# STLABTW/ST-DADK

Measured on NVIDIA B200. Metric: train_samples_per_s, higher is better.
Workload: dtype tf32

## Files before the change

### include/stdadk.h

```cpp
#ifndef STDADK_H
#define STDADK_H
#include <stddef.h>
#include <stdint.h>

#ifdef __cplusplus
extern "C" {
#endif

#define STDADK_VERSION 100
#define STDADK_MAX_Q 8

enum { STDADK_WENDLAND = 0, STDADK_GAUSSIAN = 1, STDADK_TRIANGULAR = 2 };
enum { STDADK_LOSS_NONE = 0, STDADK_LOSS_MSE = 1, STDADK_LOSS_PINBALL = 2 };

typedef struct {
    const float* knots4;
    const float* tknots2;
    int32_t k_s, k_t, p_cov, basis_fn;
} stdadk_basis;

typedef struct {
    const float* coords;
    const float* t;
    const float* xcov;
    const int64_t* index;
    int32_t grid_nx, grid_ny, grid_nt, _pad;
    int64_t row_begin;
    int64_t n_rows;
} stdadk_points;

typedef struct {
    const float* w_img;
    const float* bias;
    const float* gamma;
    const float* beta;
    int32_t n_in, n_out;
    float ln_eps;
    int32_t layer_id;
    const float* w_img_lo;
} stdadk_layer;

typedef struct {
    float p;
    uint32_t step;
    uint64_t seed;
    const int32_t* step_ptr;
    uint64_t key_offset;
} stdadk_dropout;

typedef struct {
    const float* w;
    const float* b;
    int32_t q;
    int32_t loss_type;
    const float* y;
    float taus[STDADK_MAX_Q];
    float inv_count;
    float nc_weight;
    int32_t nc_power;
    int32_t _pad;
    float* yhat;
    float* dyhat;
    float* loss_acc;
} stdadk_head;

typedef struct {
    const stdadk_basis* basis;
    stdadk_points pts;
    const float* a_img;
    stdadk_layer layer;
    stdadk_dropout drop;
    float* out_img;
    float* stats;
    const stdadk_head* head;
    const float* addend;
    float* feat_img;
    float* x_img;
    const float* a_img_lo;
    float* out_img_lo;
} stdadk_fwd_args;

typedef struct {
    const stdadk_basis* basis;
    stdadk_points pts;
    const float* a_img;
    stdadk_layer layer;
    stdadk_dropout drop;
    const float* stats;
    const stdadk_head* head;
    float* d_head_w;
    float* d_head_b;
    const float* dz_next_img;
    const float* wt_next_img;
    int32_t n_next, _pad;
    float* dz_img;
    float* d_bias;
    float* d_gamma;
    float* d_beta;
    const float* addend;
    const float* x_img;
    const float* a_img_lo;
    const float* dz_next_img_lo;
    const float* wt_next_img_lo;
    float* dz_img_lo;
} stdadk_bwd_args;

typedef struct {
    const stdadk_basis* basis;
    stdadk_points pts;
    const float* a_img;
    const float* dz_img;
    int32_t n_in, n_out;
    float* dw;
    int64_t stride_o, stride_i;
    const float* a_img_lo;
    const float* dz_img_lo;
} stdadk_wgrad_args;

typedef struct {
    const stdadk_basis* basis;
    stdadk_points pts;
    const float* dz_img;
    const float* w1s_img;
    int32_t n_out, _pad;
    float* d_centers;
    float* d_log_bw;
    const float* dz_img_lo;
    const float* w1s_img_lo;
} stdadk_knotgrad_args;

typedef struct {
    float* p;
    const float* g;
    float* m;
    float* v;
    float* shadow;
    int64_t n;
    int32_t n_groups;
    int32_t zero_grad;
    const int64_t* group_end;
    const float* hyper;
    const float* sqnorms;
    int32_t* step_count;
    float beta1, beta2, eps, ema_decay;
    float* loss_acc;
    float* loss_sum;
    float* loss_last;
    int32_t fuse_norm;
    int32_t _pad;
    float* norm_ws;
} stdadk_adamw_args;

int stdadk_version(void);
const char* stdadk_last_error(void);
size_t stdadk_sizeof(int which);

size_t stdadk_image_floats(int64_t rows, int64_t cols);

int stdadk_knots_prepare(const float* centers, const float* bw, const float* log_bw, float calib, int k,
                         float* knots4, void* stream);
int stdadk_tknots_prepare(const float* centers, const float* bw, int k, float* tknots2, void* stream);

int stdadk_basis_fwd(const stdadk_basis* basis, const stdadk_points* pts, float* phi, float* psi, void* stream);

int stdadk_pack_image(const float* src, int64_t row_stride, int64_t col_stride, int64_t rows, int64_t cols,
                      float* img, void* stream);
int stdadk_unpack_image(const float* img, int64_t rows, int64_t cols, float* dst, void* stream);
#define STDADK_MAX_PACK 8
typedef struct {
    const float* src;
    int64_t row_stride, col_stride, rows, cols;
    float* img;
    int32_t part;
    int32_t _pad;
} stdadk_pack_desc;
int stdadk_pack_images(const stdadk_pack_desc* descs, int n, void* stream);

size_t stdadk_celllist_ws_bytes(int32_t k_s, int32_t n_levels);
int stdadk_celllist_build(const float* knots4, int32_t k_s, const int32_t* level_begin, int32_t n_levels, void* ws,
                          size_t ws_bytes, void* stream);
#define STDADK_MAX_LEVELS 8
typedef struct {
    stdadk_points pts;
    const float* knots4;
    int32_t n_levels, basis_fn, n_out, p_cov;
    int32_t side[STDADK_MAX_LEVELS];
    int32_t offset[STDADK_MAX_LEVELS];
    float thetap[STDADK_MAX_LEVELS];
    const float* w1t;
    float* zs;
    const float* dz_img;
    float* dw1t;
    const void* celllist;
    int32_t celllist_k_s, _pad;
    float* d_centers;
    float* d_log_bw;
} stdadk_sparse_args;
int stdadk_sparse_l1_fwd(const stdadk_sparse_args* a, void* stream);
int stdadk_sparse_l1_wgrad(const stdadk_sparse_args* a, void* stream);

#define STDADK_MAX_HIDDEN 4
typedef struct {
    const stdadk_basis* basis;
    stdadk_points pts;
    int32_t n_layers, _pad;
    stdadk_layer layers[STDADK_MAX_HIDDEN];
    const stdadk_head* head;
} stdadk_predict_args;
int stdadk_predict_supported(const stdadk_predict_args* a);
int stdadk_predict(const stdadk_predict_args* a, void* stream);

typedef struct {
    const stdadk_basis* basis;
    const float* sites;
    int32_t grid_nx, grid_ny;
    int64_t n_sites;
    int32_t n_times, k_begin, k_end, n_layers;
    int64_t site_begin, site_end;
    stdadk_layer layers[STDADK_MAX_HIDDEN];
    const float* w1;
    int64_t w1_row_stride, w1_col_stride;
    const stdadk_head* head;
    int64_t row_base;
    float* zt_ws;
    int64_t out_k_stride;
} stdadk_field_args;
int stdadk_predict_field_supported(const stdadk_field_args* a);
int stdadk_predict_field(const stdadk_field_args* a, void* stream);

int stdadk_layer_fwd(const stdadk_fwd_args* a, void* stream);
int stdadk_layer_bwd(const stdadk_bwd_args* a, void* stream);
int stdadk_wgrad(const stdadk_wgrad_args* a, void* stream);

int stdadk_dense_basis_supported(int32_t n_in, int32_t n_out, int32_t k_s, int32_t k_t, int32_t q_head, int32_t training);
int32_t stdadk_dense_max_knots(int32_t p_cov, int32_t k_t, int32_t n_out, int32_t q_head, int32_t training);
int stdadk_knot_grad(const stdadk_knotgrad_args* a, void* stream);

size_t stdadk_sqnorm_ws_floats(void);
int stdadk_grad_sqnorm(const float* g, int64_t n, int n_groups, const int64_t* group_end, float* sqnorms,
                       float* workspace, void* stream);
int stdadk_adamw_ema_step(const stdadk_adamw_args* a, void* stream);

#define STDADK_MAX_PEERS 8
typedef struct {
    int32_t world, rank;
    float* g;
    int64_t n;
    void* recv[STDADK_MAX_PEERS];
    const int32_t* step_count;
    int32_t n_groups;
    int32_t mode;
    const int64_t* group_end;
    float* sqnorms;
    float* workspace;
} stdadk_peer_allreduce_args;
int stdadk_peer_allreduce(const stdadk_peer_allreduce_args* a, void* stream);

#ifdef __cplusplus
}
#endif
#endif
```

### st_dadk_b200/_lib.py

```python
from __future__ import annotations

import ctypes as C
import os

_HERE = os.path.dirname(os.path.abspath(__file__))
LIB_PATH = os.environ.get("STDADK_LIB") or os.path.join(_HERE, "libstdadk.so")
MAX_Q = 8

WENDLAND, GAUSSIAN, TRIANGULAR = 0, 1, 2
LOSS_NONE, LOSS_MSE, LOSS_PINBALL = 0, 1, 2
BASIS_CODE = {"wendland": WENDLAND, "gaussian": GAUSSIAN, "triangular": TRIANGULAR}
CALIBRATION = {"wendland": 1.0, "gaussian": 0.223477, "triangular": 0.654714}

fp = C.c_void_p


class Basis(C.Structure):
    _fields_ = [("knots4", fp), ("tknots2", fp), ("k_s", C.c_int32), ("k_t", C.c_int32), ("p_cov", C.c_int32),
                ("basis_fn", C.c_int32)]


class Points(C.Structure):
    _fields_ = [("coords", fp), ("t", fp), ("xcov", fp), ("index", fp), ("grid_nx", C.c_int32), ("grid_ny", C.c_int32),
                ("grid_nt", C.c_int32), ("_pad", C.c_int32), ("row_begin", C.c_int64), ("n_rows", C.c_int64)]


class Layer(C.Structure):
    _fields_ = [("w_img", fp), ("bias", fp), ("gamma", fp), ("beta", fp), ("n_in", C.c_int32), ("n_out", C.c_int32),
                ("ln_eps", C.c_float), ("layer_id", C.c_int32), ("w_img_lo", fp)]


class Dropout(C.Structure):
    _fields_ = [("p", C.c_float), ("step", C.c_uint32), ("seed", C.c_uint64), ("step_ptr", fp),
                ("key_offset", C.c_uint64)]


class Head(C.Structure):
    _fields_ = [("w", fp), ("b", fp), ("q", C.c_int32), ("loss_type", C.c_int32), ("y", fp),
                ("taus", C.c_float * MAX_Q), ("inv_count", C.c_float), ("nc_weight", C.c_float),
                ("nc_power", C.c_int32), ("_pad", C.c_int32), ("yhat", fp), ("dyhat", fp), ("loss_acc", fp)]


class FwdArgs(C.Structure):
    _fields_ = [("basis", C.POINTER(Basis)), ("pts", Points), ("a_img", fp), ("layer", Layer), ("drop", Dropout),
                ("out_img", fp), ("stats", fp), ("head", C.POINTER(Head)), ("addend", fp), ("feat_img", fp), ("x_img", fp),
                ("a_img_lo", fp), ("out_img_lo", fp)]


class BwdArgs(C.Structure):
    _fields_ = [("basis", C.POINTER(Basis)), ("pts", Points), ("a_img", fp), ("layer", Layer), ("drop", Dropout),
                ("stats", fp), ("head", C.POINTER(Head)), ("d_head_w", fp), ("d_head_b", fp), ("dz_next_img", fp),
                ("wt_next_img", fp), ("n_next", C.c_int32), ("_pad", C.c_int32), ("dz_img", fp), ("d_bias", fp),
                ("d_gamma", fp), ("d_beta", fp), ("addend", fp), ("x_img", fp), ("a_img_lo", fp), ("dz_next_img_lo", fp),
                ("wt_next_img_lo", fp), ("dz_img_lo", fp)]


class WgradArgs(C.Structure):
    _fields_ = [("basis", C.POINTER(Basis)), ("pts", Points), ("a_img", fp), ("dz_img", fp), ("n_in", C.c_int32),
                ("n_out", C.c_int32), ("dw", fp), ("stride_o", C.c_int64), ("stride_i", C.c_int64), ("a_img_lo", fp),
                ("dz_img_lo", fp)]


class KnotGradArgs(C.Structure):
    _fields_ = [("basis", C.POINTER(Basis)), ("pts", Points), ("dz_img", fp), ("w1s_img", fp), ("n_out", C.c_int32),
                ("_pad", C.c_int32), ("d_centers", fp), ("d_log_bw", fp), ("dz_img_lo", fp), ("w1s_img_lo", fp)]


class AdamWArgs(C.Structure):
    _fields_ = [("p", fp), ("g", fp), ("m", fp), ("v", fp), ("shadow", fp), ("n", C.c_int64),
                ("n_groups", C.c_int32), ("zero_grad", C.c_int32), ("group_end", C.POINTER(C.c_int64)), ("hyper", fp),
                ("sqnorms", fp), ("step_count", fp), ("beta1", C.c_float), ("beta2", C.c_float), ("eps", C.c_float),
                ("ema_decay", C.c_float), ("loss_acc", fp), ("loss_sum", fp), ("loss_last", fp), ("fuse_norm", C.c_int32),
                ("_pad", C.c_int32), ("norm_ws", fp)]


MAX_LEVELS = 8


class SparseArgs(C.Structure):
    _fields_ = [("pts", Points), ("knots4", fp), ("n_levels", C.c_int32), ("basis_fn", C.c_int32), ("n_out", C.c_int32),
                ("p_cov", C.c_int32), ("side", C.c_int32 * MAX_LEVELS), ("offset", C.c_int32 * MAX_LEVELS),
                ("thetap", C.c_float * MAX_LEVELS), ("w1t", fp), ("zs", fp), ("dz_img", fp), ("dw1t", fp),
                ("celllist", fp), ("celllist_k_s", C.c_int32), ("_pad", C.c_int32), ("d_centers", fp), ("d_log_bw", fp)]


class PackDesc(C.Structure):
    _fields_ = [("src", fp), ("row_stride", C.c_int64), ("col_stride", C.c_int64), ("rows", C.c_int64),
                ("cols", C.c_int64), ("img", fp), ("part", C.c_int32), ("_pad", C.c_int32)]


MAX_HIDDEN = 4


class PredictArgs(C.Structure):
    _fields_ = [("basis", C.POINTER(Basis)), ("pts", Points), ("n_layers", C.c_int32), ("_pad", C.c_int32),
                ("layers", Layer * MAX_HIDDEN), ("head", C.POINTER(Head))]


class FieldArgs(C.Structure):
    _fields_ = [("basis", C.POINTER(Basis)), ("sites", fp), ("grid_nx", C.c_int32), ("grid_ny", C.c_int32),
                ("n_sites", C.c_int64), ("n_times", C.c_int32), ("k_begin", C.c_int32), ("k_end", C.c_int32),
                ("n_layers", C.c_int32), ("site_begin", C.c_int64), ("site_end", C.c_int64),
                ("layers", Layer * MAX_HIDDEN), ("w1", fp), ("w1_row_stride", C.c_int64), ("w1_col_stride", C.c_int64),
                ("head", C.POINTER(Head)), ("row_base", C.c_int64), ("zt_ws", fp), ("out_k_stride", C.c_int64)]


MAX_PEERS = 8


class PeerAllreduceArgs(C.Structure):
    _fields_ = [("world", C.c_int32), ("rank", C.c_int32), ("g", fp), ("n", C.c_int64), ("recv", fp * MAX_PEERS),
                ("step_count", fp), ("n_groups", C.c_int32), ("mode", C.c_int32), ("group_end", C.POINTER(C.c_int64)),
                ("sqnorms", fp), ("workspace", fp)]


_lib = None

_PROTOS = {
    "stdadk_version": (C.c_int, []),
    "stdadk_last_error": (C.c_char_p, []),
    "stdadk_sizeof": (C.c_size_t, [C.c_int]),
    "stdadk_image_floats": (C.c_size_t, [C.c_int64, C.c_int64]),
    "stdadk_knots_prepare": (C.c_int, [fp, fp, fp, C.c_float, C.c_int, fp, fp]),
    "stdadk_tknots_prepare": (C.c_int, [fp, fp, C.c_int, fp, fp]),
    "stdadk_basis_fwd": (C.c_int, [C.POINTER(Basis), C.POINTER(Points), fp, fp, fp]),
    "stdadk_pack_image": (C.c_int, [fp, C.c_int64, C.c_int64, C.c_int64, C.c_int64, fp, fp]),
    "stdadk_unpack_image": (C.c_int, [fp, C.c_int64, C.c_int64, fp, fp]),
    "stdadk_pack_images": (C.c_int, [C.POINTER(PackDesc), C.c_int, fp]),
    "stdadk_predict_supported": (C.c_int, [C.POINTER(PredictArgs)]),
    "stdadk_predict": (C.c_int, [C.POINTER(PredictArgs), fp]),
    "stdadk_predict_field_supported": (C.c_int, [C.POINTER(FieldArgs)]),
    "stdadk_predict_field": (C.c_int, [C.POINTER(FieldArgs), fp]),
    "stdadk_peer_allreduce": (C.c_int, [C.POINTER(PeerAllreduceArgs), fp]),
    "stdadk_layer_fwd": (C.c_int, [C.POINTER(FwdArgs), fp]),
    "stdadk_layer_bwd": (C.c_int, [C.POINTER(BwdArgs), fp]),
    "stdadk_wgrad": (C.c_int, [C.POINTER(WgradArgs), fp]),
    "stdadk_dense_basis_supported": (C.c_int, [C.c_int32] * 6),
    "stdadk_dense_max_knots": (C.c_int32, [C.c_int32] * 5),
    "stdadk_knot_grad": (C.c_int, [C.POINTER(KnotGradArgs), fp]),
    "stdadk_sqnorm_ws_floats": (C.c_size_t, []),
    "stdadk_grad_sqnorm": (C.c_int, [fp, C.c_int64, C.c_int, C.POINTER(C.c_int64), fp, fp, fp]),
    "stdadk_adamw_ema_step": (C.c_int, [C.POINTER(AdamWArgs), fp]),
    "stdadk_celllist_ws_bytes": (C.c_size_t, [C.c_int32, C.c_int32]),
    "stdadk_celllist_build": (C.c_int, [fp, C.c_int32, C.POINTER(C.c_int32), C.c_int32, fp, C.c_size_t, fp]),
    "stdadk_sparse_l1_fwd": (C.c_int, [C.POINTER(SparseArgs), fp]),
    "stdadk_sparse_l1_wgrad": (C.c_int, [C.POINTER(SparseArgs), fp]),
}
EXPORTED = list(_PROTOS)


def lib():
    global _lib
    if _lib is None:
        if not os.path.exists(LIB_PATH):
            raise RuntimeError(
                f"{LIB_PATH} not found: build it with `python -c 'import __graft_entry__ as g; g.build()'` "
                "(nvcc, sm_100a).  st_dadk_b200 has no CPU or PyTorch fallback path.")
        L = C.CDLL(LIB_PATH)
        for name, (res, args) in _PROTOS.items():
            if not hasattr(L, name):
                continue
            fn = getattr(L, name)
            fn.restype = res
            fn.argtypes = args
        structs = [(0, Basis), (1, Points), (2, Layer), (3, Dropout), (4, Head), (5, FwdArgs), (6, BwdArgs), (7, WgradArgs),
                   (8, KnotGradArgs), (9, AdamWArgs), (10, PackDesc), (11, SparseArgs), (12, PredictArgs),
                   (14, PeerAllreduceArgs), (15, FieldArgs)]
        for i, st in structs:
            if L.stdadk_sizeof(i) != C.sizeof(st):
                raise RuntimeError(f"libstdadk ABI mismatch: {st.__name__} is {C.sizeof(st)} B in the binding, "
                                   f"{L.stdadk_sizeof(i)} B in the library")
        _lib = L
    return _lib


def check(code: int, what: str):
    if code != 0:
        msg = lib().stdadk_last_error().decode("utf-8", "replace")
        raise RuntimeError(f"libstdadk {what} failed (code {code}): {msg}")
```

### st_dadk_b200/csrc/api.cu

```cuda
#include <cstdarg>
#include <cstdio>
#include <cstring>

#include "layer.cuh"
#include "misc.cuh"
#include "sparse.cuh"
#include "predict.cuh"
#include "field.cuh"

using namespace stdadk;

static thread_local char g_err[512] = "";

static int fail(int code, const char* fmt, ...) {
    va_list ap;
    va_start(ap, fmt);
    vsnprintf(g_err, sizeof(g_err), fmt, ap);
    va_end(ap);
    return code;
}
static int check_launch(const char* what) {
    cudaError_t e = cudaGetLastError();
    if (e != cudaSuccess) return fail((int)e, "%s: %s", what, cudaGetErrorString(e));
    return 0;
// ... 183 lines not shown
    tknots_prepare_kernel<<<(k + 127) / 128, 128, 0, (cudaStream_t)stream>>>(centers, bw, k,
                                                                              reinterpret_cast<float2*>(tknots2));
    return check_launch("tknots_prepare");
}

int stdadk_basis_fwd(const stdadk_basis* basis, const stdadk_points* pts, float* phi, float* psi, void* stream) {
    if (int r = check_device()) return r;
    REQUIRE(basis && pts, "basis_fwd: NULL descriptor");
    if (int r = check_basis_points(basis, *pts, -1)) return r;
    if (pts->n_rows <= 0) return 0;
    long long total = pts->n_rows * (long long)(basis->k_s + basis->k_t);
    if (total == 0) return 0;
    basis_fwd_kernel<<<grid_for(total, 256), 256, 0, (cudaStream_t)stream>>>(to_basis(basis), to_points(*pts), phi,
                                                                              psi);
    return check_launch("basis_fwd");
}

int stdadk_pack_image(const float* src, int64_t row_stride, int64_t col_stride, int64_t rows, int64_t cols,
                      float* img, void* stream) {
    if (int r = check_device()) return r;
    REQUIRE(src && img && rows > 0 && cols > 0, "pack_image: bad arguments");
    REQUIRE((reinterpret_cast<uintptr_t>(img) & 127) == 0, "pack_image: image must be 128-byte aligned");
    int slabs = (int)ceil_div64(cols, SLAB_K);
    long long chunks = (long long)ceil_div64(rows, TILE_M) * slabs * (SLAB_FLOATS / 4);
    pack_image_kernel<<<grid_for(chunks, 256), 256, 0, (cudaStream_t)stream>>>(src, row_stride, col_stride, rows, cols,
                                                                                img, chunks, slabs);
    return check_launch("pack_image");
}

int stdadk_pack_images(const stdadk_pack_desc* descs, int n, void* stream) {
    if (int r = check_device()) return r;
    REQUIRE(descs && n >= 1 && n <= STDADK_MAX_PACK, "pack_images: 1..%d descriptors, got %d", STDADK_MAX_PACK, n);
    PackBatch B{};
    B.n = n;
    long long max_chunks = 0;
    for (int i = 0; i < n; ++i) {
        REQUIRE(descs[i].src && descs[i].img && descs[i].rows > 0 && descs[i].cols > 0, "pack_images: bad descriptor %d", i);
        REQUIRE((reinterpret_cast<uintptr_t>(descs[i].img) & 127) == 0, "pack_images: image %d must be 128-byte aligned", i);
        B.d[i] = descs[i];
        long long chunks = ceil_div64(descs[i].rows, TILE_M) * ceil_div64(descs[i].cols, SLAB_K) * (SLAB_FLOATS / 4);
        if (chunks > max_chunks) max_chunks = chunks;
    }
    dim3 grid(grid_for(max_chunks, 256, 2), n);
    launch_chained(pack_images_kernel, grid, 256, 0, stream, B);
    return check_launch("pack_images");
}

int stdadk_unpack_image(const float* img, int64_t rows, int64_t cols, float* dst, void* stream) {
    if (int r = check_device()) return r;
    REQUIRE(dst && img && rows > 0 && cols > 0, "unpack_image: bad arguments");
    int slabs = (int)ceil_div64(cols, SLAB_K);
    unpack_image_kernel<<<grid_for(rows * cols, 256), 256, 0, (cudaStream_t)stream>>>(img, rows, cols, dst, slabs);
    return check_launch("unpack_image");
}

static int check_layer(const stdadk_layer& l, const char* who) {
    REQUIRE(l.w_img && l.bias, "%s: weight image / bias is NULL", who);
    REQUIRE(l.n_out >= 1 && l.n_out <= MAX_N, "%s: n_out=%d outside [1,%d] (one UMMA N / LayerNorm row per thread)", who,
            l.n_out, MAX_N);
    REQUIRE(l.n_in >= 1, "%s: n_in=%d", who, l.n_in);
    REQUIRE((l.gamma == nullptr) == (l.beta == nullptr), "%s: gamma and beta must both be given or both NULL", who);
    REQUIRE(((reinterpret_cast<uintptr_t>(l.w_img) | reinterpret_cast<uintptr_t>(l.w_img_lo)) & 127) == 0,
            "%s: weight images must be 128-byte aligned", who);
    return 0;
}

constexpr uint32_t SMEM_LIMIT = 227 * 1024;
constexpr int BWD_CG = 2, BWD_NS = 4;
static uint32_t fwd_smem(int n_pad, int q, int k_s, int k_t, int tab_chunks, int cg) {
    return plan_smem(n_pad, q, k_s, k_t, false, cg, cg == 2 ? 2 : 4, tab_chunks).total;
}
static uint32_t bwd_smem(int n_pad, int q, int k_s, int k_t, int tab_chunks) {
    return plan_smem(n_pad, q, k_s, k_t, true, BWD_CG, BWD_NS, tab_chunks).total;
}

static unsigned long long* g_predict_dbg = nullptr;
int stdadk_layer_fwd(const stdadk_fwd_args* a, void* stream) {
    if (int r = check_device()) return r;
    REQUIRE(a, "layer_fwd: NULL args");
    if (int r = check_layer(a->layer, "layer_fwd")) return r;
    REQUIRE((a->basis != nullptr) != (a->a_img != nullptr), "layer_fwd: give exactly one of basis / a_img");
    if (a->basis)
        if (int r = check_basis_points(a->basis, a->pts, a->layer.n_in)) return r;
    REQUIRE(a->drop.p >= 0.0f && a->drop.p < 1.0f, "layer_fwd: dropout p=%f", a->drop.p);
    REQUIRE(!a->addend || (a->layer.n_out % 4 == 0 && (reinterpret_cast<uintptr_t>(a->addend) & 15) == 0),
            "layer_fwd: addend needs n_out %% 4 == 0 and 16-byte alignment");
    if (a->head) {
        REQUIRE(a->head->q >= 1 && a->head->q <= STDADK_MAX_Q, "layer_fwd: head q=%d outside [1,%d]", a->head->q,
                STDADK_MAX_Q);
        REQUIRE(a->head->w && a->head->b && a->head->yhat, "layer_fwd: head w/b/yhat NULL");
        REQUIRE(a->head->loss_type == STDADK_LOSS_NONE || (a->head->y && a->head->loss_acc),
                "layer_fwd: loss requested without y / loss_acc");
    } else {
        REQUIRE(a->out_img, "layer_fwd: out_img is NULL and there is no head");
    }
    const bool x3 = a->layer.w_img_lo != nullptr;
    if (x3) {
        REQUIRE(!a->a_img || a->a_img_lo, "layer_fwd: tf32x3 needs a_img_lo next to a_img");
        REQUIRE(!a->out_img || a->out_img_lo, "layer_fwd: tf32x3 needs out_img_lo next to out_img");
        REQUIRE(!a->feat_img, "layer_fwd: feat_img is not available in tf32x3 mode");
    }
    if (a->pts.n_rows <= 0) return 0;
    FwdK K{};
    K.basis = to_basis(a->basis);
    K.pts = to_points(a->pts);
    K.L = to_layer(a->layer, a->drop);
    K.head = to_head(a->head);
    K.a_img = a->a_img;
    K.a_img_lo = a->a_img_lo;
    K.out_img_lo = x3 ? a->out_img_lo : nullptr;
    K.passes = x3 ? 3 : 1;
    K.addend = a->addend;
    K.x_img = a->x_img;
    K.feat_img = a->basis ? a->feat_img : nullptr;
    K.dbg = g_predict_dbg;
    K.out_img = a->out_img;
    K.stats = a->stats;
    K.has_head = a->head ? 1 : 0;
    K.k_slabs = pad32(a->layer.n_in) / SLAB_K;
    K.n_pad = pad32(a->layer.n_out);
    K.thresh16 = dropout_thresh16(a->drop.p);
    K.drop_scale = a->drop.p > 0.0f ? 1.0f / (1.0f - a->drop.p) : 1.0f;
    const bool basis = a->basis != nullptr;
    int tiles = (int)ceil_div64(a->pts.n_rows, TILE_M);
    const int sms = g_sm_count > 0 ? g_sm_count : 148;
    const int cg = tiles >= 2 * sms ? 2 : 4;
    const bool half_tiles = 2 * tiles <= sms;
    if (half_tiles) tiles *= 2;
    K.tmem_cols = half_tiles ? tmem_cols_m64(K.n_pad) : pow2_cols(K.n_pad);
    const uint32_t smem = fwd_smem(K.n_pad, K.has_head ? K.head.q : 0, basis ? K.basis.k_s : 0, basis ? K.basis.k_t : 0,
                                   basis ? K.k_slabs * 8 : 0, cg);
    REQUIRE(smem <= SMEM_LIMIT, "layer_fwd: needs %u B of shared memory (> 227 KB): too many knots for the dense path",
            smem);
    K.n_tiles = tiles;
#define LAUNCH_FWD(B, TM, C)                                                                                 \
    do {                                                                                                     \
        if (int r = set_smem(layer_fwd_kernel<B, TM, C, (C == 2 ? 2 : 4)>, smem)) return r;                  \
        launch_chained(layer_fwd_kernel<B, TM, C, (C == 2 ? 2 : 4)>, dim3(tiles), n_threads(C), smem, stream, K); \
    } while (0)
    if (basis) {
        if (half_tiles) LAUNCH_FWD(true, 64, 4);
        else if (cg == 2) LAUNCH_FWD(true, 128, 2);
        else LAUNCH_FWD(true, 128, 4);
    } else {
        if (half_tiles) LAUNCH_FWD(false, 64, 4);
        else if (cg == 2) LAUNCH_FWD(false, 128, 2);
        else LAUNCH_FWD(false, 128, 4);
    }
#undef LAUNCH_FWD
    return check_launch("layer_fwd");
}

extern "C" void stdadk_debug_counters(void* dev_u64x16) { g_predict_dbg = static_cast<unsigned long long*>(dev_u64x16); }

static int fill_pred_layers(const stdadk_layer* layers, int n_layers, PredLayerP* out, const char* who) {
    for (int l = 0; l < n_layers; ++l) {
        const stdadk_layer& y = layers[l];
        if (int r = check_layer(y, who)) return r;
        REQUIRE(l == 0 || y.n_in == layers[l - 1].n_out, "%s: block %d n_in=%d != previous n_out=%d", who, l, y.n_in,
                layers[l - 1].n_out);
        PredLayerP& L = out[l];
        L.w_img = y.w_img;
        L.bias = y.bias;
        L.gamma = y.gamma;
        L.beta = y.beta;
        L.n_out = y.n_out;
        L.n_pad = pad32(y.n_out);
        L.k_slabs = pad32(y.n_in) / SLAB_K;
        L.has_ln = y.gamma != nullptr;
        L.eps = y.ln_eps;
    }
    return 0;
}

static int predict_fill(const stdadk_predict_args* a, PredK* K) {
    REQUIRE(a && a->basis && a->head, "predict: NULL args / basis / head");
    REQUIRE(a->n_layers >= 1 && a->n_layers <= PF_MAX_LAYERS, "predict: %d hidden blocks outside [1,%d]", a->n_layers,
            PF_MAX_LAYERS);
    if (int r = check_basis_points(a->basis, a->pts, a->layers[0].n_in)) return r;
    REQUIRE(a->head->q >= 1 && a->head->q <= STDADK_MAX_Q, "predict: head q=%d outside [1,%d]", a->head->q, STDADK_MAX_Q);
    REQUIRE(a->head->w && a->head->b && a->head->yhat, "predict: head w/b/yhat NULL");
    *K = PredK{};
    K->basis = to_basis(a->basis);
    K->pts = to_points(a->pts);
    K->n_layers = a->n_layers;
    K->q = a->head->q;
    K->head_w = a->head->w;
    K->head_b = a->head->b;
    K->yhat = a->head->yhat;
    if (int r = fill_pred_layers(a->layers, a->n_layers, K->L, "predict")) return r;
    uint32_t bytes = plan_predict(*K);
    REQUIRE(bytes <= 227 * 1024, "predict: the fused kernel needs %u B of shared memory (> 227 KB) for this shape", bytes);
    K->n_tiles = (int)ceil_div64(a->pts.n_rows, TILE_M);
    K->dbg = g_predict_dbg;
    return 0;
}

int stdadk_predict_supported(const stdadk_predict_args* a) {
    PredK K;
    return predict_fill(a, &K) == 0 ? 1 : 0;
}

int stdadk_predict(const stdadk_predict_args* a, void* stream) {
    if (int r = check_device()) return r;
    PredK Kl;
    if (int r = predict_fill(a, &Kl)) return r;
    if (a->pts.n_rows <= 0) return 0;
    if (int r = set_smem(predict_fused_kernel, Kl.sm.total)) return r;
    const int sms = g_sm_count > 0 ? g_sm_count : 148;
    const int grid = Kl.n_tiles < sms ? Kl.n_tiles : sms;
    predict_fused_kernel<<<grid, PF_NT, Kl.sm.total, (cudaStream_t)stream>>>(Kl);
    return check_launch("predict");
}

static int field_fill(const stdadk_field_args* a, FieldK* K) {
    REQUIRE(a && a->basis && a->head, "predict_field: NULL args / basis / head");
    REQUIRE(a->n_layers >= 1 && a->n_layers <= PF_MAX_LAYERS, "predict_field: %d hidden blocks outside [1,%d]", a->n_layers,
            PF_MAX_LAYERS);
    const stdadk_basis* b = a->basis;
    REQUIRE(b->p_cov == 0, "predict_field: covariates (p_cov=%d) are per (site, time): use stdadk_predict", b->p_cov);
    REQUIRE(b->k_s >= 1 && b->knots4 && (b->k_t == 0 || b->tknots2), "predict_field: basis tables missing");
    REQUIRE(((reinterpret_cast<uintptr_t>(b->knots4)) & 15) == 0, "predict_field: knots4 must be 16-byte aligned");
    REQUIRE(b->basis_fn >= 0 && b->basis_fn <= 2, "predict_field: unknown basis_fn %d", b->basis_fn);
    REQUIRE(a->layers[0].n_in == b->k_s, "predict_field: layers[0] is the spatial part: n_in=%d != k_s=%d", a->layers[0].n_in,
            b->k_s);
    REQUIRE(a->n_sites >= 1 && a->n_times >= 1, "predict_field: n_sites / n_times");
    REQUIRE(a->sites || (a->grid_nx > 0 && a->grid_ny > 0 && (int64_t)a->grid_nx * a->grid_ny == a->n_sites),
            "predict_field: give sites or a lattice with nx*ny == n_sites");
    REQUIRE(!a->sites || (reinterpret_cast<uintptr_t>(a->sites) & 7) == 0, "predict_field: sites must be 8-byte aligned");
    REQUIRE(0 <= a->k_begin && a->k_begin <= a->k_end && a->k_end <= a->n_times, "predict_field: time range");
    REQUIRE(0 <= a->site_begin && a->site_begin <= a->site_end && a->site_end <= a->n_sites, "predict_field: site range");
    REQUIRE(a->out_k_stride >= 0, "predict_field: out_k_stride");
    REQUIRE(a->head->q >= 1 && a->head->q <= STDADK_MAX_Q && a->head->w && a->head->b && a->head->yhat,
            "predict_field: head q / w / b / yhat");
    REQUIRE(a->w1 && a->zt_ws && (reinterpret_cast<uintptr_t>(a->zt_ws) & 15) == 0, "predict_field: w1 / zt_ws");
    *K = FieldK{};
    K->basis = to_basis(b);
    K->basis.k_t = 0;
    K->basis.tknots = nullptr;
    K->sites = a->sites;
    K->nx = a->grid_nx;
    K->ny = a->grid_ny;
    K->n_sites = a->n_sites;
    K->site_begin = a->site_begin;
    K->site_end = a->site_end;
    K->k_begin = a->k_begin;
    K->k_end = a->k_end;
    K->n_layers = a->n_layers;
    K->q = a->head->q;
    K->head_w = a->head->w;
    K->head_b = a->head->b;
    K->yhat = a->head->yhat;
    K->row_base = a->row_base;
    K->out_k_stride = a->out_k_stride > 0 ? a->out_k_stride : a->n_sites;
    K->zt = a->zt_ws;
    K->dbg = g_predict_dbg;
    if (int r = fill_pred_layers(a->layers, a->n_layers, K->L, "predict_field")) return r;
    REQUIRE(K->L[0].k_slabs <= PF_HSLABS, "predict_field: %d spatial knots exceed the resident operand (%d)", b->k_s,
            PF_HSLABS * SLAB_K);
    uint32_t bytes = plan_field(*K);
    REQUIRE(bytes <= 227 * 1024, "predict_field: the kernel needs %u B of shared memory (> 227 KB) for this shape", bytes);
    const int sms = g_sm_count > 0 ? g_sm_count : 148;
    const long long n_s = a->site_end - a->site_begin;
    const int tk = a->k_end - a->k_begin;
    K->n_site_tiles = (int)ceil_div64(n_s, TILE_M);
    int best_chunk = tk > 0 ? tk : 1;
    double best_cost = 1e30;
    for (int chunk = 1; chunk <= tk; ++chunk) {
        const long long units = (long long)K->n_site_tiles * ((tk + chunk - 1) / chunk);
        const double cost = (double)ceil_div64(units, sms) * (chunk + 1.0);
        if (cost < best_cost - 1e-9 || (cost < best_cost + 1e-9 && chunk > best_chunk)) {
            best_cost = cost;
            best_chunk = chunk;
        }
    }
    K->k_chunk = best_chunk;
    K->n_kchunks = tk > 0 ? (tk + best_chunk - 1) / best_chunk : 0;
    const long long units = (long long)K->n_site_tiles * K->n_kchunks;
    REQUIRE(units < (1ll << 31), "predict_field: too many work units");
    K->n_units = (int)units;
    return 0;
}

int stdadk_predict_field_supported(const stdadk_field_args* a) {
    FieldK K;
    return field_fill(a, &K) == 0 ? 1 : 0;
}

int stdadk_predict_field(const stdadk_field_args* a, void* stream) {
    if (int r = check_device()) return r;
    FieldK K;
    if (int r = field_fill(a, &K)) return r;
    if (K.n_units <= 0) return 0;
    const int pad0 = K.L[0].n_pad, total = a->n_times * pad0;
    field_zt_kernel<<<(total + 255) / 256, 256, 0, (cudaStream_t)stream>>>(
        a->w1, a->w1_row_stride, a->w1_col_stride, a->basis->k_s, a->layers[0].bias,
        reinterpret_cast<const float2*>(a->basis->tknots2), a->basis->k_t, K.L[0].n_out, pad0, a->n_times, a->zt_ws);
    if (int r = check_launch("predict_field (zt)")) return r;
    if (int r = set_smem(predict_field_kernel, K.sm.total)) return r;
    const int sms = g_sm_count > 0 ? g_sm_count : 148;
    const int grid = K.n_units < sms ? K.n_units : sms;
    predict_field_kernel<<<grid, PF_NT, K.sm.total, (cudaStream_t)stream>>>(K);
    return check_launch("predict_field");
}

int stdadk_layer_bwd(const stdadk_bwd_args* a, void* stream) {
    if (int r = check_device()) return r;
    REQUIRE(a, "layer_bwd: NULL args");
    if (int r = check_layer(a->layer, "layer_bwd")) return r;
    REQUIRE(a->x_img || ((a->basis != nullptr) != (a->a_img != nullptr)), "layer_bwd: give exactly one of basis / a_img");
    if (a->basis && !a->x_img)
        if (int r = check_basis_points(a->basis, a->pts, a->layer.n_in)) return r;
    REQUIRE((a->head != nullptr) != (a->dz_next_img != nullptr), "layer_bwd: give exactly one of head / dz_next_img");
    REQUIRE(a->dz_img && a->d_bias, "layer_bwd: dz_img / d_bias NULL");
    REQUIRE(!a->layer.gamma || (a->d_gamma && a->d_beta && a->stats), "layer_bwd: LayerNorm needs d_gamma/d_beta/stats");
    if (a->head) {
        REQUIRE(a->head->q >= 1 && a->head->q <= STDADK_MAX_Q && a->head->w && a->head->dyhat && a->d_head_w &&
                    a->d_head_b,
                "layer_bwd: head arguments incomplete");
    } else {
        REQUIRE(a->wt_next_img && a->n_next >= 1 && a->n_next <= MAX_N, "layer_bwd: wt_next_img / n_next invalid");
    }
    const bool x3 = a->layer.w_img_lo != nullptr;
    if (x3) {
        REQUIRE(a->x_img || !a->a_img || a->a_img_lo, "layer_bwd: tf32x3 needs a_img_lo next to a_img");
        REQUIRE(a->head || (a->dz_next_img_lo && a->wt_next_img_lo), "layer_bwd: tf32x3 needs dz_next_img_lo / wt_next_img_lo");
        REQUIRE(a->dz_img_lo, "layer_bwd: tf32x3 needs dz_img_lo");
    }
    if (a->pts.n_rows <= 0) return 0;
    BwdK K{};
    K.basis = to_basis(a->basis);
    K.pts = to_points(a->pts);
    K.L = to_layer(a->layer, a->drop);
    K.head = to_head(a->head);
    K.a_img = a->a_img;
    K.a_img_lo = a->a_img_lo;
    K.dz_next_img_lo = a->dz_next_img_lo;
    K.wt_next_img_lo = a->wt_next_img_lo;
    K.dz_img_lo = x3 ? a->dz_img_lo : nullptr;
    K.passes = x3 ? 3 : 1;
    K.addend = a->addend;
    K.x_img = a->x_img;
    K.stats = a->stats;
    K.dz_next_img = a->dz_next_img;
    K.wt_next_img = a->wt_next_img;
    K.dz_img = a->dz_img;
    K.d_bias = a->d_bias;
    K.d_gamma = a->d_gamma;
    K.d_beta = a->d_beta;
    K.d_head_w = a->d_head_w;
    K.d_head_b = a->d_head_b;
    K.has_head = a->head ? 1 : 0;
    K.k_slabs = a->x_img ? 0 : pad32(a->layer.n_in) / SLAB_K;
    K.k_slabs2 = a->head ? 0 : pad32(a->n_next) / SLAB_K;
    K.n_pad = pad32(a->layer.n_out);
    K.thresh16 = dropout_thresh16(a->drop.p);
    K.drop_scale = a->drop.p > 0.0f ? 1.0f / (1.0f - a->drop.p) : 1.0f;
    const bool basis = a->basis != nullptr && a->x_img == nullptr;
    constexpr int BCG = BWD_CG, BNS = BWD_NS;
    const uint32_t smem = bwd_smem(K.n_pad, K.has_head ? K.head.q : 0, basis ? K.basis.k_s : 0, basis ? K.basis.k_t : 0,
                                   basis ? K.k_slabs * 8 : 0);
    REQUIRE(smem <= SMEM_LIMIT, "layer_bwd: needs %u B of shared memory (> 227 KB)", smem);
    int tiles = (int)ceil_div64(a->pts.n_rows, TILE_M);
    const int sms = g_sm_count > 0 ? g_sm_count : 148;
    const bool half_tiles = a->x_img && 2 * tiles <= sms;
    if (half_tiles) tiles *= 2;
    K.tmem_cols = 2 * (half_tiles ? tmem_cols_m64(K.n_pad) : pow2_cols(K.n_pad));
    const bool ln = a->layer.gamma != nullptr, hd = a->head != nullptr;
#define LAUNCH_BWD(B, TM, LNV, HD)                                                                          \
    do {                                                                                                    \
        if (int r = set_smem(layer_bwd_kernel<B, TM, BCG, BNS, LNV, HD>, smem)) return r;                   \
        launch_chained(layer_bwd_kernel<B, TM, BCG, BNS, LNV, HD>, dim3(tiles), n_threads(BCG), smem, stream, K); \
    } while (0)
    if (half_tiles) {
        if (ln && hd) LAUNCH_BWD(false, 64, true, true);
        else if (ln) LAUNCH_BWD(false, 64, true, false);
        else if (hd) LAUNCH_BWD(false, 64, false, true);
        else LAUNCH_BWD(false, 64, false, false);
    } else if (basis) {
        if (ln && hd) LAUNCH_BWD(true, 128, true, true);
        else if (ln) LAUNCH_BWD(true, 128, true, false);
        else if (hd) LAUNCH_BWD(true, 128, false, true);
        else LAUNCH_BWD(true, 128, false, false);
    } else {
        if (ln && hd) LAUNCH_BWD(false, 128, true, true);
        else if (ln) LAUNCH_BWD(false, 128, true, false);
        else if (hd) LAUNCH_BWD(false, 128, false, true);
        else LAUNCH_BWD(false, 128, false, false);
    }
#undef LAUNCH_BWD
    return check_launch("layer_bwd");
}

int stdadk_wgrad(const stdadk_wgrad_args* a, void* stream) {
    if (int r = check_device()) return r;
    REQUIRE(a, "wgrad: NULL args");
    REQUIRE((a->basis != nullptr) != (a->a_img != nullptr), "wgrad: give exactly one of basis / a_img");
    REQUIRE(a->dz_img && a->dw, "wgrad: dz_img / dw NULL");
    REQUIRE(a->n_out >= 1 && a->n_out <= MAX_N && a->n_in >= 1, "wgrad: bad sizes n_in=%d n_out=%d", a->n_in, a->n_out);
    if (a->basis)
        if (int r = check_basis_points(a->basis, a->pts, a->n_in)) return r;
    if (a->pts.n_rows <= 0) return 0;
    const bool x3 = a->dz_img_lo != nullptr;
    REQUIRE(!x3 || !a->a_img || a->a_img_lo, "wgrad: tf32x3 needs a_img_lo next to a_img");
    WgradK K{};
    K.basis = to_basis(a->basis);
    K.pts = to_points(a->pts);
    K.a_img = a->a_img;
    K.a_img_lo = a->a_img_lo;
    K.dz_img_lo = a->dz_img_lo;
    K.passes = x3 ? 3 : 1;
    K.dz_img = a->dz_img;
    K.dw = a->dw;
    K.stride_o = a->stride_o;
    K.stride_i = a->stride_i;
    K.n_in = a->n_in;
    K.n_out = a->n_out;
    K.a_slabs = pad32(a->n_in) / SLAB_K;
    K.dz_slabs = pad32(a->n_out) / SLAB_K;
    K.n_row_tiles = (int)ceil_div64(a->pts.n_rows, TILE_M);
    int n_tiles_n = (K.a_slabs + 7) / 8;
    K.nt_slabs = (K.a_slabs + n_tiles_n - 1) / n_tiles_n;
    K.tmem_cols = pow2_cols(K.nt_slabs * SLAB_K);
    int m_tiles = (K.dz_slabs + 3) / 4;
    int per = m_tiles * n_tiles_n;
    int sms = g_sm_count > 0 ? g_sm_count : 148;
    int splits = sms / per;
    if (splits < 1) splits = 1;
    if (splits > K.n_row_tiles) splits = K.n_row_tiles;
    const bool basis = a->basis != nullptr;
    uint32_t smem = wgrad_smem_bytes(basis ? K.basis.k_s : 0, basis ? K.basis.k_t : 0);
    REQUIRE(smem <= SMEM_LIMIT, "wgrad: needs %u B of shared memory (> 227 KB)", smem);
    dim3 grid(splits, m_tiles, n_tiles_n);
    constexpr int WCG = 2;
    if (basis) {
        if (int r = set_smem(wgrad_kernel<true, WCG>, smem)) return r;
        launch_chained(wgrad_kernel<true, WCG>, grid, n_threads(WCG), smem, stream, K);
    } else {
        if (int r = set_smem(wgrad_kernel<false, WCG>, smem)) return r;
        launch_chained(wgrad_kernel<false, WCG>, grid, n_threads(WCG), smem, stream, K);
    }
    return check_launch("wgrad");
}

static int dense_basis_check(int n_in, int n_out, int k_s, int k_t, int q_head, int training) {
    REQUIRE(n_out >= 1 && n_out <= MAX_N && k_s >= 0 && k_t >= 0 && n_in >= k_s + k_t && q_head >= 0 &&
                q_head <= STDADK_MAX_Q,
            "dense_basis_supported: bad sizes n_in=%d n_out=%d k_s=%d k_t=%d q_head=%d", n_in, n_out, k_s, k_t, q_head);
    const int n_pad = pad32(n_out), tab_chunks = pad32(n_in) / SLAB_K * 8;
    for (int cg : {4, 2}) {
        const uint32_t b = fwd_smem(n_pad, q_head, k_s, k_t, tab_chunks, cg);
        REQUIRE(b <= SMEM_LIMIT, "layer_fwd: needs %u B of shared memory (> 227 KB): too many knots for the dense path", b);
    }
    if (!training) return 0;
    const uint32_t bb = bwd_smem(n_pad, q_head, k_s, k_t, tab_chunks);
    REQUIRE(bb <= SMEM_LIMIT, "layer_bwd: needs %u B of shared memory (> 227 KB)", bb);
    const uint32_t wb = wgrad_smem_bytes(k_s, k_t);
    REQUIRE(wb <= SMEM_LIMIT, "wgrad: needs %u B of shared memory (> 227 KB)", wb);
    return 0;
}

int stdadk_dense_basis_supported(int32_t n_in, int32_t n_out, int32_t k_s, int32_t k_t, int32_t q_head, int32_t training) {
    return dense_basis_check(n_in, n_out, k_s, k_t, q_head, training) == 0 ? 1 : 0;
}

int32_t stdadk_dense_max_knots(int32_t p_cov, int32_t k_t, int32_t n_out, int32_t q_head, int32_t training) {
    if (p_cov < 0 || dense_basis_check(p_cov + k_t, n_out, 0, k_t, q_head, training)) return -1;
    int lo = 0, hi = 1 << 14;
    while (hi - lo > 1) {
        const int mid = (lo + hi) / 2;
        if (dense_basis_check(p_cov + mid + k_t, n_out, mid, k_t, q_head, training) == 0) lo = mid;
        else hi = mid;
    }
    return lo;
}

int stdadk_knot_grad(const stdadk_knotgrad_args* a, void* stream) {
    if (int r = check_device()) return r;
    REQUIRE(a && a->basis && a->dz_img && a->w1s_img && a->d_centers && a->d_log_bw, "knot_grad: NULL argument");
    if (int r = check_basis_points(a->basis, a->pts, -1)) return r;
    REQUIRE(a->n_out >= 1 && a->n_out <= MAX_N, "knot_grad: n_out=%d", a->n_out);
    if (a->pts.n_rows <= 0 || a->basis->k_s == 0) return 0;
    KnotGradK K{};
    K.basis = to_basis(a->basis);
    K.pts = to_points(a->pts);
    REQUIRE((a->dz_img_lo != nullptr) == (a->w1s_img_lo != nullptr), "knot_grad: give both residual images or neither");
    K.dz_img = a->dz_img;
    K.w1s_img = a->w1s_img;
    K.dz_img_lo = a->dz_img_lo;
    K.w1s_img_lo = a->w1s_img_lo;
    K.passes = a->dz_img_lo ? 3 : 1;
    K.d_centers = a->d_centers;
    K.d_log_bw = a->d_log_bw;
    K.n_out = a->n_out;
    K.k_slabs = pad32(a->n_out) / SLAB_K;
// ... 42 lines not shown
    }
    REQUIRE((a->d_centers == nullptr) == (a->d_log_bw == nullptr), "sparse_l1: give d_centers and d_log_bw together");
    REQUIRE(!(wgrad && a->d_centers) || (a->w1t && (reinterpret_cast<uintptr_t>(a->w1t) & 15) == 0),
            "sparse_l1_wgrad: knot gradients need w1t (G = dz1 . W1t row)");
    K->d_centers = wgrad ? a->d_centers : nullptr;
    K->d_log_bw = wgrad ? a->d_log_bw : nullptr;
    K->knots = reinterpret_cast<const float4*>(a->knots4);
    K->w1t = a->w1t;
    K->zs = a->zs;
    K->dz_img = a->dz_img;
    K->dw1t = a->dw1t;
    K->n_out = a->n_out;
    K->p_cov = a->p_cov;
    K->fn = a->basis_fn;
    return 0;
}

static int make_groups(int n_groups, const int64_t* group_end, int64_t n, GroupsP* G) {
    REQUIRE(n_groups >= 1 && n_groups <= 8 && group_end, "optimizer: 1..8 parameter groups supported, got %d", n_groups);
    int64_t prev = 0;
    for (int i = 0; i < n_groups; ++i) {
        REQUIRE(group_end[i] >= prev, "optimizer: group_end must be non-decreasing");
        G->end[i] = prev = group_end[i];
    }
    REQUIRE(prev == n, "optimizer: last group_end (%lld) != n (%lld)", (long long)prev, (long long)n);
    G->n = n_groups;
    return 0;
}

size_t stdadk_celllist_ws_bytes(int32_t k_s, int32_t n_levels) {
    if (k_s < 0 || n_levels < 1 || n_levels > SP_MAX_LEVELS) return 0;
    return celllist_bytes(k_s, n_levels);
}

int stdadk_celllist_build(const float* knots4, int32_t k_s, const int32_t* level_begin, int32_t n_levels, void* ws,
                          size_t ws_bytes, void* stream) {
    if (int r = check_device()) return r;
    REQUIRE(knots4 && level_begin && ws && k_s >= 1, "celllist_build: NULL argument / no knots");
    REQUIRE(n_levels >= 1 && n_levels <= SP_MAX_LEVELS, "celllist_build: 1..%d levels, got %d", SP_MAX_LEVELS, n_levels);
    REQUIRE(((reinterpret_cast<uintptr_t>(ws) | reinterpret_cast<uintptr_t>(knots4)) & 15) == 0,
            "celllist_build: knots4 / workspace must be 16-byte aligned");
    REQUIRE(ws_bytes >= celllist_bytes(k_s, n_levels), "celllist_build: workspace of %zu B, need %zu B", ws_bytes,
            celllist_bytes(k_s, n_levels));
    CellBuildK K{};
    K.knots = reinterpret_cast<const float4*>(knots4);
    K.k_s = k_s;
    K.n_levels = n_levels;
    for (int l = 0; l <= n_levels; ++l) {
        REQUIRE(level_begin[l] >= (l ? level_begin[l - 1] : 0) && level_begin[l] <= k_s, "celllist_build: level_begin not monotone");
        K.level_begin[l] = level_begin[l];
    }
    REQUIRE(level_begin[0] == 0 && level_begin[n_levels] == k_s, "celllist_build: levels must cover [0, k_s)");
    K.ws = static_cast<int*>(ws);
    size_t ib = (celllist_ints(k_s, n_levels) * 4 + 15) & ~(size_t)15;
    K.sorted = reinterpret_cast<float4*>(static_cast<uint8_t*>(ws) + ib);
    celllist_build_kernel<<<1, CL_THREADS, 0, (cudaStream_t)stream>>>(K);
    return check_launch("celllist_build");
}

size_t stdadk_sqnorm_ws_floats(void) { return (size_t)SQNORM_BLOCKS * 8 + 8; }

int stdadk_grad_sqnorm(const float* g, int64_t n, int n_groups, const int64_t* group_end, float* sqnorms,
                       float* workspace, void* stream) {
    if (int r = check_device()) return r;
    REQUIRE(g && sqnorms && workspace && n > 0, "grad_sqnorm: bad arguments (workspace of stdadk_sqnorm_ws_floats() "
            "zero-initialised floats is required)");
    REQUIRE((reinterpret_cast<uintptr_t>(g) & 15) == 0, "grad_sqnorm: g must be 16-byte aligned");
    GroupsP G{};
    if (int r = make_groups(n_groups, group_end, n, &G)) return r;
    long long blocks = ((n >> 2) + SQNORM_THREADS * 4 - 1) / (SQNORM_THREADS * 4);
    if (blocks < 1) blocks = 1;
    if (blocks > SQNORM_BLOCKS) blocks = SQNORM_BLOCKS;
    sqnorm_kernel<<<(int)blocks, SQNORM_THREADS, 0, (cudaStream_t)stream>>>(g, n, G, sqnorms, workspace);
    return check_launch("grad_sqnorm");
}

int stdadk_sparse_l1_fwd(const stdadk_sparse_args* a, void* stream) {
    if (int r = check_device()) return r;
    SparseK K{};
    if (int r = sparse_fill(a, &K, false)) return r;
    if (a->pts.n_rows <= 0) return 0;
    int blocks = grid_for(a->pts.n_rows, SP_WARPS, 8);
    sparse_spatial_fwd_kernel<<<blocks, SP_WARPS * 32, 0, (cudaStream_t)stream>>>(K);
    return check_launch("sparse_l1_fwd");
}

int stdadk_sparse_l1_wgrad(const stdadk_sparse_args* a, void* stream) {
    if (int r = check_device()) return r;
    SparseK K{};
    if (int r = sparse_fill(a, &K, true)) return r;
    if (a->pts.n_rows <= 0) return 0;
    int blocks = grid_for(a->pts.n_rows, SP_WARPS, 8);
    sparse_spatial_wgrad_kernel<<<blocks, SP_WARPS * 32, 0, (cudaStream_t)stream>>>(K);
    return check_launch("sparse_l1_wgrad");
}

__global__ void step_inc_kernel(int* c) { *c += 1; }

int stdadk_peer_allreduce(const stdadk_peer_allreduce_args* a, void* stream) {
    if (int r = check_device()) return r;
    REQUIRE(a && a->g && a->step_count, "peer_allreduce: NULL argument");
    REQUIRE(a->world >= 2 && a->world <= PEER_MAX && a->rank >= 0 && a->rank < a->world,
            "peer_allreduce: world=%d rank=%d outside [2,%d]", a->world, a->rank, PEER_MAX);
    REQUIRE(a->n > 0 && a->n % 4 == 0, "peer_allreduce: n=%lld must be a positive multiple of 4", (long long)a->n);
    static_assert(PEER_MAX == STDADK_MAX_PEERS, "peer limits differ");
    REQUIRE((reinterpret_cast<uintptr_t>(a->g) & 15) == 0, "peer_allreduce: g must be 16-byte aligned");
    PeerK K{};
    for (int r = 0; r < a->world; ++r) {
        REQUIRE(a->recv[r] && (reinterpret_cast<uintptr_t>(a->recv[r]) & 15) == 0,
                "peer_allreduce: rank %d receive area not mapped / not 16-byte aligned", r);
        K.recv[r] = static_cast<uint4*>(a->recv[r]);
    }
    K.g = a->g;
    K.n2 = a->n / 2;
    K.step_count = a->step_count;
    K.rank = a->rank;
    K.world = a->world;
    REQUIRE(a->mode >= 0 && a->mode <= 2, "peer_allreduce: mode=%d (0 automatic, 1 one-shot, 2 two-phase)", a->mode);
    K.two_phase = a->mode == 2 || (a->mode == 0 && a->world >= 4);
    if (a->n_groups > 0) {
        REQUIRE(a->group_end && a->sqnorms && a->workspace, "peer_allreduce: fused norm needs group_end / sqnorms / workspace");
        K.n_norm = a->group_end[a->n_groups - 1];
        REQUIRE(K.n_norm <= a->n, "peer_allreduce: norm range exceeds n");
        if (int r = make_groups(a->n_groups, a->group_end, K.n_norm, &K.G)) return r;
        K.sq_out = a->sqnorms;
        K.ws = a->workspace;
    }
    long long blocks = (K.n2 + PEER_THREADS * 2 - 1) / (PEER_THREADS * 2);
    if (blocks > 148) blocks = 148;
    if (blocks < 1) blocks = 1;
    peer_allreduce_kernel<<<(int)blocks, PEER_THREADS, 0, (cudaStream_t)stream>>>(K);
    return check_launch("peer_allreduce");
}

int stdadk_adamw_ema_step(const stdadk_adamw_args* a, void* stream) {
    if (int r = check_device()) return r;
    REQUIRE(a && a->p && a->g && a->m && a->v && a->hyper && a->step_count && a->n > 0, "adamw: bad arguments");
    AdamK K{};
    if (int r = make_groups(a->n_groups, a->group_end, a->n, &K.G)) return r;
    K.p = a->p;
    K.g = a->g;
    K.m = a->m;
    K.v = a->v;
    K.shadow = a->shadow;
    K.n = a->n;
    K.hyper = a->hyper;
    K.sqnorms = a->sqnorms;
    K.step_count = a->step_count;
    K.beta1 = a->beta1;
    K.beta2 = a->beta2;
    K.eps = a->eps;
    K.ema_decay = a->ema_decay;
    K.g_zero = a->zero_grad ? const_cast<float*>(a->g) : nullptr;
    K.loss_acc = a->loss_acc;
    K.loss_sum = a->loss_sum;
    K.loss_last = a->loss_last;
    REQUIRE(((reinterpret_cast<uintptr_t>(a->p) | reinterpret_cast<uintptr_t>(a->g) | reinterpret_cast<uintptr_t>(a->m) |
              reinterpret_cast<uintptr_t>(a->v) | reinterpret_cast<uintptr_t>(a->shadow)) & 15) == 0,
            "adamw: buffers must be 16-byte aligned");
    if (a->fuse_norm) {
        REQUIRE(a->norm_ws, "adamw: fuse_norm needs norm_ws");
        K.sq_out = const_cast<float*>(a->sqnorms);
        K.norm_ws = a->norm_ws;
        K.step_rw = a->step_count;
        long long blocks = ((a->n + 3) / 4 + 255) / 256;
        if (blocks > 148) blocks = 148;
        const int sms = g_sm_count > 0 ? g_sm_count : 148;
        if (blocks > sms) blocks = sms;
        if (blocks < 1) blocks = 1;
        launch_chained(adamw_ema_kernel<true>, dim3((unsigned)blocks), 256, 0, stream, K);
        return check_launch("adamw_ema_step (fused tail)");
    }
    step_inc_kernel<<<1, 1, 0, (cudaStream_t)stream>>>(a->step_count);
    adamw_ema_kernel<false><<<grid_for((a->n + 3) / 4, 256, 8), 256, 0, (cudaStream_t)stream>>>(K);
    return check_launch("adamw_ema_step");
}

}
```

### st_dadk_b200/csrc/common.cuh

```cuda
#pragma once
#include <cuda_runtime.h>
#include <stdint.h>
#include <type_traits>

#include "../../include/stdadk.h"
#include "ptx.cuh"

namespace stdadk {

constexpr int TILE_M = 128;
constexpr int SLAB_K = 32;
constexpr int SLAB_FLOATS = TILE_M * SLAB_K;
constexpr int SLAB_BYTES = SLAB_FLOATS * 4;
constexpr int MAX_N = 256;

__host__ __device__ inline int pad32(int x) { return (x + 31) & ~31; }
__host__ __device__ inline int64_t ceil_div64(int64_t a, int64_t b) { return (a + b - 1) / b; }

struct BasisP {
    const float4* knots;
    const float2* tknots;
    int k_s, k_t, p_cov, fn;
};
struct PointsP {
    const float* coords;
    const float* t;
    const float* xcov;
    const long long* index;
    int nx, ny, nt, _pad;
    long long row_begin;
    long long n_rows;
};
struct HeadP {
    const float* w;
    const float* b;
    const float* y;
    float* yhat;
    float* dyhat;
    float* loss_acc;
    int q, loss_type, nc_power, _pad;
    float inv_count, nc_weight;
    float taus[STDADK_MAX_Q];
};
struct LayerP {
    const float* w_img;
    const float* w_img_lo;
    const float* bias;
    const float* gamma;
    const float* beta;
    int n_in, n_out, layer_id, _pad;
    float eps, drop_p;
    unsigned int step, _pad2;
    unsigned long long seed;
    const int* step_ptr;
    unsigned long long key_offset;
};
__device__ __forceinline__ unsigned int dropout_step(const LayerP& L) {
    return L.step_ptr ? (unsigned int)(*L.step_ptr) : L.step;
}
__device__ __forceinline__ long long sample_of(const PointsP& P, long long g) { return P.index ? P.index[g] : g; }

__device__ __forceinline__ float rsqrt_approx(float x) {
    float r;
    asm("rsqrt.approx.ftz.f32 %0, %1;" : "=f"(r) : "f"(x));
    return r;
}
__device__ __forceinline__ float ex2_approx(float x) {
    float r;
    asm("ex2.approx.ftz.f32 %0, %1;" : "=f"(r) : "f"(x));
    return r;
}
template <int FN>
__device__ __forceinline__ float phi_from_d2(float d2, float th2, float inv_th) {
    if (FN == STDADK_GAUSSIAN) return ex2_approx(-0.72134752044448170f * (d2 * inv_th * inv_th));
    const float r = d2 * rsqrt_approx(fmaxf(d2, 1e-30f)) * inv_th;
    const float u = fmaxf(1.0f - r, 0.0f);
    float v;
    if (FN == STDADK_TRIANGULAR) {
        v = u;
    } else {
        const float u2 = u * u;
        v = (u2 * u2) * u2 * fmaf(fmaf(35.0f / 3.0f, r, 6.0f), r, 1.0f);
    }
    return d2 < th2 ? v : 0.0f;
}
__device__ __forceinline__ float phi_eval(int fn, float dx, float dy, float th2, float inv_th) {
    const float d2 = __fadd_rn(__fmul_rn(dx, dx), __fmul_rn(dy, dy));
    if (fn == STDADK_GAUSSIAN) return phi_from_d2<STDADK_GAUSSIAN>(d2, th2, inv_th);
    if (!(d2 < th2)) return 0.0f;
    if (fn == STDADK_TRIANGULAR) return phi_from_d2<STDADK_TRIANGULAR>(d2, th2, inv_th);
    return phi_from_d2<STDADK_WENDLAND>(d2, th2, inv_th);
}
__device__ __forceinline__ float phi_dr(int fn, float r) {
    if (fn == STDADK_GAUSSIAN) return -r * exp2f(-0.72134752044448170f * r * r);
    if (!(r < 1.0f)) return 0.0f;
    if (fn == STDADK_TRIANGULAR) return -1.0f;
    float u = 1.0f - r;
    float u2 = u * u;
    return -(56.0f / 3.0f) * r * fmaf(5.0f, r, 1.0f) * u2 * u2 * u;
}
__device__ __forceinline__ float psi_eval(float t, float c, float inv_bw) {
    float s = (t - c) * inv_bw;
    return ex2_approx(-0.72134752044448170f * s * s);
}

__device__ __forceinline__ void load_point(const PointsP& P, long long g, float& x, float& y, float& t) {
    if (P.nx > 0) {
        long long j = g % P.ny;
        long long i = (g / P.ny) % P.nx;
        long long k = g / ((long long)P.ny * P.nx);
        x = P.nx > 1 ? __fdiv_rn((float)i, (float)(P.nx - 1)) : 0.0f;
        y = P.ny > 1 ? __fdiv_rn((float)j, (float)(P.ny - 1)) : 0.0f;
        t = P.nt > 1 ? __fdiv_rn((float)k, (float)(P.nt - 1)) : 0.0f;
    } else {
        long long sidx = sample_of(P, g);
        float2 c = *reinterpret_cast<const float2*>(P.coords + 2 * sidx);
        x = c.x;
        y = c.y;
        t = P.t[sidx];
    }
}

__device__ __forceinline__ float feature_value(const BasisP& B, const float4* sk, const float2* st, int f, float x,
                                               float y, float t, const float* xrow) {
    if (f < B.p_cov) return xrow ? xrow[f] : 0.0f;
    f -= B.p_cov;
    if (f < B.k_s) {
        float4 kn = sk[f];
        return phi_eval(B.fn, x - kn.x, y - kn.y, kn.z, kn.w);
    }
    f -= B.k_s;
    if (f < B.k_t) {
        float2 tk = st[f];
        return psi_eval(t, tk.x, tk.y);
    }
    return 0.0f;
}

__device__ __forceinline__ void philox4x32_10(uint32_t c0, uint32_t c1, uint32_t c2, uint32_t c3, uint32_t k0,
                                              uint32_t k1, uint32_t (&out)[4]) {
#pragma unroll
    for (int i = 0; i < 10; ++i) {
        uint32_t hi0 = __umulhi(0xD2511F53u, c0), lo0 = 0xD2511F53u * c0;
        uint32_t hi1 = __umulhi(0xCD9E8D57u, c2), lo1 = 0xCD9E8D57u * c2;
        c0 = hi1 ^ c1 ^ k0;
        c1 = lo1;
        c2 = hi0 ^ c3 ^ k1;
        c3 = lo0;
        k0 += 0x9E3779B9u;
        k1 += 0xBB67AE85u;
    }
    out[0] = c0; out[1] = c1; out[2] = c2; out[3] = c3;
}
__device__ __noinline__ uint32_t dropout_keep8(unsigned long long seed, uint32_t step, uint32_t layer,
                                                  unsigned long long row, uint32_t block, uint32_t thresh16) {
    uint32_t o[4];
    philox4x32_10((uint32_t)row, block, layer | ((uint32_t)(row >> 32) << 8), step, (uint32_t)seed,
                  (uint32_t)(seed >> 32), o);
    uint32_t bits = 0;
#pragma unroll
    for (int e = 0; e < 8; ++e) {
// ... 31 lines not shown
```

### st_dadk_b200/csrc/layer.cuh

```cuda
#pragma once
#include "common.cuh"

namespace stdadk {

constexpr int WG_NSTAGE = 2;
constexpr int RED_STRIDE = 4 + STDADK_MAX_Q;
__host__ __device__ constexpr int n_work(int cg) { return 128 * cg; }
__host__ __device__ constexpr int n_threads(int cg) { return 128 * cg + 64; }
__device__ __forceinline__ void worker_barrier(int nw) { asm volatile("bar.sync 1, %0;" ::"r"(nw) : "memory"); }

template <int TM>
struct TileGeo {
    static_assert(TM == 128 || TM == 64, "tile height");
    static constexpr int ROWS_PER_WARP = TM / 4;
    static constexpr int WARP_COLS = TM == 128 ? 32 : 64;
    __device__ static int row(int q4, int lane) { return q4 * ROWS_PER_WARP + (TM == 128 ? lane : (lane & 15)); }
    __device__ static int chunk_off(int lane) { return TM == 128 ? 0 : (lane >> 4) * 32; }
    __device__ static int group(int cg, int lane) { return TM == 128 ? cg : 2 * cg + (lane >> 4); }
    __host__ __device__ static constexpr int groups(int cg) { return TM == 128 ? cg : 2 * cg; }
};
template <int TM>
__device__ __forceinline__ void acc_ld(uint32_t taddr, float (&v)[32]) {
    if (TM == 128) tmem_ld32(taddr, v);
    else tmem_ld16x2<32>(taddr, v);
}
__device__ __forceinline__ float2 halfwarp_transpose_sum(float (&v)[32], int lane) {
#pragma unroll
    for (int off = 8, n = 16; off >= 1; off >>= 1, n >>= 1) {
        bool upper = (lane & off) != 0;
#pragma unroll
        for (int i = 0; i < n; ++i) {
            float send = upper ? v[i] : v[i + n];
            float keep = upper ? v[i + n] : v[i];
            v[i] = keep + __shfl_xor_sync(0xffffffffu, send, off);
        }
    }
    return make_float2(v[0], v[1]);
}
template <int TM>
__device__ __forceinline__ void colsum_chunk(float* cs, int c0, bool cvalid, float (&v)[32], int lane) {
    if (TM == 128) {
        const float s = warp_transpose_sum(v, lane);
        atomicAdd(&cs[c0 + lane], s);
    } else {
        const float2 s = halfwarp_transpose_sum(v, lane);
        if (cvalid) {
            atomicAdd(&cs[c0 + 2 * (lane & 15)], s.x);
            atomicAdd(&cs[c0 + 2 * (lane & 15) + 1], s.y);
        }
    }
}

struct SmemPlan {
    uint32_t a_off, b_off, bar_off, tmem_off, vec_off, headw_off, knots_off, tknots_off, colsum_off, red_off, total;
};
__host__ __device__ inline SmemPlan plan_smem(int n_pad, int q, int k_s, int k_t, bool bwd, int cg = 1, int ns = 2,
                                              int tab_chunks = 0) {
    SmemPlan s;
    uint32_t o = 0;
    s.a_off = o; o += ns * SLAB_BYTES;
    s.b_off = o; o += ns * (uint32_t)n_pad * 128u;
    s.bar_off = o; o += 128;
    s.tmem_off = o; o += 16;
    s.vec_off = o; o += 4u * n_pad * 4u;
    s.headw_off = o; o += (uint32_t)(q > 0 ? (q * n_pad + STDADK_MAX_Q) * 4 : 0);
    o = (o + 15u) & ~15u;
    s.knots_off = o; o += tab_chunks > 0 ? (uint32_t)tab_chunks * 64u : (uint32_t)k_s * 16u;
    s.tknots_off = o; o += tab_chunks > 0 ? 0u : (uint32_t)k_t * 8u;
    o = (o + 15u) & ~15u;
    s.colsum_off = o; o += bwd ? (uint32_t)((3 + q) * n_pad + STDADK_MAX_Q) * 4u : 0u;
    s.red_off = s.a_off;
    (void)cg;
    s.total = o + 1024;
    return s;
}

struct FwdK {
    BasisP basis;
    PointsP pts;
    LayerP L;
    HeadP head;
    const float* a_img;
    const float* a_img_lo;
    const float* addend;
    float* out_img;
    float* out_img_lo;
    float* x_img;
    float* feat_img;
    float* stats;
    int has_head, k_slabs, n_pad, tmem_cols;
    unsigned int thresh16;
    float drop_scale;
    int n_tiles, passes;
    unsigned long long* dbg;
};
#ifdef STDADK_PF_DEBUG
#define FWD_T(slot)                                                       \
    do {                                                                  \
        if (P.dbg && tid == 0) {                                          \
            unsigned long long now_;                                      \
            asm volatile("mov.u64 %0, %%globaltimer;" : "=l"(now_));      \
            atomicAdd(P.dbg + (slot), now_ - t_prev_);                    \
            t_prev_ = now_;                                               \
        }                                                                 \
    } while (0)
#define FWD_WAIT(slot, stmt)                                               \
    do {                                                                   \
        unsigned long long w0_ = 0, w1_;                                   \
        if (P.dbg) asm volatile("mov.u64 %0, %%globaltimer;" : "=l"(w0_)); \
        stmt;                                                              \
        if (P.dbg) {                                                       \
            asm volatile("mov.u64 %0, %%globaltimer;" : "=l"(w1_));        \
            atomicAdd(P.dbg + (slot), w1_ - w0_);                          \
        }                                                                  \
    } while (0)
#else
#define FWD_T(slot)
#define FWD_WAIT(slot, stmt) stmt
#endif

struct BwdK {
    BasisP basis;
    PointsP pts;
    LayerP L;
    HeadP head;
    const float* a_img;
    const float* a_img_lo;
    const float* addend;
    const float* x_img;
    const float* stats;
    const float* dz_next_img;
    const float* dz_next_img_lo;
    const float* wt_next_img;
    const float* wt_next_img_lo;
    float* dz_img;
    float* dz_img_lo;
    float* d_bias;
    float* d_gamma;
    float* d_beta;
    float* d_head_w;
    float* d_head_b;
    int has_head, k_slabs, k_slabs2, n_pad, tmem_cols, passes;
    unsigned int thresh16;
    float drop_scale;
};

template <int FN>
__device__ __forceinline__ float4 spatial_chunk(const float4* kp, float x, float y, bool lo) {
    float d2[4], th2[4], ith[4];
    bool in = false;
#pragma unroll
    for (int e = 0; e < 4; ++e) {
        const float4 kn = kp[e];
        const float dx = x - kn.x, dy = y - kn.y;
        d2[e] = __fadd_rn(__fmul_rn(dx, dx), __fmul_rn(dy, dy));
        th2[e] = kn.z;
        ith[e] = kn.w;
        in |= d2[e] < th2[e];
    }
    if (FN != STDADK_GAUSSIAN && !__any_sync(__activemask(), in)) return make_float4(0.f, 0.f, 0.f, 0.f);
    float o[4];
#pragma unroll
    for (int e = 0; e < 4; ++e) o[e] = tf32_part(phi_from_d2<FN>(d2[e], th2[e], ith[e]), lo);
    return make_float4(o[0], o[1], o[2], o[3]);
}
__device__ __forceinline__ float4 feature_chunk(const BasisP& B, const float4* sk, const float2* st, int f, float x,
                                                float y, float t, const float* xrow, bool lo = false) {
    const int s0 = B.p_cov, s1 = B.p_cov + B.k_s, t1 = s1 + B.k_t;
    if (f >= s0 && f + 4 <= s1) {
        const float4* kp = sk + (f - s0);
        if (B.fn == STDADK_WENDLAND) return spatial_chunk<STDADK_WENDLAND>(kp, x, y, lo);
        if (B.fn == STDADK_TRIANGULAR) return spatial_chunk<STDADK_TRIANGULAR>(kp, x, y, lo);
        return spatial_chunk<STDADK_GAUSSIAN>(kp, x, y, lo);
    }
    if (f >= s1 && f + 4 <= t1) {
        const float2* tp = st + (f - s1);
        float o[4];
#pragma unroll
        for (int e = 0; e < 4; ++e) {
            float2 tk = tp[e];
            o[e] = tf32_part(psi_eval(t, tk.x, tk.y), lo);
        }
        return make_float4(o[0], o[1], o[2], o[3]);
    }
    if (f >= t1) return make_float4(0.f, 0.f, 0.f, 0.f);
    return make_float4(tf32_part(feature_value(B, sk, st, f + 0, x, y, t, xrow), lo),
                       tf32_part(feature_value(B, sk, st, f + 1, x, y, t, xrow), lo),
                       tf32_part(feature_value(B, sk, st, f + 2, x, y, t, xrow), lo),
                       tf32_part(feature_value(B, sk, st, f + 3, x, y, t, xrow), lo));
}

__device__ __forceinline__ int chunk_kind(const BasisP& B, int f) {
    const int s0 = B.p_cov, s1 = s0 + B.k_s, t1 = s1 + B.k_t;
    if (f >= s0 && f + 4 <= s1) return 0;
    if (f >= s1 && f + 4 <= t1) return 1;
    if (f >= t1) return 2;
    return 3;
}
__device__ __forceinline__ void build_chunk_tables(const BasisP& B, float4* tab, int n_chunks, int tid, int nt) {
    for (int ci = tid; ci < n_chunks; ci += nt) {
        const int f = 4 * ci, kind = chunk_kind(B, f);
        float4* g = tab + 4 * ci;
        if (kind == 0) {
            const float4* kp = B.knots + (f - B.p_cov);
            const float4 k0 = kp[0], k1 = kp[1], k2 = kp[2], k3 = kp[3];
            g[0] = make_float4(k0.x, k1.x, k2.x, k3.x);
            g[1] = make_float4(k0.y, k1.y, k2.y, k3.y);
            g[2] = make_float4(k0.z, k1.z, k2.z, k3.z);
            g[3] = make_float4(k0.w, k1.w, k2.w, k3.w);
        } else if (kind == 1) {
            const float2* tp = B.tknots + (f - B.p_cov - B.k_s);
            const float2 t0 = tp[0], t1 = tp[1], t2 = tp[2], t3 = tp[3];
            g[0] = make_float4(t0.x, t1.x, t2.x, t3.x);
            g[1] = make_float4(t0.y, t1.y, t2.y, t3.y);
        }
    }
}
template <int FN, bool LO, int NC>
__device__ __forceinline__ void spatial_chunks_soa(const float4* g, float2 xx, float2 yy, float4 (&out)[NC]) {
    constexpr bool lo = LO;
    float2 d2a[NC], d2b[NC];
    float4 th2[NC], ith[NC];
    bool in = false;
#pragma unroll
    for (int k = 0; k < NC; ++k) {
        const float4 cx = g[4 * k], cy = g[4 * k + 1];
        th2[k] = g[4 * k + 2];
        ith[k] = g[4 * k + 3];
        const float2 dxa = sub2(xx, make_float2(cx.x, cx.y)), dxb = sub2(xx, make_float2(cx.z, cx.w));
        const float2 dya = sub2(yy, make_float2(cy.x, cy.y)), dyb = sub2(yy, make_float2(cy.z, cy.w));
        const float2 pxa = mul2(dxa, dxa), pya = mul2(dya, dya), pxb = mul2(dxb, dxb), pyb = mul2(dyb, dyb);
        d2a[k] = make_float2(__fadd_rn(pxa.x, pya.x), __fadd_rn(pxa.y, pya.y));
        d2b[k] = make_float2(__fadd_rn(pxb.x, pyb.x), __fadd_rn(pxb.y, pyb.y));
        in |= (d2a[k].x < th2[k].x) | (d2a[k].y < th2[k].y) | (d2b[k].x < th2[k].z) | (d2b[k].y < th2[k].w);
    }
    if (FN == STDADK_GAUSSIAN) {
        const float2 kk = make_float2(-0.72134752044448170f, -0.72134752044448170f);
#pragma unroll
        for (int k = 0; k < NC; ++k) {
            const float2 ia = make_float2(ith[k].x, ith[k].y), ib = make_float2(ith[k].z, ith[k].w);
            const float2 ea = mul2(kk, mul2(mul2(d2a[k], ia), ia)), eb = mul2(kk, mul2(mul2(d2b[k], ib), ib));
            out[k] = make_float4(tf32_part(ex2_approx(ea.x), lo), tf32_part(ex2_approx(ea.y), lo),
                                 tf32_part(ex2_approx(eb.x), lo), tf32_part(ex2_approx(eb.y), lo));
        }
        return;
    }
    if (!__any_sync(__activemask(), in)) {
#pragma unroll
        for (int k = 0; k < NC; ++k) out[k] = make_float4(0.f, 0.f, 0.f, 0.f);
        return;
    }
    const float2 one = make_float2(1.0f, 1.0f);
#pragma unroll
    for (int k = 0; k < NC; ++k) {
        const float2 qa = make_float2(rsqrt_approx(fmaxf(d2a[k].x, 1e-30f)), rsqrt_approx(fmaxf(d2a[k].y, 1e-30f)));
        const float2 qb = make_float2(rsqrt_approx(fmaxf(d2b[k].x, 1e-30f)), rsqrt_approx(fmaxf(d2b[k].y, 1e-30f)));
        const float2 ra = mul2(mul2(d2a[k], qa), make_float2(ith[k].x, ith[k].y));
        const float2 rb = mul2(mul2(d2b[k], qb), make_float2(ith[k].z, ith[k].w));
        float2 ua = sub2(one, ra), ub = sub2(one, rb);
        ua = make_float2(fmaxf(ua.x, 0.0f), fmaxf(ua.y, 0.0f));
        ub = make_float2(fmaxf(ub.x, 0.0f), fmaxf(ub.y, 0.0f));
        float2 va = ua, vb = ub;
        if (FN == STDADK_WENDLAND) {
            const float2 c35 = make_float2(35.0f / 3.0f, 35.0f / 3.0f), c6 = make_float2(6.0f, 6.0f);
            const float2 u2a = mul2(ua, ua), u2b = mul2(ub, ub);
            va = mul2(mul2(mul2(u2a, u2a), u2a), fma2(fma2(c35, ra, c6), ra, one));
            vb = mul2(mul2(mul2(u2b, u2b), u2b), fma2(fma2(c35, rb, c6), rb, one));
        }
        out[k] = make_float4(tf32_part(d2a[k].x < th2[k].x ? va.x : 0.0f, lo), tf32_part(d2a[k].y < th2[k].y ? va.y : 0.0f, lo),
                             tf32_part(d2b[k].x < th2[k].z ? vb.x : 0.0f, lo), tf32_part(d2b[k].y < th2[k].w ? vb.y : 0.0f, lo));
    }
}
template <int FN, bool LO>
__device__ __forceinline__ float4 spatial_chunk_soa(const float4* g, float2 xx, float2 yy) {
    float4 o[1];
    spatial_chunks_soa<FN, LO, 1>(g, xx, yy, o);
    return o[0];
}
template <bool LO>
__device__ __forceinline__ float4 temporal_chunk_soa(const float4* g, float2 tt) {
    constexpr bool lo = LO;
    const float4 c = g[0], ib = g[1];
    const float2 kk = make_float2(-0.72134752044448170f, -0.72134752044448170f);
    const float2 sa = mul2(sub2(tt, make_float2(c.x, c.y)), make_float2(ib.x, ib.y));
    const float2 sb = mul2(sub2(tt, make_float2(c.z, c.w)), make_float2(ib.z, ib.w));
    const float2 ea = mul2(mul2(kk, sa), sa), eb = mul2(mul2(kk, sb), sb);
    return make_float4(tf32_part(ex2_approx(ea.x), lo), tf32_part(ex2_approx(ea.y), lo), tf32_part(ex2_approx(eb.x), lo),
                       tf32_part(ex2_approx(eb.y), lo));
}
template <int FN, bool LO, int NC>
__device__ __forceinline__ void gen_basis_slab_soa(const BasisP& B, const float4* tab, int slab, float x, float y, float t,
                                                   const float* xrow, uint32_t slab_saddr, uint32_t r, int c_begin, int c_end,
                                                   float* gslab) {
    constexpr bool lo = LO;
    const float2 xx = make_float2(x, x), yy = make_float2(y, y), tt = make_float2(t, t);
// ... 94 lines not shown
#pragma unroll
    for (int c = 0; c < 8; ++c) {
        const float4 hi = make_float4(to_tf32(v[4 * c]), to_tf32(v[4 * c + 1]), to_tf32(v[4 * c + 2]), to_tf32(v[4 * c + 3]));
        *reinterpret_cast<float4*>(reinterpret_cast<uint8_t*>(img + off) + swz_off(row, c)) = hi;
        if (img_lo)
            *reinterpret_cast<float4*>(reinterpret_cast<uint8_t*>(img_lo + off) + swz_off(row, c)) =
                make_float4(to_tf32(v[4 * c] - hi.x), to_tf32(v[4 * c + 1] - hi.y), to_tf32(v[4 * c + 2] - hi.z),
                            to_tf32(v[4 * c + 3] - hi.w));
    }
}

__device__ __forceinline__ uint8_t* align_smem(uint8_t* p) {
    return p + ((1024u - (smem_u32(p) & 1023u)) & 1023u);
}

__device__ __forceinline__ void add_addend_chunk(float (&v)[32], const float* addend_row, int c0, int n_out) {
#pragma unroll
    for (int c = 0; c < 8; ++c) {
        if (c0 + 4 * c < n_out) {
            float4 a = *reinterpret_cast<const float4*>(addend_row + c0 + 4 * c);
            v[4 * c] += a.x; v[4 * c + 1] += a.y; v[4 * c + 2] += a.z; v[4 * c + 3] += a.w;
        }
    }
}

__device__ __forceinline__ void image_store_chunk(float* img, int tile, int slabs, int c0, uint32_t row, const float (&v)[32]) {
    float* dst = img + ((size_t)tile * slabs + (c0 / SLAB_K)) * SLAB_FLOATS;
#pragma unroll
    for (int c = 0; c < 8; ++c)
        *reinterpret_cast<float4*>(reinterpret_cast<uint8_t*>(dst) + swz_off(row, c)) =
            make_float4(v[4 * c], v[4 * c + 1], v[4 * c + 2], v[4 * c + 3]);
}
__device__ __forceinline__ void image_load_chunk(const float* img, int tile, int slabs, int c0, uint32_t row, float (&v)[32]) {
    const float* src = img + ((size_t)tile * slabs + (c0 / SLAB_K)) * SLAB_FLOATS;
#pragma unroll
    for (int c = 0; c < 8; ++c) {
        float4 q = *reinterpret_cast<const float4*>(reinterpret_cast<const uint8_t*>(src) + swz_off(row, c));
        v[4 * c] = q.x; v[4 * c + 1] = q.y; v[4 * c + 2] = q.z; v[4 * c + 3] = q.w;
    }
}

__device__ __forceinline__ float row_loss(const HeadP& H, const float* yh, float yt, float* dy) {
    float loss = 0.0f;
    const int q = H.q;
    if (H.loss_type == STDADK_LOSS_MSE) {
#pragma unroll
        for (int k = 0; k < STDADK_MAX_Q; ++k)
            if (k < q) {
                float e = yh[k] - yt;
                loss += e * e;
                dy[k] = 2.0f * e * H.inv_count;
            }
        loss *= H.inv_count;
    } else {
#pragma unroll
        for (int k = 0; k < STDADK_MAX_Q; ++k)
            if (k < q) {
                float tau = H.taus[k];
                float err = yt - yh[k];
                loss += fmaxf((tau - 1.0f) * err, tau * err);
                float g = err > 0.0f ? -tau : (err < 0.0f ? 1.0f - tau : 0.5f - tau);
                dy[k] = g * H.inv_count;
            }
        loss *= H.inv_count;
        if (H.nc_weight > 0.0f && q > 1) {
            float inv_rows = H.inv_count * (float)q;
            float pen = 0.0f;
#pragma unroll
            for (int k = 0; k < STDADK_MAX_Q - 1; ++k)
                if (k + 1 < q) {
                    float d = yh[k] - yh[k + 1];
                    if (d > 0.0f) {
                        float gd = (H.nc_power == 2 ? 2.0f * d : 1.0f) * H.nc_weight * inv_rows;
                        pen += (H.nc_power == 2 ? d * d : d);
                        dy[k] += gd;
                        dy[k + 1] -= gd;
                    }
                }
            loss += pen * H.nc_weight * inv_rows;
        }
    }
    return loss;
}

__device__ __forceinline__ void pf_bias_stats(float (&v)[32], const float* sb, int nv, bool& have, float& K, float& S1,
                                              float& S2) {
#pragma unroll
    for (int c = 0; c < 8; ++c) {
        const float4 b = *reinterpret_cast<const float4*>(sb + 4 * c);
        const float2 lo = add2(make_float2(v[4 * c], v[4 * c + 1]), make_float2(b.x, b.y));
        const float2 hi = add2(make_float2(v[4 * c + 2], v[4 * c + 3]), make_float2(b.z, b.w));
        v[4 * c] = lo.x; v[4 * c + 1] = lo.y; v[4 * c + 2] = hi.x; v[4 * c + 3] = hi.y;
    }
    if (!have) {
        K = v[0];
        have = true;
    }
    if (nv >= 32) {
        const float2 nk = make_float2(-K, -K);
        float2 a1[2] = {make_float2(0.f, 0.f), make_float2(0.f, 0.f)}, a2[2] = {make_float2(0.f, 0.f), make_float2(0.f, 0.f)};
#pragma unroll
        for (int i = 0; i < 32; i += 2) {
            const float2 d = add2(make_float2(v[i], v[i + 1]), nk);
            a1[(i >> 1) & 1] = add2(a1[(i >> 1) & 1], d);
            a2[(i >> 1) & 1] = fma2(d, d, a2[(i >> 1) & 1]);
        }
        S1 += (a1[0].x + a1[0].y) + (a1[1].x + a1[1].y);
        S2 += (a2[0].x + a2[0].y) + (a2[1].x + a2[1].y);
    } else {
#pragma unroll
        for (int i = 0; i < 32; ++i)
            if (i < nv) {
                const float d = v[i] - K;
                S1 += d;
                S2 = fmaf(d, d, S2);
            }
    }
}

__device__ __forceinline__ void pf_normalize(float (&v)[32], const float* sg, const float* sbt, bool has_ln, float rstd,
                                             float nmr, int nv) {
    if (has_ln) {
        const float2 r2 = make_float2(rstd, rstd), n2 = make_float2(nmr, nmr);
#pragma unroll
        for (int c = 0; c < 8; ++c) {
            const float4 g = *reinterpret_cast<const float4*>(sg + 4 * c);
            const float4 b = *reinterpret_cast<const float4*>(sbt + 4 * c);
            const float2 y0 = fma2(fma2(make_float2(v[4 * c], v[4 * c + 1]), r2, n2), make_float2(g.x, g.y),
                                   make_float2(b.x, b.y));
            const float2 y1 = fma2(fma2(make_float2(v[4 * c + 2], v[4 * c + 3]), r2, n2), make_float2(g.z, g.w),
                                   make_float2(b.z, b.w));
            v[4 * c] = fmaxf(y0.x, 0.0f);
            v[4 * c + 1] = fmaxf(y0.y, 0.0f);
            v[4 * c + 2] = fmaxf(y1.x, 0.0f);
            v[4 * c + 3] = fmaxf(y1.y, 0.0f);
        }
    } else {
#pragma unroll
        for (int i = 0; i < 32; ++i) v[i] = fmaxf(v[i], 0.0f);
    }
    if (nv < 32) {
#pragma unroll
        for (int i = 0; i < 32; ++i)
            if (i >= nv) v[i] = 0.0f;
    }
}

__device__ __forceinline__ uint32_t pf_keep_mask(unsigned long long seed, uint32_t step, uint32_t layer,
                                                 unsigned long long key_row, int c0, uint32_t thresh16) {
    uint32_t keep = 0;
#pragma unroll 1
    for (int b = 0; b < 4; ++b) keep |= dropout_keep8(seed, step, layer, key_row, (uint32_t)(c0 / 8 + b), thresh16) << (8 * b);
    return keep;
}
__device__ __forceinline__ void pf_dropout(float (&v)[32], uint32_t keep, float scale) {
#pragma unroll
    for (int i = 0; i < 32; ++i) v[i] = ((keep >> i) & 1u) ? v[i] * scale : 0.0f;
}
__device__ __forceinline__ void pf_head_partial(const float (&v)[32], const float* shw, int n_pad, int c0, int q,
                                                float (&yh)[STDADK_MAX_Q]) {
#pragma unroll 1
    for (int k = 0; k < q; ++k) {
        const float* wk = shw + k * n_pad + c0;
        float a0 = 0.0f, a1 = 0.0f, a2 = 0.0f, a3 = 0.0f;
#pragma unroll
        for (int c = 0; c < 8; ++c) {
            const float4 w = *reinterpret_cast<const float4*>(wk + 4 * c);
            a0 = fmaf(v[4 * c], w.x, a0);
            a1 = fmaf(v[4 * c + 1], w.y, a1);
            a2 = fmaf(v[4 * c + 2], w.z, a2);
            a3 = fmaf(v[4 * c + 3], w.w, a3);
        }
        const float acc = (a0 + a1) + (a2 + a3);
#pragma unroll
        for (int kk = 0; kk < STDADK_MAX_Q; ++kk)
            if (kk == k) yh[kk] += acc;
    }
}

struct EpiCtx {
    const float* sbias;
    const float* sgam;
    const float* sbet;
    const float* shw;
    const float* shb;
    float* red;
    uint32_t trow;
    int tile, row, irow, cg, lane;
    long long lrow, grow;
    bool rvalid, tile_valid;
};
template <int CG, int TM>
__device__ __forceinline__ void fwd_epilogue(const FwdK& P, const EpiCtx& E) {
    using G = TileGeo<TM>;
    constexpr int NW = n_work(CG), NG = G::groups(CG), WSTEP = G::WARP_COLS * CG;
    const float* sbias = E.sbias;
    const float* sgam = E.sgam;
    const float* sbet = E.sbet;
    const float* shw = E.shw;
    const float* shb = E.shb;
    float* red = E.red;
    const uint32_t trow = E.trow;
    const int tile = E.tile, row = E.row, irow = E.irow, cg = E.cg, lane = E.lane;
    const long long lrow = E.lrow, grow = E.grow;
    const bool rvalid = E.rvalid, tile_valid = E.tile_valid;
    const int n_pad = P.n_pad, n_out = P.L.n_out;
    const bool has_ln = P.L.gamma != nullptr;
    const int coff = G::chunk_off(lane), grp = G::group(cg, lane);
    float* myred = red + ((size_t)grp * TM + row) * RED_STRIDE;
    const float* arow = (P.addend && rvalid) ? P.addend + (size_t)lrow * n_out : nullptr;
    float v[32];
    float mean = 0.0f, rstd = 1.0f;
    if (has_ln) {
        float K = 0.0f, S1 = 0.0f, S2 = 0.0f, cntv = 0.0f;
        bool have = false;
        for (int wc = G::WARP_COLS * cg; wc < n_pad; wc += WSTEP) {
            const int c0 = wc + coff, nv = n_out - c0;
            if ((TM == 128 ? nv : n_out - wc) <= 0) break;
            acc_ld<TM>(trow + wc, v);
            if (TM == 128 || nv > 0) {
                if (arow) add_addend_chunk(v, arow, c0, n_out);
                pf_bias_stats(v, sbias + c0, min(nv, 32), have, K, S1, S2);
                cntv += (float)min(nv, 32);
            }
        }
        const float inv_n = 1.0f / (float)n_out;
        if (NG > 1) {
            *reinterpret_cast<float4*>(myred) = make_float4(K, S1, S2, cntv);
            worker_barrier(NW);
            float4 part[NG];
            float tot = 0.0f;
#pragma unroll
            for (int g = 0; g < NG; ++g) {
                part[g] = *reinterpret_cast<const float4*>(red + ((size_t)g * TM + row) * RED_STRIDE);
                tot += fmaf(part[g].w, part[g].x, part[g].y);
            }
            mean = tot * inv_n;
            float m2 = 0.0f;
#pragma unroll
            for (int g = 0; g < NG; ++g) {
                float dk = mean - part[g].x;
                m2 += part[g].z - 2.0f * dk * part[g].y + part[g].w * dk * dk;
            }
            rstd = 1.0f / sqrtf(fmaxf(m2 * inv_n, 0.0f) + P.L.eps);
        } else {
            float m1 = S1 * inv_n;
            mean = K + m1;
            rstd = 1.0f / sqrtf(fmaxf(S2 * inv_n - m1 * m1, 0.0f) + P.L.eps);
        }
        if (P.stats && rvalid && grp == 0) {
            P.stats[2 * lrow] = mean;
            P.stats[2 * lrow + 1] = rstd;
        }
    }
    const float nmr = -mean * rstd;
    float yh[STDADK_MAX_Q];
#pragma unroll
    for (int k = 0; k < STDADK_MAX_Q; ++k) yh[k] = 0.0f;
    const bool drop = P.L.drop_p > 0.0f;
    const unsigned int drop_step = drop ? dropout_step(P.L) : 0u;
    for (int wc = G::WARP_COLS * cg; wc < n_pad; wc += WSTEP) {
        const int c0 = wc + coff;
        const bool cvalid = TM == 128 || c0 < n_pad;
        uint32_t keep = 0xFFFFFFFFu;
        if (drop && cvalid)
            keep = pf_keep_mask(P.L.seed, drop_step, (uint32_t)P.L.layer_id, P.L.key_offset + (unsigned long long)lrow, c0,
                                P.thresh16);
        acc_ld<TM>(trow + wc, v);
        if (arow) add_addend_chunk(v, arow, c0, n_out);
#pragma unroll
        for (int c = 0; c < 8; ++c) {
            const float4 b = *reinterpret_cast<const float4*>(sbias + c0 + 4 * c);
            const float2 lo = add2(make_float2(v[4 * c], v[4 * c + 1]), make_float2(b.x, b.y));
            const float2 hi = add2(make_float2(v[4 * c + 2], v[4 * c + 3]), make_float2(b.z, b.w));
            v[4 * c] = lo.x; v[4 * c + 1] = lo.y; v[4 * c + 2] = hi.x; v[4 * c + 3] = hi.y;
        }
        if (P.x_img && tile_valid && cvalid)
            image_store_chunk(P.x_img, tile, n_pad / SLAB_K, c0, (uint32_t)irow, v);
        const int nv = rvalid ? min(32, max(n_out - c0, 0)) : 0;
        pf_normalize(v, sgam + c0, sbet + c0, has_ln, rstd, nmr, nv);
        if (drop) pf_dropout(v, keep, P.drop_scale);
        if (P.has_head && cvalid) pf_head_partial(v, shw, n_pad, c0, P.head.q, yh);
        if (P.out_img && tile_valid && cvalid)
            store_operand_chunk(P.out_img, P.out_img_lo, tile, n_pad / SLAB_K, c0, (uint32_t)irow, v);
    }
    if (P.has_head) {
        if (NG > 1) {
#pragma unroll
            for (int k = 0; k < STDADK_MAX_Q; ++k)
                if (k < P.head.q) myred[4 + k] = yh[k];
            worker_barrier(NW);
        }
        if (cg == 0) {
            float loss = 0.0f;
            if (rvalid && grp == 0) {
                float dy[STDADK_MAX_Q];
#pragma unroll
                for (int k = 0; k < STDADK_MAX_Q; ++k)
                    if (k < P.head.q) {
                        if (NG > 1) {
                            float acc = 0.0f;
#pragma unroll
                            for (int g = 0; g < NG; ++g) acc += red[((size_t)g * TM + row) * RED_STRIDE + 4 + k];
                            yh[k] = acc;
                        }
                        yh[k] += shb[k];
// ... 84 lines not shown
    tc_fence_after();
    const uint32_t tmem_base = *tmem_slot;
    FWD_T(0);

    if (warp == 4 * CG) {
        if (lane == 0) {
            const size_t a_off = (size_t)itile * P.k_slabs * SLAB_FLOATS + (size_t)irow0 * SLAB_K;
            const int n_virt = P.k_slabs * P.passes;
            const int n_pre = BASIS ? 0 : min(n_virt, NSTAGE);
            for (int v = 0; v < n_pre; ++v) {
                const int s = v / P.passes, p = v - s * P.passes;
                issue_slab_copies(pass_b_lo(p) ? P.L.w_img_lo : P.L.w_img, P.k_slabs, s, n_pad,
                                  (pass_a_lo(p) ? P.a_img_lo : P.a_img) + a_off, sA + (size_t)v * SLAB_FLOATS,
                                  sB + v * b_stage_floats, &full[v], TM * 128u, true);
            }
            pdl_wait();
            pdl_launch_dependents();
            for (int v = 0; v < n_pre; ++v) {
                const int s = v / P.passes, p = v - s * P.passes;
                issue_a_slab(s, (pass_a_lo(p) ? P.a_img_lo : P.a_img) + a_off, sA + (size_t)v * SLAB_FLOATS, &full[v],
                             TM * 128u);
            }
            for (int v = n_pre; v < n_virt; ++v) {
                const int s = v / P.passes, p = v - s * P.passes;
                int stage = v % NSTAGE, it = v / NSTAGE;
                if (it > 0) FWD_WAIT(7, mbar_wait(&empty[stage], (it - 1) & 1));
                const float* w_src = pass_b_lo(p) ? P.L.w_img_lo : P.L.w_img;
                const float* a_tile = BASIS ? nullptr : (pass_a_lo(p) ? P.a_img_lo : P.a_img) + a_off;
                issue_slab_copies(w_src, P.k_slabs, s, n_pad, a_tile, sA + (size_t)stage * SLAB_FLOATS,
                                  sB + stage * b_stage_floats, &full[stage], TM * 128u);
            }
        }
        __syncwarp();
    } else if (warp == 4 * CG + 1) {
        if (lane == 0) {
            const uint32_t idesc = umma_idesc_tf32((uint32_t)n_pad, 0, 0, TM);
            const int n_virt = P.k_slabs * P.passes;
            for (int s = 0; s < n_virt; ++s) {
                int stage = s % NSTAGE, it = s / NSTAGE;
                FWD_WAIT(6, mbar_wait(&full[stage], it & 1));
                tc_fence_after();
                issue_slab_mma(tmem_base, sA + (size_t)stage * SLAB_FLOATS, sB + stage * b_stage_floats, idesc,
                               s == 0);
                umma_commit(&empty[stage]);
            }
            umma_commit(accf);
        }
        __syncwarp();
    } else {
        pdl_wait();
        const int q4 = warp & 3, cg = warp >> 2;
        const int row = G::row(q4, lane), grp = G::group(cg, lane);
        const long long lrow = (long long)tile * TM + row;
        const bool rvalid = tile_valid && lrow < P.pts.n_rows;
        const long long grow = P.pts.row_begin + lrow;
        if (BASIS) {
            float x = 0.f, y = 0.f, t = 0.f;
            const float* xrow = nullptr;
            if (rvalid) {
                load_point(P.pts, grow, x, y, t);
                if (P.basis.p_cov > 0 && P.pts.xcov) xrow = P.pts.xcov + sample_of(P.pts, grow) * P.basis.p_cov;
            }
            auto gen_all = [&](auto fn_tag) {
                constexpr int FN = decltype(fn_tag)::value;
                int stage = 0, it = 0;
                for (int s = 0; s < P.k_slabs; ++s) {
                    float* gslab = (P.feat_img && tile_valid)
                                       ? P.feat_img + ((size_t)itile * P.k_slabs + s) * SLAB_FLOATS + (size_t)irow0 * SLAB_K
                                       : nullptr;
                    for (int p = 0; p < P.passes; ++p) {
                        if (it > 0) {
                            if (tid == 0) FWD_WAIT(5, mbar_wait(&empty[stage], (it - 1) & 1));
                            else mbar_wait(&empty[stage], (it - 1) & 1);
                        }
                        const uint32_t sa = smem_u32(sA + (size_t)stage * SLAB_FLOATS);
                        if (pass_a_lo(p))
                            gen_basis_slab_soa<FN, true, 2>(P.basis, ctab, s, x, y, t, xrow, sa, (uint32_t)row, grp * (8 / NG),
                                                         (grp + 1) * (8 / NG), nullptr);
                        else
                            gen_basis_slab_soa<FN, false, 2>(P.basis, ctab, s, x, y, t, xrow, sa, (uint32_t)row, grp * (8 / NG),
                                                          (grp + 1) * (8 / NG), p == 0 ? gslab : nullptr);
                        fence_proxy_async_smem();
                        mbar_arrive_warp(&full[stage]);
                        if (++stage == NSTAGE) { stage = 0; ++it; }
                    }
                }
            };
            if (P.basis.fn == STDADK_WENDLAND) gen_all(std::integral_constant<int, STDADK_WENDLAND>{});
            else if (P.basis.fn == STDADK_TRIANGULAR) gen_all(std::integral_constant<int, STDADK_TRIANGULAR>{});
            else gen_all(std::integral_constant<int, STDADK_GAUSSIAN>{});
        }
        FWD_T(1);
        mbar_wait(accf, 0);
        tc_fence_after();
        FWD_T(2);
        EpiCtx E{sbias, sgam, sbet, shw, shb, red, tmem_base + ((uint32_t)(q4 * 32) << 16), itile, row, irow0 + row, cg, lane,
                 lrow, grow, rvalid, tile_valid};
        fwd_epilogue<CG, TM>(P, E);
        tc_fence_before();
        FWD_T(3);
    }
    __syncthreads();
    if (warp == 4 * CG) tmem_dealloc(tmem_base, (uint32_t)P.tmem_cols);
    FWD_T(4);
}

__device__ __forceinline__ void head_dh_chunk(float (&g)[32], const float (&dyh)[STDADK_MAX_Q], const float* shw, int n_pad,
                                              int c0, int q) {
#pragma unroll
    for (int i = 0; i < 32; ++i) g[i] = 0.0f;
#pragma unroll 1
    for (int k = 0; k < q; ++k) {
        float dk = 0.0f;
#pragma unroll
        for (int kk = 0; kk < STDADK_MAX_Q; ++kk)
            if (kk == k) dk = dyh[kk];
        const float* wk = shw + k * n_pad + c0;
#pragma unroll
        for (int i = 0; i < 32; ++i) g[i] = fmaf(dk, wk[i], g[i]);
    }
}

template <bool BASIS, int TM, int CG, int NS, bool LN, bool HEAD>
__global__ void __launch_bounds__(n_threads(CG), 1) layer_bwd_kernel(const __grid_constant__ BwdK P) {
    using G = TileGeo<TM>;
    constexpr int NW = n_work(CG), NT = n_threads(CG), NSTAGE = NS, NG = G::groups(CG);
    constexpr int WSTEP = G::WARP_COLS * CG;
    constexpr int MAXCH = MAX_N / WSTEP;
    extern __shared__ uint8_t smem_raw[];
    uint8_t* smem = align_smem(smem_raw);
    const int q = HEAD ? P.head.q : 0;
    const SmemPlan sp = plan_smem(P.n_pad, q, BASIS ? P.basis.k_s : 0, BASIS ? P.basis.k_t : 0, true, CG, NS,
                                  BASIS ? P.k_slabs * 8 : 0);
    float* sA = reinterpret_cast<float*>(smem + sp.a_off);
    float* sB = reinterpret_cast<float*>(smem + sp.b_off);
    uint64_t* full = reinterpret_cast<uint64_t*>(smem + sp.bar_off);
    uint64_t* empty = full + NSTAGE;
    uint64_t* accf = full + 2 * NSTAGE;
    uint32_t* tmem_slot = reinterpret_cast<uint32_t*>(smem + sp.tmem_off);
    float* sbias = reinterpret_cast<float*>(smem + sp.vec_off);
    float* sgam = sbias + P.n_pad;
    float* sbet = sgam + P.n_pad;
    float* shw = reinterpret_cast<float*>(smem + sp.headw_off);
    float4* ctab = reinterpret_cast<float4*>(smem + sp.knots_off);
    float* cs_bias = reinterpret_cast<float*>(smem + sp.colsum_off);
    float* cs_gam = cs_bias + P.n_pad;
    float* cs_bet = cs_gam + P.n_pad;
    float* cs_hw = cs_bet + P.n_pad;
    float* cs_hb = cs_hw + q * P.n_pad;
    float* red = reinterpret_cast<float*>(smem + sp.red_off);

    const int tid = threadIdx.x, warp = tid >> 5, lane = tid & 31;
    const int tile = blockIdx.x;
    const int itile = tile / (TILE_M / TM), irow0 = (tile % (TILE_M / TM)) * TM;
    const int n_pad = P.n_pad, n_out = P.L.n_out;
    constexpr bool has_ln = LN;
    const size_t b_stage_floats = (size_t)n_pad * SLAB_K;
    const int virt1 = P.k_slabs * P.passes;
    const int total_slabs = virt1 + P.k_slabs2 * P.passes;
    const uint32_t acc1_off = (uint32_t)(P.tmem_cols / 2);

    if (tid == NW) {
        for (int s = 0; s < NSTAGE; ++s) {
            mbar_init(&full[s], BASIS ? 1 + NW / 32 : 1);
            mbar_init(&empty[s], 1);
        }
        mbar_init(accf, 1);
        mbar_fence_init();
    }
    if (warp == 4 * CG) {
        __syncwarp();
        tmem_alloc(tmem_slot, (uint32_t)P.tmem_cols);
    }
    if (BASIS) build_chunk_tables(P.basis, ctab, P.k_slabs * 8, tid, NT);
    for (int i = tid; i < n_pad; i += NT) {
        bool ok = i < n_out;
        sbias[i] = ok ? P.L.bias[i] : 0.0f;
        sgam[i] = (ok && has_ln) ? P.L.gamma[i] : 1.0f;
        sbet[i] = (ok && has_ln) ? P.L.beta[i] : 0.0f;
    }
    for (int i = tid; i < (3 + q) * n_pad + STDADK_MAX_Q; i += NT) cs_bias[i] = 0.0f;
    if (HEAD) {
        for (int i = tid; i < q * n_pad; i += NT) {
            int k = i / n_pad, c = i - k * n_pad;
            shw[i] = c < n_out ? P.head.w[(size_t)k * n_out + c] : 0.0f;
        }
    }
    tc_fence_before();
    __syncthreads();
    tc_fence_after();
    const uint32_t tmem_base = *tmem_slot;

    if (warp == 4 * CG) {
        if (lane == 0) {
            const size_t a_off = (size_t)itile * P.k_slabs * SLAB_FLOATS + (size_t)irow0 * SLAB_K;
            const size_t dzn_off = (size_t)itile * P.k_slabs2 * SLAB_FLOATS + (size_t)irow0 * SLAB_K;
            const int n_pre = min(total_slabs, NSTAGE);
            auto wait_then_dz_next = [&]() {
                pdl_wait();
                pdl_launch_dependents();
                for (int v = virt1; v < n_pre; ++v) {
                    const int s = (v - virt1) / P.passes, p = (v - virt1) - s * P.passes;
                    issue_a_slab(s, (pass_a_lo(p) ? P.dz_next_img_lo : P.dz_next_img) + dzn_off,
                                 sA + (size_t)v * SLAB_FLOATS, &full[v], TM * 128u);
                }
            };
            for (int v = 0; v < total_slabs; ++v) {
                if (v == n_pre) wait_then_dz_next();
                int stage = v % NSTAGE, it = v / NSTAGE;
                if (it > 0) mbar_wait(&empty[stage], (it - 1) & 1);
                float* a_dst = sA + (size_t)stage * SLAB_FLOATS;
                float* b_dst = sB + stage * b_stage_floats;
                if (v < virt1) {
                    const int s = v / P.passes, p = v - s * P.passes;
                    const float* a_tile = BASIS ? nullptr : (pass_a_lo(p) ? P.a_img_lo : P.a_img) + a_off;
                    issue_slab_copies(pass_b_lo(p) ? P.L.w_img_lo : P.L.w_img, P.k_slabs, s, n_pad, a_tile, a_dst, b_dst,
                                      &full[stage], TM * 128u);
                } else {
                    const int s = (v - virt1) / P.passes, p = (v - virt1) - s * P.passes;
                    issue_slab_copies(pass_b_lo(p) ? P.wt_next_img_lo : P.wt_next_img, P.k_slabs2, s, n_pad,
                                      (pass_a_lo(p) ? P.dz_next_img_lo : P.dz_next_img) + dzn_off, a_dst, b_dst, &full[stage],
                                      TM * 128u, v < n_pre);
                }
            }
            if (total_slabs == n_pre) wait_then_dz_next();
        }
        __syncwarp();
    } else if (warp == 4 * CG + 1) {
        if (lane == 0) {
            const uint32_t idesc = umma_idesc_tf32((uint32_t)n_pad, 0, 0, TM);
            for (int s = 0; s < total_slabs; ++s) {
                int stage = s % NSTAGE, it = s / NSTAGE;
                mbar_wait(&full[stage], it & 1);
                tc_fence_after();
                bool second = s >= virt1;
                issue_slab_mma(tmem_base + (second ? acc1_off : 0u), sA + (size_t)stage * SLAB_FLOATS,
                               sB + stage * b_stage_floats, idesc, s == 0 || s == virt1);
                umma_commit(&empty[stage]);
            }
            umma_commit(accf);
        }
        __syncwarp();
    } else {
        const int q4 = warp & 3, cg = warp >> 2;
        const int row = G::row(q4, lane), irow = irow0 + row, grp = G::group(cg, lane), coff = G::chunk_off(lane);
        const int c_begin = grp * (8 / NG), c_end = (grp + 1) * (8 / NG);
        const long long lrow = (long long)tile * TM + row;
        const bool rvalid = lrow < P.pts.n_rows;
        const long long grow = P.pts.row_begin + lrow;
        if (BASIS) {
            float x = 0.f, y = 0.f, t = 0.f;
            const float* xrow = nullptr;
            if (rvalid) {
                load_point(P.pts, grow, x, y, t);
                if (P.basis.p_cov > 0 && P.pts.xcov) xrow = P.pts.xcov + sample_of(P.pts, grow) * P.basis.p_cov;
            }
            auto gen_all = [&](auto fn_tag) {
                constexpr int FN = decltype(fn_tag)::value;
                for (int v = 0; v < total_slabs; ++v) {
                    int stage = v % NSTAGE, it = v / NSTAGE;
                    if (it > 0) mbar_wait(&empty[stage], (it - 1) & 1);
                    if (v < virt1) {
                        const int s = v / P.passes, p = v - s * P.passes;
                        const uint32_t sa = smem_u32(sA + (size_t)stage * SLAB_FLOATS);
                        if (pass_a_lo(p))
                            gen_basis_slab_soa<FN, true, 2>(P.basis, ctab, s, x, y, t, xrow, sa, (uint32_t)row, c_begin,
                                                            c_end, nullptr);
                        else
                            gen_basis_slab_soa<FN, false, 2>(P.basis, ctab, s, x, y, t, xrow, sa, (uint32_t)row, c_begin,
                                                             c_end, nullptr);
                        fence_proxy_async_smem();
                    }
                    mbar_arrive_warp(&full[stage]);
                }
            };
            if (P.basis.fn == STDADK_WENDLAND) gen_all(std::integral_constant<int, STDADK_WENDLAND>{});
            else if (P.basis.fn == STDADK_TRIANGULAR) gen_all(std::integral_constant<int, STDADK_TRIANGULAR>{});
            else gen_all(std::integral_constant<int, STDADK_GAUSSIAN>{});
        }
        pdl_wait();
        mbar_wait(accf, 0);
        tc_fence_after();
        const uint32_t trow = tmem_base + ((uint32_t)(q4 * 32) << 16);
        float* myred = red + ((size_t)grp * TM + row) * RED_STRIDE;
        const float* arow = (P.addend && rvalid) ? P.addend + (size_t)lrow * n_out : nullptr;
        float mean = 0.0f, rstd = 1.0f;
        if (has_ln && rvalid) {
            mean = P.stats[2 * lrow];
            rstd = P.stats[2 * lrow + 1];
        }
        float dyh[STDADK_MAX_Q];
#pragma unroll
        for (int k = 0; k < STDADK_MAX_Q; ++k)
            dyh[k] = (HEAD && rvalid && k < q) ? P.head.dyhat[lrow * q + k] : 0.0f;
        const bool drop = P.L.drop_p > 0.0f;
        const unsigned int drop_step = drop ? dropout_step(P.L) : 0u;
        const float inv_n = 1.0f / (float)n_out;
        uint32_t actbits[MAXCH];
        float Sa = 0.0f, Sb = 0.0f;
        float z[32], g[32], tmp[32];

        int ch = 0;
        for (int wc = G::WARP_COLS * cg; wc < n_pad; wc += WSTEP, ++ch) {
            const int c0 = wc + coff;
            const bool cvalid = TM == 128 || c0 < n_pad;
            if (P.x_img) {
                if (cvalid) image_load_chunk(P.x_img, itile, n_pad / SLAB_K, c0, (uint32_t)irow, z);
            } else {
                acc_ld<TM>(trow + wc, z);
                if (arow) add_addend_chunk(z, arow, c0, n_out);
#pragma unroll
                for (int i = 0; i < 32; ++i) z[i] += sbias[c0 + i];
            }
            if (!cvalid)
#pragma unroll
                for (int i = 0; i < 32; ++i) z[i] = 0.0f;
            if (!HEAD) acc_ld<TM>(trow + acc1_off + wc, g);
            else head_dh_chunk(g, dyh, shw, n_pad, c0, cvalid ? q : 0);
            uint32_t keep = 0xFFFFFFFFu;
            if (drop && cvalid) {
                keep = 0;
#pragma unroll 1
                for (int b = 0; b < 4; ++b)
                    keep |= dropout_keep8(P.L.seed, drop_step, (uint32_t)P.L.layer_id, P.L.key_offset + (unsigned long long)lrow,
                                          (uint32_t)(c0 / 8 + b), P.thresh16)
                            << (8 * b);
            }
            uint32_t act = 0;
#pragma unroll
            for (int i = 0; i < 32; ++i) {
                const int col = c0 + i;
                float x = z[i];
                float xh = has_ln ? (x - mean) * rstd : x;
                float yv = has_ln ? fmaf(xh, sgam[col], sbet[col]) : x;
                bool on = (yv > 0.0f) && ((keep >> i) & 1u) && (col < n_out) && rvalid;
                act |= (on ? 1u : 0u) << i;
                const float dh = g[i];
                float h = on ? yv * P.drop_scale : 0.0f;
                g[i] = on ? dh * P.drop_scale : 0.0f;
                z[i] = xh;
                tmp[i] = h;
            }
#pragma unroll
            for (int k = 0; k < MAXCH; ++k)
                if (k == ch) actbits[k] = act;
            if (HEAD) {
                for (int k = 0; k < q; ++k) {
                    float hv[32];
                    const float dk = dyh[k];
#pragma unroll
                    for (int i = 0; i < 32; ++i) hv[i] = dk * tmp[i];
                    colsum_chunk<TM>(cs_hw + k * n_pad, c0, cvalid, hv, lane);
                }
            }
            if (has_ln) {
#pragma unroll
                for (int i = 0; i < 32; ++i) {
                    float gy = g[i] * sgam[c0 + i];
                    Sa += gy;
                    Sb = fmaf(gy, z[i], Sb);
                    tmp[i] = g[i] * z[i];
                }
                colsum_chunk<TM>(cs_gam, c0, cvalid, tmp, lane);
#pragma unroll
                for (int i = 0; i < 32; ++i) tmp[i] = g[i];
                colsum_chunk<TM>(cs_bet, c0, cvalid, tmp, lane);
            } else {
                if (cvalid) store_operand_chunk(P.dz_img, P.dz_img_lo, itile, n_pad / SLAB_K, c0, (uint32_t)irow, g);
                colsum_chunk<TM>(cs_bias, c0, cvalid, g, lane);
            }
        }
        if (HEAD && cg == 0) {
            for (int k = 0; k < q; ++k) {
                float s = warp_sum(TM == 128 || lane < 16 ? dyh[k] : 0.0f);
                if (lane == 0) atomicAdd(&cs_hb[k], s);
            }
        }
        if (has_ln) {
            if (NG > 1) {
                myred[0] = Sa;
                myred[1] = Sb;
                worker_barrier(NW);
                Sa = Sb = 0.0f;
#pragma unroll
                for (int gq = 0; gq < NG; ++gq) {
                    Sa += red[((size_t)gq * TM + row) * RED_STRIDE];
                    Sb += red[((size_t)gq * TM + row) * RED_STRIDE + 1];
                }
            }
            const float ma = Sa * inv_n, mb = Sb * inv_n;
            ch = 0;
            for (int wc = G::WARP_COLS * cg; wc < n_pad; wc += WSTEP, ++ch) {
                const int c0 = wc + coff;
                const bool cvalid = TM == 128 || c0 < n_pad;
                if (P.x_img) {
                    if (cvalid) image_load_chunk(P.x_img, itile, n_pad / SLAB_K, c0, (uint32_t)irow, z);
                } else {
                    acc_ld<TM>(trow + wc, z);
                    if (arow) add_addend_chunk(z, arow, c0, n_out);
#pragma unroll
                    for (int i = 0; i < 32; ++i) z[i] += sbias[c0 + i];
                }
                if (!cvalid)
#pragma unroll
                    for (int i = 0; i < 32; ++i) z[i] = 0.0f;
                if (!HEAD) acc_ld<TM>(trow + acc1_off + wc, g);
                else head_dh_chunk(g, dyh, shw, n_pad, c0, cvalid ? q : 0);
                uint32_t act = 0;
#pragma unroll
                for (int k = 0; k < MAXCH; ++k)
                    if (k == ch) act = actbits[k];
#pragma unroll
                for (int i = 0; i < 32; ++i) {
                    const int col = c0 + i;
                    float xh = (z[i] - mean) * rstd;
                    const float dh = g[i];
                    float gy = ((act >> i) & 1u) ? dh * P.drop_scale * sgam[col] : 0.0f;
                    float dz = rstd * (gy - ma - xh * mb);
                    g[i] = (col < n_out && rvalid) ? dz : 0.0f;
                }
                if (cvalid) store_operand_chunk(P.dz_img, P.dz_img_lo, itile, n_pad / SLAB_K, c0, (uint32_t)irow, g);
                colsum_chunk<TM>(cs_bias, c0, cvalid, g, lane);
            }
        }
        tc_fence_before();
        worker_barrier(NW);
        for (int c = tid; c < n_out; c += NW) {
            atomicAdd(&P.d_bias[c], cs_bias[c]);
            if (has_ln) {
                atomicAdd(&P.d_gamma[c], cs_gam[c]);
                atomicAdd(&P.d_beta[c], cs_bet[c]);
            }
            for (int k = 0; k < q; ++k) atomicAdd(&P.d_head_w[(size_t)k * n_out + c], cs_hw[k * n_pad + c]);
        }
        if (tid < q) atomicAdd(&P.d_head_b[tid], cs_hb[tid]);
    }
    __syncthreads();
    if (warp == 4 * CG) tmem_dealloc(tmem_base, (uint32_t)P.tmem_cols);
}

struct WgradK {
    BasisP basis;
    PointsP pts;
    const float* a_img;
    const float* a_img_lo;
    const float* dz_img;
    const float* dz_img_lo;
    float* dw;
    long long stride_o, stride_i;
    int n_in, n_out, a_slabs, dz_slabs, n_row_tiles, nt_slabs, tmem_cols, passes;
};
constexpr int WG_HALF_ROWS = 64;
constexpr int WG_CHUNK_BYTES = WG_HALF_ROWS * 128;
constexpr int WG_A_BYTES = 4 * WG_CHUNK_BYTES;
constexpr int WG_B_BYTES = 8 * WG_CHUNK_BYTES;
constexpr int WG_STAGE_BYTES = WG_A_BYTES + WG_B_BYTES;

__host__ __device__ inline uint32_t wgrad_smem_bytes(int k_s, int k_t) {
    return WG_NSTAGE * WG_STAGE_BYTES + 64 + 16 + 16 + (uint32_t)k_s * 16u + (uint32_t)k_t * 8u + 16 + 1024;
}
__device__ __forceinline__ uint32_t swz32_off(uint32_t row, uint32_t c16) {
    return row * 128u + ((((c16 >> 1) ^ (row & 3u)) << 5) | ((c16 & 1u) << 4));
}
__device__ __forceinline__ uint64_t umma_desc_sw128_32b(uint32_t saddr, uint32_t lbo_bytes, uint32_t sbo_bytes) {
    return (uint64_t)((saddr & 0x3FFFFu) >> 4) | ((uint64_t)((lbo_bytes >> 4) & 0x3FFFu) << 16) |
           ((uint64_t)((sbo_bytes >> 4) & 0x3FFFu) << 32) | (1ull << 46) | (1ull << 61);
}
template <int NW>
__device__ __forceinline__ void restage_half_tiles(const float* dz_tile, int mslab0, int m_chunks, const float* a_tile,
                                                   int nslab0, int n_chunks, int half, uint32_t sa, uint32_t sb, int tid) {
    constexpr int BD = 2048 / NW, BA = 4096 / NW;
    static_assert(NW * BD == 2048 && NW * BA == 4096, "worker count must divide the half-tile unit counts");
    const int units_d = m_chunks * 512, units_a = a_tile ? n_chunks * 512 : 0;
    const size_t hoff = (size_t)half * WG_HALF_ROWS * SLAB_K;
    float4 vd[BD], va[BA];
#pragma unroll
    for (int j = 0; j < BD; ++j) {
        const int u = tid + j * NW;
        if (u < units_d)
            vd[j] = __ldg(reinterpret_cast<const float4*>(dz_tile + (size_t)(mslab0 + (u >> 9)) * SLAB_FLOATS + hoff) + (u & 511));
    }
#pragma unroll
    for (int j = 0; j < BA; ++j) {
        const int u = tid + j * NW;
        if (u < units_a)
            va[j] = __ldg(reinterpret_cast<const float4*>(a_tile + (size_t)(nslab0 + (u >> 9)) * SLAB_FLOATS + hoff) + (u & 511));
    }
#pragma unroll
    for (int j = 0; j < BD; ++j) {
        const int u = tid + j * NW;
        if (u < units_d) {
            const int c = u >> 9, w = u & 511;
            const uint32_t r = (uint32_t)(w >> 3), lc = (uint32_t)(w & 7) ^ (r & 7u);
            st_shared_v4(sa + c * WG_CHUNK_BYTES + swz32_off(r, lc), vd[j].x, vd[j].y, vd[j].z, vd[j].w);
        }
    }
#pragma unroll
    for (int j = 0; j < BA; ++j) {
        const int u = tid + j * NW;
        if (u < units_a) {
            const int c = u >> 9, w = u & 511;
            const uint32_t r = (uint32_t)(w >> 3), lc = (uint32_t)(w & 7) ^ (r & 7u);
            st_shared_v4(sb + c * WG_CHUNK_BYTES + swz32_off(r, lc), va[j].x, va[j].y, va[j].z, va[j].w);
        }
    }
}

template <int NW>
__device__ __noinline__ void wgrad_gen_basis_half(const WgradK& P, const float4* sk, const float2* st, int rt, int half,
                                                  int pass, uint32_t sb, int row64, int par, int n_chunks) {
    float x = 0.f, y = 0.f, t = 0.f;
    const float* xrow = nullptr;
    long long lrow = (long long)rt * TILE_M + half * WG_HALF_ROWS + row64;
    if (lrow < P.pts.n_rows) {
        long long grow = P.pts.row_begin + lrow;
        load_point(P.pts, grow, x, y, t);
        if (P.basis.p_cov > 0 && P.pts.xcov) xrow = P.pts.xcov + sample_of(P.pts, grow) * P.basis.p_cov;
    }
    const int ni = blockIdx.z;
    for (int c = par; c < n_chunks; c += NW / 64) {
        const int slab = ni * P.nt_slabs + c;
#pragma unroll 1
        for (int c16 = 0; c16 < 8; ++c16) {
            float4 v = feature_chunk(P.basis, sk, st, slab * SLAB_K + c16 * 4, x, y, t, xrow, pass_b_lo(pass));
            st_shared_v4(sb + c * WG_CHUNK_BYTES + swz32_off((uint32_t)row64, (uint32_t)c16), v.x, v.y, v.z, v.w);
        }
    }
}

template <bool BASIS, int CG>
__global__ void __launch_bounds__(n_threads(CG), 1) wgrad_kernel(const __grid_constant__ WgradK P) {
    constexpr int NW = n_work(CG), NT = n_threads(CG);
    extern __shared__ uint8_t smem_raw[];
    uint8_t* smem = align_smem(smem_raw);
    uint8_t* stage_base = smem;
    uint64_t* full = reinterpret_cast<uint64_t*>(smem + WG_NSTAGE * WG_STAGE_BYTES);
    uint64_t* empty = full + WG_NSTAGE;
    uint64_t* accf = full + 2 * WG_NSTAGE;
    uint64_t* kbar = accf + 1;
    uint32_t* tmem_slot = reinterpret_cast<uint32_t*>(smem + WG_NSTAGE * WG_STAGE_BYTES + 64);
    float4* sk = reinterpret_cast<float4*>(smem + WG_NSTAGE * WG_STAGE_BYTES + 96);
    float2* st = reinterpret_cast<float2*>(reinterpret_cast<uint8_t*>(sk) + (size_t)(BASIS ? P.basis.k_s : 0) * 16);

    const int tid = threadIdx.x, warp = tid >> 5, lane = tid & 31;
    const int split = blockIdx.x, n_split = gridDim.x, mi = blockIdx.y, ni = blockIdx.z;
    const int m_chunks = min(4, P.dz_slabs - mi * 4);
    const int n_chunks = min(P.nt_slabs, P.a_slabs - ni * P.nt_slabs);
    const int n_mma = n_chunks * SLAB_K;
    int my_tiles = 0;
    for (int rt = split; rt < P.n_row_tiles; rt += n_split) ++my_tiles;
    const int n_iter = my_tiles * 2 * P.passes;

    if (tid == NW) {
        for (int s = 0; s < WG_NSTAGE; ++s) {
            mbar_init(&full[s], NW / 32);
            mbar_init(&empty[s], 1);
        }
        mbar_init(accf, 1);
        mbar_init(kbar, 1);
        mbar_fence_init();
        if (BASIS) stage_knots_async(P.basis, sk, st, kbar);
    }
    if (warp == 4 * CG) {
        __syncwarp();
        tmem_alloc(tmem_slot, (uint32_t)P.tmem_cols);
    }
    if (m_chunks < 4) {
        for (int s = 0; s < WG_NSTAGE; ++s) {
            float4* zp = reinterpret_cast<float4*>(stage_base + s * WG_STAGE_BYTES + m_chunks * WG_CHUNK_BYTES);
            int n16 = (4 - m_chunks) * WG_CHUNK_BYTES / 16;
            for (int i = tid; i < n16; i += NT) zp[i] = make_float4(0.f, 0.f, 0.f, 0.f);
        }
        fence_proxy_async_smem();
    }
    tc_fence_before();
    __syncthreads();
    tc_fence_after();
    const uint32_t tmem_base = *tmem_slot;

    if (n_iter > 0) {
        if (warp == 4 * CG + 1) {
            if (lane == 0) {
                const uint32_t idesc = umma_idesc_tf32((uint32_t)n_mma, 1, 1);
                for (int itn = 0; itn < n_iter; ++itn) {
                    int stage = itn % WG_NSTAGE, it = itn / WG_NSTAGE;
                    mbar_wait(&full[stage], it & 1);
                    tc_fence_after();
                    uint32_t sa = smem_u32(stage_base + stage * WG_STAGE_BYTES);
// ... 199 lines not shown
```

### st_dadk_b200/csrc/misc.cuh

```cuda
#pragma once
#include "common.cuh"

namespace stdadk {

__global__ void pack_image_kernel(const float* __restrict__ src, long long row_stride, long long col_stride,
                                  long long rows, long long cols, float* __restrict__ img, long long n_chunks,
                                  int slabs) {
    for (long long idx = blockIdx.x * (long long)blockDim.x + threadIdx.x; idx < n_chunks;
         idx += (long long)gridDim.x * blockDim.x) {
        int chunk = (int)(idx & 7);
        int row = (int)((idx >> 3) & 127);
        long long ts = idx >> 10;
        int slab = (int)(ts % slabs);
        long long tile = ts / slabs;
        long long r = tile * TILE_M + row;
        float v[4];
#pragma unroll
        for (int e = 0; e < 4; ++e) {
            long long c = (long long)slab * SLAB_K + chunk * 4 + e;
            v[e] = (r < rows && c < cols) ? to_tf32(src[r * row_stride + c * col_stride]) : 0.0f;
        }
        float* dst = img + ts * SLAB_FLOATS;
        *reinterpret_cast<float4*>(reinterpret_cast<uint8_t*>(dst) + swz_off((uint32_t)row, (uint32_t)chunk)) =
            make_float4(v[0], v[1], v[2], v[3]);
// ... 198 lines not shown
    return make_float2(__uint_as_float(q.x), __uint_as_float(q.z));
}
constexpr int PEER_THREADS = 256;
__device__ __forceinline__ void peer_two_phase(const PeerK& P, unsigned int epoch, long long par_off, long long i0,
                                               long long stride) {
    float2* g2 = reinterpret_cast<float2*>(P.g);
    const long long m = (P.n2 + P.world - 1) / P.world;
    const long long own_lo = (long long)P.rank * m, own_hi = min(P.n2, own_lo + m);
    const uint4* mine = P.recv[P.rank];
    for (long long i = i0; i < P.n2; i += stride) {
        if (i >= own_lo && i < own_hi) continue;
        const int owner = (int)(i / m);
        const float2 v = g2[i];
        uint4* dst = nullptr;
#pragma unroll
        for (int p = 0; p < PEER_MAX; ++p)
            if (p == owner) dst = P.recv[p];
        st_sys_v4(dst + (par_off + P.rank) * P.n2 + i, make_uint4(__float_as_uint(v.x), epoch, __float_as_uint(v.y), epoch));
    }
    for (long long i = i0; i < P.n2; i += stride) {
        if (i < own_lo || i >= own_hi) continue;
        const float2 own = g2[i];
        float2 sum = make_float2(0.0f, 0.0f);
#pragma unroll
        for (int s = 0; s < PEER_MAX; ++s)
            if (s < P.world) {
                const float2 v = s == P.rank ? own : peer_wait_packet(mine + (par_off + s) * P.n2 + i, epoch);
                sum.x += v.x;
                sum.y += v.y;
            }
        g2[i] = sum;
        const uint4 pkt = make_uint4(__float_as_uint(sum.x), epoch, __float_as_uint(sum.y), epoch);
#pragma unroll
        for (int p = 0; p < PEER_MAX; ++p)
            if (p < P.world && p != P.rank) st_sys_v4(P.recv[p] + (par_off + P.rank) * P.n2 + i, pkt);
    }
    for (long long i = i0; i < P.n2; i += stride) {
        if (i >= own_lo && i < own_hi) continue;
        const int owner = (int)(i / m);
        g2[i] = peer_wait_packet(mine + (par_off + owner) * P.n2 + i, epoch);
    }
}
__global__ void __launch_bounds__(PEER_THREADS) peer_allreduce_kernel(const __grid_constant__ PeerK P) {
    const unsigned int epoch = (unsigned int)(*P.step_count) + 1u;
    const long long par_off = (long long)(epoch & 1u) * P.world;
    const long long stride = (long long)gridDim.x * blockDim.x;
    const long long i0 = blockIdx.x * (long long)blockDim.x + threadIdx.x;
    float2* g2 = reinterpret_cast<float2*>(P.g);
    float acc[8];
#pragma unroll
    for (int k = 0; k < 8; ++k) acc[k] = 0.0f;
    if (P.two_phase) {
        peer_two_phase(P, epoch, par_off, i0, stride);
        if (P.G.n == 0) return;
        for (long long i = i0; i < P.n2; i += stride) {
            const float2 sum = g2[i];
            const long long e = i << 1;
            const float vv[2] = {sum.x, sum.y};
#pragma unroll
            for (int j = 0; j < 2; ++j)
                if (e + j < P.n_norm) {
                    const int gi = group_of(P.G, e + j);
#pragma unroll
                    for (int k = 0; k < 8; ++k)
                        if (k == gi) acc[k] = fmaf(vv[j], vv[j], acc[k]);
                }
        }
    } else {
    for (long long i = i0; i < P.n2; i += stride) {
        const float2 v = g2[i];
        const uint4 pkt = make_uint4(__float_as_uint(v.x), epoch, __float_as_uint(v.y), epoch);
#pragma unroll
        for (int p = 0; p < PEER_MAX; ++p)
            if (p < P.world && p != P.rank) st_sys_v4(P.recv[p] + (par_off + P.rank) * P.n2 + i, pkt);
    }
    const uint4* mine = P.recv[P.rank];
    for (long long i = i0; i < P.n2; i += stride) {
        const float2 own = g2[i];
        float2 sum = make_float2(0.0f, 0.0f);
#pragma unroll
        for (int s = 0; s < PEER_MAX; ++s)
            if (s < P.world) {
                float2 v = own;
                if (s != P.rank) v = peer_wait_packet(mine + (par_off + s) * P.n2 + i, epoch);
                sum.x += v.x;
                sum.y += v.y;
            }
        g2[i] = sum;
        if (P.G.n > 0) {
            const long long e = i << 1;
            const float vv[2] = {sum.x, sum.y};
#pragma unroll
            for (int j = 0; j < 2; ++j)
                if (e + j < P.n_norm) {
                    const int gi = group_of(P.G, e + j);
#pragma unroll
                    for (int k = 0; k < 8; ++k)
                        if (k == gi) acc[k] = fmaf(vv[j], vv[j], acc[k]);
                }
        }
    }
    }
    if (P.G.n == 0) return;
    __shared__ float wsum[PEER_THREADS / 32][8];
    __shared__ bool last;
    const int warp = threadIdx.x >> 5, lane = threadIdx.x & 31;
#pragma unroll
    for (int k = 0; k < 8; ++k) {
        float s = warp_sum(acc[k]);
        if (lane == 0) wsum[warp][k] = s;
    }
    __syncthreads();
    if (threadIdx.x < 8) {
        float s = 0.0f;
        for (int w = 0; w < PEER_THREADS / 32; ++w) s += wsum[w][threadIdx.x];
        P.ws[blockIdx.x * 8 + threadIdx.x] = s;
    }
    __threadfence();
    __syncthreads();
    if (threadIdx.x == 0) {
        unsigned int* ticket = reinterpret_cast<unsigned int*>(P.ws + gridDim.x * 8);
        unsigned int t = atomicAdd(ticket, 1u);
        last = (t == gridDim.x - 1);
        if (last) *ticket = 0u;
    }
    __syncthreads();
    if (last && threadIdx.x < P.G.n) {
        __threadfence();
        float s = 0.0f;
        for (unsigned int b = 0; b < gridDim.x; ++b) s += P.ws[b * 8 + threadIdx.x];
        P.sq_out[threadIdx.x] = s;
    }
}

struct AdamK {
    float* p;
    const float* g;
    float* m;
    float* v;
    float* shadow;
    long long n;
    GroupsP G;
    const float* hyper;
    const float* sqnorms;
    const int* step_count;
    float beta1, beta2, eps, ema_decay;
    float* g_zero;
    float* loss_acc;
    float* loss_sum;
    float* loss_last;
    float* sq_out;
    float* norm_ws;
    int* step_rw;
};
template <bool FUSED>
__global__ void __launch_bounds__(256) adamw_ema_kernel(AdamK A) {
    __shared__ float s_sq[8];
    int step;
    if (FUSED) {
        pdl_wait();
        step = *A.step_count + 1;
        float acc[8];
#pragma unroll
        for (int k = 0; k < 8; ++k) acc[k] = 0.0f;
        if (A.sqnorms) {
            const long long n4q = A.n >> 2;
            const float4* gq = reinterpret_cast<const float4*>(A.g);
            for (long long i = blockIdx.x * (long long)blockDim.x + threadIdx.x; i < n4q; i += (long long)gridDim.x * blockDim.x) {
                const float4 v = __ldg(gq + i);
                const long long e = i << 2;
                const float vv[4] = {v.x, v.y, v.z, v.w};
#pragma unroll
                for (int j = 0; j < 4; ++j) {
                    const int gi = group_of(A.G, e + j);
#pragma unroll
                    for (int k = 0; k < 8; ++k)
                        if (k == gi) acc[k] = fmaf(vv[j], vv[j], acc[k]);
                }
            }
            if (blockIdx.x == 0 && threadIdx.x < (A.n & 3)) {
                const long long i = (n4q << 2) + threadIdx.x;
                const float v = A.g[i];
                const int gi = group_of(A.G, i);
#pragma unroll
                for (int k = 0; k < 8; ++k)
                    if (k == gi) acc[k] = fmaf(v, v, acc[k]);
            }
        }
        __shared__ float wsum[8][8];
        const int warp = threadIdx.x >> 5, lane = threadIdx.x & 31;
#pragma unroll
        for (int k = 0; k < 8; ++k) {
            const float sk = warp_sum(acc[k]);
            if (lane == 0) wsum[warp][k] = sk;
        }
        __syncthreads();
        if (threadIdx.x < 8) {
            float sk = 0.0f;
            for (int w = 0; w < 8; ++w) sk += wsum[w][threadIdx.x];
            A.norm_ws[blockIdx.x * 8 + threadIdx.x] = sk;
        }
        __threadfence();
        __syncthreads();
        if (threadIdx.x == 0) {
            unsigned int* cnt = reinterpret_cast<unsigned int*>(A.norm_ws + gridDim.x * 8);
            volatile unsigned int* gen = cnt + 1;
            const unsigned int my_gen = *gen;
            if (atomicAdd(cnt, 1u) == gridDim.x - 1) {
                *cnt = 0u;
                __threadfence();
                atomicAdd(const_cast<unsigned int*>(gen), 1u);
            } else {
                long long t0 = clock64();
                while (*gen == my_gen) {
                    if (clock64() - t0 > 4000000000LL) __trap();
                }
            }
            __threadfence();
        }
        __syncthreads();
        if (threadIdx.x < 8) {
            float sk = 0.0f;
            for (unsigned int b = 0; b < gridDim.x; ++b) sk += __ldcg(&A.norm_ws[b * 8 + threadIdx.x]);
            s_sq[threadIdx.x] = sk;
            if (blockIdx.x == 0 && A.sq_out && threadIdx.x < A.G.n) A.sq_out[threadIdx.x] = sk;
        }
        if (blockIdx.x == 0 && threadIdx.x == 0) *A.step_rw = step;
        __syncthreads();
    } else {
        step = *A.step_count;
    }
    const float bc1 = 1.0f - powf(A.beta1, (float)step);
    const float bc2 = 1.0f - powf(A.beta2, (float)step);
    const float inv_sqrt_bc2 = 1.0f / sqrtf(bc2);
    float lr[8], wd[8], clip[8];
#pragma unroll
    for (int k = 0; k < 8; ++k) {
        lr[k] = wd[k] = 0.0f;
        clip[k] = 1.0f;
        if (k < A.G.n) {
            lr[k] = A.hyper[4 * k];
            wd[k] = A.hyper[4 * k + 1];
            float mx = A.hyper[4 * k + 2];
            if (A.sqnorms && mx > 0.0f) clip[k] = fminf(1.0f, mx / (sqrtf(FUSED ? s_sq[k] : A.sqnorms[k]) + 1e-6f));
        }
    }
    auto update = [&](long long i, float g, float& p, float& m, float& v, float& sh) {
        int gi = group_of(A.G, i);
        float l = lr[0], w = wd[0], c = clip[0];
#pragma unroll
        for (int k = 1; k < 8; ++k)
            if (k == gi) { l = lr[k]; w = wd[k]; c = clip[k]; }
        g *= c;
        p *= (1.0f - l * w);
        m = A.beta1 * m + (1.0f - A.beta1) * g;
        v = A.beta2 * v + (1.0f - A.beta2) * g * g;
        float denom = sqrtf(v) * inv_sqrt_bc2 + A.eps;
        p -= (l / bc1) * (m / denom);
        sh = A.ema_decay * sh + (1.0f - A.ema_decay) * p;
    };
    const long long n4 = A.n >> 2;
    const float4* g4 = reinterpret_cast<const float4*>(A.g);
    float4* p4 = reinterpret_cast<float4*>(A.p);
    float4* m4 = reinterpret_cast<float4*>(A.m);
    float4* v4 = reinterpret_cast<float4*>(A.v);
    float4* s4 = reinterpret_cast<float4*>(A.shadow);
    for (long long i = blockIdx.x * (long long)blockDim.x + threadIdx.x; i < n4;
         i += (long long)gridDim.x * blockDim.x) {
        float4 g = __ldg(g4 + i), p = p4[i], m = m4[i], v = v4[i];
        float4 sh = s4 ? s4[i] : make_float4(0.f, 0.f, 0.f, 0.f);
        const long long e = i << 2;
        update(e, g.x, p.x, m.x, v.x, sh.x);
        update(e + 1, g.y, p.y, m.y, v.y, sh.y);
        update(e + 2, g.z, p.z, m.z, v.z, sh.z);
        update(e + 3, g.w, p.w, m.w, v.w, sh.w);
        p4[i] = p;
        m4[i] = m;
        v4[i] = v;
        if (s4) s4[i] = sh;
        if (A.g_zero) reinterpret_cast<float4*>(A.g_zero)[i] = make_float4(0.f, 0.f, 0.f, 0.f);
    }
    if (blockIdx.x == 0 && threadIdx.x == 0 && A.loss_acc && A.loss_sum) {
        const float step_loss = *A.loss_acc;
        *A.loss_sum += step_loss;
        if (A.loss_last) *A.loss_last = step_loss;
        *A.loss_acc = 0.0f;
    }
    if (blockIdx.x == 0 && threadIdx.x < (A.n & 3)) {
        long long i = (n4 << 2) + threadIdx.x;
        float p = A.p[i], m = A.m[i], v = A.v[i], sh = A.shadow ? A.shadow[i] : 0.0f;
        update(i, A.g[i], p, m, v, sh);
        A.p[i] = p;
        A.m[i] = m;
        A.v[i] = v;
        if (A.shadow) A.shadow[i] = sh;
        if (A.g_zero) A.g_zero[i] = 0.0f;
    }
}

}
```

### st_dadk_b200/executor.py

```python
from __future__ import annotations

import ctypes as C
from dataclasses import dataclass
from typing import Dict, List, Optional, Sequence, Tuple

import torch

from . import _lib as L
from . import ops


@dataclass
class NetSpec:
    centers: torch.Tensor
    bandwidths: Optional[torch.Tensor]
    log_bandwidths: Optional[torch.Tensor]
    t_centers: torch.Tensor
    t_bandwidths: torch.Tensor
    weights: List[torch.Tensor]
    biases: List[torch.Tensor]
    gammas: List[Optional[torch.Tensor]]
    betas: List[Optional[torch.Tensor]]
    head_w: torch.Tensor
    head_b: torch.Tensor
    basis_fn: str = "wendland"
    p_cov: int = 0
    dropout: float = 0.0
    ln_eps: float = 1e-5
    learnable_basis: bool = False
    lattice_sides: Optional[List[int]] = None
    level_sizes: Optional[List[int]] = None
    precision: str = "tf32"

    @property
    def n_hidden(self):
        return len(self.weights)

    @property
    def q(self):
        return self.head_w.shape[0]


@dataclass
class LossSpec:
    kind: str = "mse"
    taus: Sequence[float] = ()
    nc_weight: float = 0.0
    nc_power: int = 1


class _Workspace:
    def __init__(self, spec: NetSpec, n_rows: int, device, sparse: bool = False, save_x: bool = False,
                 save_feat: bool = False):
        self.n_rows = n_rows
        self.feat = ops.new_image(n_rows, spec.weights[0].shape[1], device) if save_feat else None
        self.zs = torch.empty(n_rows, spec.weights[0].shape[0], dtype=torch.float32, device=device) if sparse else None
        self.h = [ops.new_image(n_rows, w.shape[0], device) for w in spec.weights[:-1]]
        self.dz = [ops.new_image(n_rows, w.shape[0], device) for w in spec.weights]
        x3 = spec.precision == "tf32x3"
        self.h_lo = [ops.new_image(n_rows, w.shape[0], device) for w in spec.weights[:-1]] if x3 else None
        self.dz_lo = [ops.new_image(n_rows, w.shape[0], device) for w in spec.weights] if x3 else None
        self.stats = [torch.empty(n_rows, 2, dtype=torch.float32, device=device) if g is not None else None
                      for g in spec.gammas]
        self.x = [ops.new_image(n_rows, w.shape[0], device) for w in spec.weights] if save_x else None
        self.yhat = torch.empty(n_rows, spec.q, dtype=torch.float32, device=device)
        self.dyhat = torch.empty(n_rows, spec.q, dtype=torch.float32, device=device)


class Executor:
    MAX_WORKSPACES = 4
    DENSE_MAX_KNOTS = 2048
    SAVE_X_MAX_ROWS = 148 * 2 * 128
    SAVE_FEAT_MIN_ROWS = SAVE_X_MAX_ROWS + 1
    store_basis_operand = False

    def __init__(self, spec: NetSpec, force_sparse: bool = False, force_dense: bool = False):
        self.spec = spec
        self.force_sparse = force_sparse
        self.force_dense = force_dense
        self._setup_regime(spec)
        dev = spec.centers.device
        if dev.type != "cuda":
            raise RuntimeError("st_dadk_b200.Executor needs CUDA tensors: the hot path has no CPU implementation")
        self.device = dev
        self._ws: Dict[int, _Workspace] = {}
        self.on_evict = None
        self._ctx = None
        self._pack_key = None
        self.w_img: List[torch.Tensor] = [None] * spec.n_hidden
        self.wt_img: List[torch.Tensor] = [None] * spec.n_hidden
        self.w1s_img = None
        self.w_img_lo: List[torch.Tensor] = [None] * spec.n_hidden
        self.wt_img_lo: List[torch.Tensor] = [None] * spec.n_hidden
        self.w1s_img_lo = None
        self.knots4 = torch.empty(max(spec.centers.shape[0], 1), 4, dtype=torch.float32, device=dev)
        self.tknots2 = torch.empty(max(spec.t_centers.shape[0], 1), 2, dtype=torch.float32, device=dev)
        self.loss_acc = torch.zeros(1, dtype=torch.float32, device=dev)
        self._grad_flat = None
        self.grads = None
        self._knots_ready = False
        self._side = None
        self.fused_predict = True
        self._fused_ok = None
        self._field_ok = None
        self._cell_ws = None
        self._w1sf_img = None
        self._w1sf_key = None
        self._zt_ws = None

    @property
    def x3(self) -> bool:
        return self.spec.precision == "tf32x3"

    def _setup_regime(self, spec: NetSpec):
        if spec.precision not in ("tf32", "tf32x3"):
            raise ValueError(f"precision must be 'tf32' or 'tf32x3', got {spec.precision!r}")
        k_s, k_t = spec.centers.shape[0], spec.t_centers.shape[0]
        n_out = spec.weights[0].shape[0]
        q_head = spec.q if spec.n_hidden == 1 else 0
        fits, why = ops.dense_basis_supported(spec.p_cov, k_s, k_t, n_out, q_head)
        too_big = ""
        self.predict_only = None
        if not fits:
            limit = ops.dense_max_knots(spec.p_cov, k_t, n_out, q_head)
            too_big = (f"the dense path holds at most {limit} spatial knots with a first block of {n_out} outputs "
                       f"and {k_t} temporal knots ({why})")
            if self.force_dense:
                fwd_fits, fwd_why = ops.dense_basis_supported(spec.p_cov, k_s, k_t, n_out, q_head, training=False)
                if not fwd_fits:
                    fwd_limit = ops.dense_max_knots(spec.p_cov, k_t, n_out, q_head, training=False)
                    raise RuntimeError(f"force_dense: {k_s} spatial knots do not fit: the dense forward holds at most "
                                       f"{fwd_limit} spatial knots with a first block of {n_out} outputs and {k_t} "
                                       f"temporal knots ({fwd_why})")
                self.predict_only = f"force_dense: {k_s} spatial knots can be predicted but not trained: {too_big}"
        want = self.force_sparse or (not self.force_dense and (k_s > self.DENSE_MAX_KNOTS or not fits))
        self.sparse = False
        self.lat = None
        self.level_begin = None
        if not want:
            return
        problems = []
        if spec.basis_fn == "gaussian":
            problems.append("the gaussian basis is not compactly supported")
        if spec.p_cov != 0:
            problems.append("covariates are not supported together with the support walk")
        if spec.weights[0].shape[0] % 4:
            problems.append("first hidden width must be a multiple of 4")
        sizes = [int(v) for v in (spec.level_sizes or [k_s])]
        if sum(sizes) != k_s or len(sizes) > 8:
            problems.append("level_sizes must be at most 8 contiguous ranges adding up to the number of knots")
        if problems:
            if self.force_sparse or not fits:
                reason = f" ({too_big})" if too_big else ""
                raise RuntimeError(f"{k_s} spatial knots need the support-walking path{reason}, but " + "; ".join(problems))
            return
        if spec.lattice_sides is not None and not spec.learnable_basis:
            sides = [int(v) for v in spec.lattice_sides]
            offs, o = [], 0
            for sd in sides:
                offs.append(o)
                o += sd * sd
            assert o == k_s, "lattice_sides do not add up to the number of knots"
            bw = spec.bandwidths[torch.tensor(offs, device=spec.bandwidths.device)].float().cpu().numpy()
            import numpy as _np
            calib = _np.float32(L.CALIBRATION[spec.basis_fn])
            self.lat = (sides, offs, [float(_np.float32(b) * calib) for b in bw])
        else:
            self.level_begin = [0]
            for n in sizes:
                self.level_begin.append(self.level_begin[-1] + n)
        self.sparse = True

    def rebind(self, spec: NetSpec):
        if spec.precision != self.spec.precision:
            self._ws.clear()
            if self.on_evict is not None:
                self.on_evict()
        self.spec = spec
        self._setup_regime(spec)
        self._pack_key = None
        self._knots_ready = False
        self._fused_ok = None
        self._field_ok = None
        self._w1sf_key = None

    def _key(self):
        s = self.spec
        ts = [s.centers, s.bandwidths, s.log_bandwidths, *s.weights]
        return tuple((t.data_ptr(), t._version) for t in ts if t is not None)

    def prepare(self, force: bool = True, for_backward: bool = False):
        s = self.spec
        key = (self._key(), for_backward)
        if not force and key == self._pack_key:
            return
        if s.learnable_basis or not self._knots_ready:
            ops.knots_prepare(s.centers, s.bandwidths if s.log_bandwidths is None else None, s.log_bandwidths,
                              s.basis_fn, out=self.knots4)
            ops.tknots_prepare(s.t_centers, s.t_bandwidths, out=self.tknots2)
            if self.sparse and self.level_begin is not None:
                self._cell_ws = ops.celllist_build(self.knots4, self.level_begin, self._cell_ws)
            self._knots_ready = True
        srcs, outs, slots, parts = [], [], [], []
        x3 = self.x3

        def add(src, kind, l):
            store = {"w": self.w_img, "wt": self.wt_img, "w1s": None}[kind]
            srcs.append(src); outs.append(store[l] if store is not None else self.w1s_img)
            slots.append((kind, l, 0)); parts.append(0)
            if x3:
                store = {"w": self.w_img_lo, "wt": self.wt_img_lo, "w1s": None}[kind]
                srcs.append(src); outs.append(store[l] if store is not None else self.w1s_img_lo)
                slots.append((kind, l, 1)); parts.append(1)

        for l, w in enumerate(s.weights):
            if l == 0 and self.sparse:
                k_s = s.centers.shape[0]
                add(w[:, k_s:], "w", l)
                wt = w.t()
                self._w1t = wt if wt.is_contiguous() else wt.contiguous()
            else:
                add(w, "w", l)
            if for_backward and l > 0:
                add(w.t(), "wt", l)
        if for_backward and s.learnable_basis and not self.sparse:
            add(s.weights[0][:, s.p_cov:s.p_cov + s.centers.shape[0]].t(), "w1s", 0)
        for (kind, l, part), img in zip(slots, ops.pack_images(srcs, outs, parts)):
            if kind == "w":
                (self.w_img_lo if part else self.w_img)[l] = img
            elif kind == "wt":
                (self.wt_img_lo if part else self.wt_img)[l] = img
            elif part:
                self.w1s_img_lo = img
            else:
                self.w1s_img = img
        self._pack_key = key

    def _workspace(self, n_rows: int) -> _Workspace:
        ws = self._ws.get(n_rows)
        if ws is None:
            if len(self._ws) >= self.MAX_WORKSPACES:
                self._ws.pop(next(iter(self._ws)))
                if self.on_evict is not None:
                    self.on_evict()
            ws = self._ws[n_rows] = _Workspace(self.spec, n_rows, self.device, self.sparse,
                                               save_x=n_rows <= self.SAVE_X_MAX_ROWS,
                                               save_feat=(self.store_basis_operand and not self.sparse and not self.x3
                                                          and n_rows >= self.SAVE_FEAT_MIN_ROWS))
        return ws

    def _basis(self) -> L.Basis:
        s = self.spec
        k_s = 0 if self.sparse else s.centers.shape[0]
        return ops.make_basis(self.knots4, self.tknots2, k_s, s.t_centers.shape[0], s.p_cov, s.basis_fn)

# ... 136 lines not shown
        a.layers[0] = ops.make_layer(self._w1sf_img, s.biases[0], s.gammas[0], s.betas[0], k_s, w1.shape[0], s.ln_eps, 0)
        a.w1 = w1.data_ptr()
        a.w1_row_stride, a.w1_col_stride = w1.stride(0), w1.stride(1)
        a.head = C.pointer(head)
        a.row_base = row_base
        a.out_k_stride = out_k_stride
        a.zt_ws = self._zt_ws.data_ptr()
        return a

    def field_supported(self) -> bool:
        s = self.spec
        if self.sparse or self.x3 or not self.fused_predict or s.p_cov != 0 or s.n_hidden > L.MAX_HIDDEN:
            return False
        if self._field_ok is None:
            probe = torch.empty(1, s.q, dtype=torch.float32, device=self.device)
            self._field_ok = ops.predict_field_supported(self._field_args(None, (1, 1), 1, 1, 0, 1, 0, 1, probe, 0))
        return bool(self._field_ok)

    def predict_field(self, yhat: torch.Tensor, begin: int, end: int, n_sites: int, n_times: int,
                      sites: Optional[torch.Tensor] = None, grid: Optional[Tuple[int, int]] = None) -> int:
        S = n_sites
        k0, k1 = begin // S, (end - 1) // S if end > begin else begin // S
        rects = []
        if end <= begin:
            return 0
        if k0 == k1:
            rects.append((k0, k0 + 1, begin - k0 * S, end - k0 * S))
        else:
            lo = k0
            if begin > k0 * S:
                rects.append((k0, k0 + 1, begin - k0 * S, S))
                lo = k0 + 1
            hi = k1 + 1
            if end < (k1 + 1) * S:
                hi = k1
            if hi > lo:
                rects.append((lo, hi, 0, S))
            if hi == k1:
                rects.append((k1, k1 + 1, 0, end - k1 * S))
        for (ka, kb, sa, sb) in rects:
            ops.predict_field(self._field_args(sites, grid, S, n_times, ka, kb, sa, sb, yhat, begin))
        return 2 * len(rects)

    def predict_field_sites(self, yhat: torch.Tensor, site_begin: int, site_end: int, n_sites: int, n_times: int,
                            sites: Optional[torch.Tensor] = None, grid: Optional[Tuple[int, int]] = None) -> int:
        if site_end <= site_begin:
            return 0
        ops.predict_field(self._field_args(sites, grid, n_sites, n_times, 0, n_times, site_begin, site_end, yhat,
                                           site_begin, site_end - site_begin))
        return 2

    def alloc_grads(self, flat: Optional[torch.Tensor] = None, views: Optional[dict] = None):
        s = self.spec
        if views is not None:
            self._grad_flat, self.grads = flat, views
            return
        shapes = []
        for w in s.weights:
            shapes.append(w.shape[0] * w.shape[1])
        sizes = shapes + [b.numel() for b in s.biases] + \
            [g.numel() if g is not None else 0 for g in s.gammas] * 2 + \
            [s.head_w.numel(), s.head_b.numel(), s.centers.numel(), s.centers.shape[0]]
        flat = torch.zeros(sum(sizes), dtype=torch.float32, device=self.device)
        o = 0
        g = {"weights": [], "biases": [], "gammas": [], "betas": []}
        for w in s.weights:
            n = w.shape[0] * w.shape[1]
            g["weights"].append(flat[o:o + n].view(w.shape[1], w.shape[0]).t())
            o += n
        for b in s.biases:
            g["biases"].append(flat[o:o + b.numel()])
            o += b.numel()
        for name in ("gammas", "betas"):
            for gm in s.gammas:
                n = gm.numel() if gm is not None else 0
                g[name].append(flat[o:o + n] if n else None)
                o += n
        g["head_w"] = flat[o:o + s.head_w.numel()].view_as(s.head_w)
        o += s.head_w.numel()
        g["head_b"] = flat[o:o + s.head_b.numel()]
        o += s.head_b.numel()
        g["centers"] = flat[o:o + s.centers.numel()].view(-1, 2)
        o += s.centers.numel()
        g["log_bandwidths"] = flat[o:o + s.centers.shape[0]]
        self._grad_flat, self.grads = flat, g

    def _wgrad_block(self, l: int, pts, ws, basis, g):
        s = self.spec
        w = s.weights[l]
        gw = g["weights"][l]
        a = L.WgradArgs()
        a.pts = pts
        if l == 0 and ws.feat is None:
            a.basis = C.pointer(basis)
        else:
            a.a_img = (ws.feat if l == 0 else ws.h[l - 1]).data_ptr()
            if self.x3:
                a.a_img_lo = ws.h_lo[l - 1].data_ptr()
        a.dz_img = ws.dz[l].data_ptr()
        if self.x3:
            a.dz_img_lo = ws.dz_lo[l].data_ptr()
        a.n_in, a.n_out = self._n_in(l), w.shape[0]
        if l == 0 and self.sparse:
            k_s = s.centers.shape[0]
            gd = gw[:, k_s:]
            a.dw = gd.data_ptr()
            a.stride_o, a.stride_i = gd.stride(0), gd.stride(1)
            ops.wgrad(a)
            if gw.stride(0) != 1 or gw.stride(1) != w.shape[0]:
                raise RuntimeError("support-walk wgrad needs the first-layer gradient stored (in, out)-contiguous")
            kg = {}
            if s.learnable_basis:
                kg = dict(d_centers=g["centers"], d_log_bw=g["log_bandwidths"], w1t=self._w1t)
            ops.sparse_l1_wgrad(self._sparse_args(pts, ws, dz_img=ws.dz[0], dw1t=gw, **kg))
            return
        a.dw = gw.data_ptr()
        a.stride_o, a.stride_i = gw.stride(0), gw.stride(1)
        ops.wgrad(a)

    def backward(self, dyhat: Optional[torch.Tensor] = None, zero: bool = True) -> dict:
        if self._ctx is None:
            raise RuntimeError("Executor.backward called without a saved forward")
        s = self.spec
        pts, drop, ws = self._ctx
        if self.grads is None:
            self.alloc_grads()
        if zero:
            self._grad_flat.zero_()
        g = self.grads
        if dyhat is not None:
            ws.dyhat.copy_(dyhat)
        basis = self._basis()
        nh = s.n_hidden
        main = torch.cuda.current_stream()
        if self._side is None:
            self._side = torch.cuda.Stream(device=self.device)
        side = self._side
        head = ops.make_head(s.head_w, s.head_b, s.q, ws.yhat, dyhat=ws.dyhat)
        for l in reversed(range(nh)):
            a = L.BwdArgs()
            a.pts = pts
            if l == 0 and ws.feat is None:
                a.basis = C.pointer(basis)
                if self.sparse:
                    a.addend = ws.zs.data_ptr()
            else:
                a.a_img = (ws.feat if l == 0 else ws.h[l - 1]).data_ptr()
                if self.x3:
                    a.a_img_lo = ws.h_lo[l - 1].data_ptr()
            a.layer = self._layer(l)
            a.drop = drop
            if ws.x is not None:
                a.x_img = ws.x[l].data_ptr()
            if ws.stats[l] is not None:
                a.stats = ws.stats[l].data_ptr()
                a.d_gamma = g["gammas"][l].data_ptr()
                a.d_beta = g["betas"][l].data_ptr()
            if l == nh - 1:
                a.head = C.pointer(head)
                a.d_head_w = g["head_w"].data_ptr()
                a.d_head_b = g["head_b"].data_ptr()
            else:
                a.dz_next_img = ws.dz[l + 1].data_ptr()
                a.wt_next_img = self.wt_img[l + 1].data_ptr()
                a.n_next = s.weights[l + 1].shape[0]
                if self.x3:
                    a.dz_next_img_lo = ws.dz_lo[l + 1].data_ptr()
                    a.wt_next_img_lo = self.wt_img_lo[l + 1].data_ptr()
            a.dz_img = ws.dz[l].data_ptr()
            if self.x3:
                a.dz_img_lo = ws.dz_lo[l].data_ptr()
            a.d_bias = g["biases"][l].data_ptr()
            ops.layer_bwd(a)
            if l == 0:
                self._wgrad_block(l, pts, ws, basis, g)
            else:
                side.wait_stream(main)
                with torch.cuda.stream(side):
                    self._wgrad_block(l, pts, ws, basis, g)
        main.wait_stream(side)
        if s.learnable_basis and not self.sparse:
            a = L.KnotGradArgs()
            a.basis = C.pointer(basis)
            a.pts = pts
            a.dz_img = ws.dz[0].data_ptr()
            a.w1s_img = self.w1s_img.data_ptr()
            if self.x3:
                a.dz_img_lo = ws.dz_lo[0].data_ptr()
                a.w1s_img_lo = self.w1s_img_lo.data_ptr()
            a.n_out = s.weights[0].shape[0]
            a.d_centers = g["centers"].data_ptr()
            a.d_log_bw = g["log_bandwidths"].data_ptr()
            ops.knot_grad(a)
        return g
```

### st_dadk_b200/ops.py

```python
from __future__ import annotations

import ctypes as C
from typing import Optional, Sequence

import torch

from . import _lib as L

TILE_M, SLAB_K, SLAB_FLOATS = 128, 32, 4096


def _stream() -> int:
    return torch.cuda.current_stream().cuda_stream


def _ptr(t: Optional[torch.Tensor]):
    if t is None:
        return None
    if not t.is_cuda:
        raise RuntimeError("st_dadk_b200: expected a CUDA tensor (there is no CPU path)")
    return t.data_ptr()


def _f32c(t: torch.Tensor, name: str) -> torch.Tensor:
# ... 36 lines not shown
        descs[i] = L.PackDesc(_ptr(src), src.stride(0), src.stride(1), rows, cols, _ptr(out),
                              int(parts[i]) if parts is not None else 0, 0)
        res.append(out)
    for lo in range(0, len(srcs), 8):
        n = min(8, len(srcs) - lo)
        sub = (L.PackDesc * n)(*descs[lo:lo + n])
        L.check(L.lib().stdadk_pack_images(sub, n, _stream()), "pack_images")
    return res


def unpack_image(img: torch.Tensor, rows: int, cols: int) -> torch.Tensor:
    out = torch.empty(rows, cols, dtype=torch.float32, device=img.device)
    L.check(L.lib().stdadk_unpack_image(_ptr(img), rows, cols, _ptr(out), _stream()), "unpack_image")
    return out


def knots_prepare(centers: torch.Tensor, bandwidths: Optional[torch.Tensor], log_bandwidths: Optional[torch.Tensor],
                  basis_fn: str, out: Optional[torch.Tensor] = None) -> torch.Tensor:
    k = centers.shape[0]
    centers = _f32c(centers, "centers")
    bw = _f32c(bandwidths, "bandwidths") if bandwidths is not None else None
    lbw = _f32c(log_bandwidths, "log_bandwidths") if log_bandwidths is not None else None
    if out is None:
        out = torch.empty(max(k, 1), 4, dtype=torch.float32, device=centers.device)
    L.check(L.lib().stdadk_knots_prepare(_ptr(centers), _ptr(bw), _ptr(lbw), L.CALIBRATION[basis_fn], k, _ptr(out),
                                         _stream()), "knots_prepare")
    return out


def tknots_prepare(centers: torch.Tensor, bandwidths: torch.Tensor, out: Optional[torch.Tensor] = None) -> torch.Tensor:
    k = centers.shape[0]
    if out is None:
        out = torch.empty(max(k, 1), 2, dtype=torch.float32, device=centers.device)
    L.check(L.lib().stdadk_tknots_prepare(_ptr(_f32c(centers, "t_centers")), _ptr(_f32c(bandwidths, "t_bandwidths")),
                                          k, _ptr(out), _stream()), "tknots_prepare")
    return out


def make_basis(knots4: torch.Tensor, tknots2: torch.Tensor, k_s: int, k_t: int, p_cov: int, basis_fn: str) -> L.Basis:
    return L.Basis(_ptr(knots4), _ptr(tknots2), k_s, k_t, p_cov, L.BASIS_CODE[basis_fn])


class PointsRef(L.Points):
    _keep = None


def make_points(coords: Optional[torch.Tensor] = None, t: Optional[torch.Tensor] = None,
                xcov: Optional[torch.Tensor] = None, grid: Optional[Sequence[int]] = None, row_begin: int = 0,
                n_rows: Optional[int] = None, index: Optional[torch.Tensor] = None) -> L.Points:
    if grid is not None:
        nx, ny, nt = grid
        if n_rows is None:
            n_rows = nx * ny * nt - row_begin
        return PointsRef(None, None, None, None, nx, ny, nt, 0, row_begin, n_rows)
    if index is not None:
        if index.dtype != torch.int64 or not index.is_cuda or not index.is_contiguous():
            raise RuntimeError("make_points: index must be a contiguous CUDA int64 tensor")
        if n_rows is None:
            n_rows = index.shape[0] - row_begin
    if n_rows is None:
        n_rows = coords.shape[0] - row_begin
    if coords is not None:
        coords, t = _f32c(coords, "coords"), _f32c(t, "t")
    if xcov is not None and xcov.numel() > 0:
        xcov = _f32c(xcov, "X")
    else:
        xcov = None
    pts = PointsRef(_ptr(coords), _ptr(t), _ptr(xcov), _ptr(index), 0, 0, 0, 0, row_begin, n_rows)
    pts._keep = (coords, t, xcov, index)
    return pts


def basis_fwd(basis: L.Basis, pts: L.Points, device) -> tuple:
    n = pts.n_rows
    phi = torch.empty(n, basis.k_s, dtype=torch.float32, device=device)
    psi = torch.empty(n, basis.k_t, dtype=torch.float32, device=device)
    L.check(L.lib().stdadk_basis_fwd(C.byref(basis), C.byref(pts), _ptr(phi), _ptr(psi), _stream()), "basis_fwd")
    return phi, psi


def make_layer(w_img, bias, gamma, beta, n_in, n_out, eps, layer_id, w_img_lo=None) -> L.Layer:
    return L.Layer(_ptr(w_img), _ptr(bias), _ptr(gamma), _ptr(beta), n_in, n_out, eps, layer_id, _ptr(w_img_lo))


def make_head(w, b, q, yhat, loss_type=L.LOSS_NONE, y=None, taus=None, inv_count=0.0, dyhat=None, loss_acc=None,
              nc_weight=0.0, nc_power=1) -> L.Head:
    h = L.Head()
    h.w, h.b, h.q, h.loss_type, h.y = _ptr(w), _ptr(b), q, loss_type, _ptr(y)
    for i, tau in enumerate(taus or []):
        h.taus[i] = float(tau)
    h.inv_count, h.nc_weight, h.nc_power = inv_count, nc_weight, nc_power
    h.yhat, h.dyhat, h.loss_acc = _ptr(yhat), _ptr(dyhat), _ptr(loss_acc)
    return h


def layer_fwd(args: L.FwdArgs):
    L.check(L.lib().stdadk_layer_fwd(C.byref(args), _stream()), "layer_fwd")


def predict_supported(args: L.PredictArgs) -> bool:
    return bool(L.lib().stdadk_predict_supported(C.byref(args)))


def predict(args: L.PredictArgs):
    L.check(L.lib().stdadk_predict(C.byref(args), _stream()), "predict")


def predict_field_supported(args: L.FieldArgs) -> bool:
    return bool(L.lib().stdadk_predict_field_supported(C.byref(args)))


def predict_field(args: L.FieldArgs):
    L.check(L.lib().stdadk_predict_field(C.byref(args), _stream()), "predict_field")


def layer_bwd(args: L.BwdArgs):
    L.check(L.lib().stdadk_layer_bwd(C.byref(args), _stream()), "layer_bwd")


def wgrad(args: L.WgradArgs):
    L.check(L.lib().stdadk_wgrad(C.byref(args), _stream()), "wgrad")


def knot_grad(args: L.KnotGradArgs):
    L.check(L.lib().stdadk_knot_grad(C.byref(args), _stream()), "knot_grad")


def dense_basis_supported(p_cov: int, k_s: int, k_t: int, n_out: int, q_head: int, training: bool = True) -> tuple:
    lib = L.lib()
    if lib.stdadk_dense_basis_supported(p_cov + k_s + k_t, n_out, k_s, k_t, q_head, int(training)):
        return True, ""
    return False, lib.stdadk_last_error().decode("utf-8", "replace")


def dense_max_knots(p_cov: int, k_t: int, n_out: int, q_head: int, training: bool = True) -> int:
    return int(L.lib().stdadk_dense_max_knots(p_cov, k_t, n_out, q_head, int(training)))


_sqnorm_ws = {}


def grad_sqnorm(g: torch.Tensor, group_end: Sequence[int], out: torch.Tensor, workspace: Optional[torch.Tensor] = None):
    if workspace is None:
        workspace = _sqnorm_ws.get(g.device)
        if workspace is None:
            workspace = _sqnorm_ws[g.device] = torch.zeros(L.lib().stdadk_sqnorm_ws_floats(), device=g.device)
    arr = (C.c_int64 * len(group_end))(*group_end)
    L.check(L.lib().stdadk_grad_sqnorm(_ptr(g), g.numel(), len(group_end), arr, _ptr(out), _ptr(workspace), _stream()),
            "grad_sqnorm")


def adamw_ema_step(p, g, m, v, shadow, group_end: Sequence[int], hyper: torch.Tensor, sqnorms, step_count,
                   beta1=0.9, beta2=0.999, eps=1e-8, ema_decay=0.0, zero_grad=False, loss_acc=None, loss_sum=None,
                   loss_last=None, norm_ws=None):
    arr = (C.c_int64 * len(group_end))(*group_end)
    a = L.AdamWArgs(_ptr(p), _ptr(g), _ptr(m), _ptr(v), _ptr(shadow), p.numel(), len(group_end), int(bool(zero_grad)),
                    arr, _ptr(hyper), _ptr(sqnorms), _ptr(step_count), beta1, beta2, eps, ema_decay, _ptr(loss_acc),
                    _ptr(loss_sum), _ptr(loss_last), int(norm_ws is not None), 0, _ptr(norm_ws))
    L.check(L.lib().stdadk_adamw_ema_step(C.byref(a), _stream()), "adamw_ema_step")


def peer_allreduce(args: L.PeerAllreduceArgs):
    L.check(L.lib().stdadk_peer_allreduce(C.byref(args), _stream()), "peer_allreduce")


def make_sparse_args(pts: L.Points, knots4, basis_fn: str, n_out: int, p_cov: int, sides=None, offsets=None,
                     thetaps=None, w1t=None, zs=None, dz_img=None, dw1t=None, celllist=None, n_levels=None,
                     d_centers=None, d_log_bw=None) -> L.SparseArgs:
    a = L.SparseArgs()
    a.pts = pts
    a.knots4 = _ptr(knots4)
    a.basis_fn, a.n_out, a.p_cov = L.BASIS_CODE[basis_fn], n_out, p_cov
    if celllist is not None:
        a.n_levels, a.celllist, a.celllist_k_s = int(n_levels), _ptr(celllist), int(knots4.shape[0])
    else:
        a.n_levels = len(sides)
        for i, (sd, of, th) in enumerate(zip(sides, offsets, thetaps)):
            a.side[i], a.offset[i], a.thetap[i] = int(sd), int(of), float(th)
    a.w1t, a.zs, a.dz_img, a.dw1t = _ptr(w1t), _ptr(zs), _ptr(dz_img), _ptr(dw1t)
    a.d_centers, a.d_log_bw = _ptr(d_centers), _ptr(d_log_bw)
    return a


def celllist_build(knots4: torch.Tensor, level_begin: Sequence[int], ws: Optional[torch.Tensor] = None) -> torch.Tensor:
    k_s, nl = int(knots4.shape[0]), len(level_begin) - 1
    need = L.lib().stdadk_celllist_ws_bytes(k_s, nl)
    if need == 0:
        raise RuntimeError(f"celllist_build: unsupported shape (k_s={k_s}, levels={nl})")
    if ws is None or ws.numel() * 4 < need:
        ws = torch.empty((need + 3) // 4, dtype=torch.int32, device=knots4.device)
    arr = (C.c_int32 * (nl + 1))(*[int(v) for v in level_begin])
    L.check(L.lib().stdadk_celllist_build(_ptr(knots4), k_s, arr, nl, _ptr(ws), ws.numel() * 4, _stream()), "celllist_build")
    return ws


def sparse_l1_fwd(args: L.SparseArgs):
    L.check(L.lib().stdadk_sparse_l1_fwd(C.byref(args), _stream()), "sparse_l1_fwd")


def sparse_l1_wgrad(args: L.SparseArgs):
    L.check(L.lib().stdadk_sparse_l1_wgrad(C.byref(args), _stream()), "sparse_l1_wgrad")
```

### st_dadk_b200/trainer.py

```python
from __future__ import annotations

import math
import os
import warnings
from dataclasses import dataclass
from typing import Dict, List, Optional

import numpy as np
import torch
import torch.distributed as dist

import threading

from . import _lib as L
from . import ops
from .executor import Executor, LossSpec, NetSpec


def _dist_on() -> bool:
    return dist.is_available() and dist.is_initialized() and dist.get_world_size() > 1


_CAPTURE_LOCK = threading.Lock()

# ... 197 lines not shown
            for gq in self.opt.param_groups:
                gq["initial_lr"] = gq["lr"]
        self.batches_per_epoch = max(1, batches_per_epoch)
        self.warmup_epochs = int(c.get("warmup_epochs", 0))
        self.warmup_steps = self.warmup_epochs * self.batches_per_epoch if self.warmup_epochs > 0 else 0
        self.scheduler = None
        if c.get("scheduler") == "cosine":
            self.scheduler = torch.optim.lr_scheduler.CosineAnnealingLR(self.opt, T_max=c.get("epochs", 100),
                                                                        eta_min=self.lr * 0.5)
        self.ema_decay = 1.0 - 1.0 / (10.0 * self.batches_per_epoch)
        self.global_step = 0
        ng = len(self.opt.param_groups)
        self._hyper_ring = [torch.zeros(ng, 4, dtype=torch.float32).pin_memory() for _ in range(self.HYPER_SLOTS)]
        self._hyper_ev = [None] * self.HYPER_SLOTS
        self._hyper_k = 0
        self._hyper_last = None
        self.hyper = torch.zeros(ng, 4, dtype=torch.float32, device=self.device)

    HYPER_SLOTS = 16

    def _hyper_values(self):
        rows = []
        for gq in self.opt.param_groups:
            clip = self.clip * (0.1 if (self.learnable and gq.get("name") == "basis") else 1.0)
            rows.append((float(gq["lr"]), float(self.wd), float(clip)))
        return tuple(rows)

    def _push_hyper(self):
        vals = self._hyper_values()
        if vals == self._hyper_last:
            return
        k = self._hyper_k
        self._hyper_k = (k + 1) % self.HYPER_SLOTS
        if self._hyper_ev[k] is not None:
            self._hyper_ev[k].synchronize()
        slot = self._hyper_ring[k]
        for i, (lr, wd, clip) in enumerate(vals):
            slot[i, 0], slot[i, 1], slot[i, 2] = lr, wd, clip
        self.hyper.copy_(slot, non_blocking=True)
        ev = torch.cuda.Event()
        ev.record(torch.cuda.current_stream())
        self._hyper_ev[k] = ev
        self._hyper_last = vals

    def begin_epoch(self, epoch: int):
        if not (self.learnable and self.unfreeze_epoch > 0):
            return
        for gq in self.opt.param_groups:
            if gq.get("name") != "basis":
                continue
            if epoch == self.unfreeze_epoch:
                gq["lr"] = gq["target_lr"] * (0.1 if self.rampup_epochs > 0 else 1.0)
            elif self.unfreeze_epoch < epoch < self.unfreeze_epoch + self.rampup_epochs:
                gq["lr"] = gq["target_lr"] * (0.1 + 0.9 * (epoch - self.unfreeze_epoch) / self.rampup_epochs)

    def end_epoch(self, epoch: int):
        if self.scheduler is not None and epoch >= self.warmup_epochs:
            with warnings.catch_warnings():
                warnings.simplefilter("ignore")
                self.scheduler.step()

    def _penalty_terms(self):
        c, m = self.cfg, self.model
        terms = []
        if self.learnable:
            w = float(c.get("domain_penalty_weight", 0.0))
            if w > 0:
                terms.append(w * m.compute_domain_penalty())
            w = float(c.get("movement_penalty_weight", 0.0))
            if w > 0:
                terms.append(w * m.compute_movement_penalty())
        stype = c.get("sparsity_penalty_type", "none")
        l1, lg = float(c.get("sparsity_lambda_l1", 0.001)), float(c.get("sparsity_lambda_group", 0.01))
        if stype != "none" and (l1 != 0.0 or lg != 0.0):
            pen = m.compute_sparsity_penalty(penalty_type=stype, lambda_l1=l1, lambda_group=lg)
            if c.get("sparsity_apply_to_spatial", True):
                terms.append(pen["spatial_penalty"])
            if c.get("sparsity_apply_to_temporal", True):
                terms.append(pen["temporal_penalty"])
        if c.get("regression_type") == "multi-quantile" and c.get("use_delta_reparameterization", False):
            lam = float(c.get("non_crossing_lambda", 0.0))
            if lam > 0 and m.delta_params is not None and len(m.delta_params) > 1:
                pnc = 0.0
                for d in list(m.delta_params)[1:]:
                    pnc = pnc + d[0] - torch.max(d[0], torch.clamp(-d[1:], min=0.0).sum())
                terms.append(lam * pnc)
        return terms

    def _add_penalty_grads(self):
        terms = self._penalty_terms()
        if not terms:
            return None
        total = sum(terms)
        params = [p for p in self.model.parameters() if p.requires_grad]
        sb = self.model.spatial_basis
        sb._hook_enabled = False
        try:
            grads = torch.autograd.grad(total, params, allow_unused=True)
        finally:
            sb._hook_enabled = True
        for p, gr in zip(params, grads):
            if gr is not None:
                self.flat.gviews[id(p)].add_(gr)
        return total.detach()

    def _finish_special_grads(self):
        m = self.model
        if m.delta_params is not None:
            dbeta = torch.cat([self.flat.g_head_b[:, None], self.flat.g_head_w], dim=1)
            ddelta = torch.flip(torch.cumsum(torch.flip(dbeta, [0]), dim=0), [0])
            for k, d in enumerate(m.delta_params):
                self.flat.gviews[id(d)].copy_(ddelta[k])

    def _damp_center_grads(self):
        sb = self.model.spatial_basis
        if self.learnable and sb.gradient_damping:
            gv = self.flat.gviews[id(sb.centers)]
            gv.copy_(sb._damping_factor() * gv)

    def _step_compute(self, table, perm, row_begin: int, n_rows: int, global_rows: int, key_offset: int = 0):
        ex, fl = self.ex, self.flat
        if not self._g_clean:
            fl.g.zero_()
            ex.loss_acc.zero_()
        self._g_clean = False
        self._refresh_head()
        ex.prepare(force=True, for_backward=True)
        pts = ops.make_points(table.coords, table.t, table.X, index=perm, row_begin=row_begin, n_rows=n_rows)
        ex.forward(pts, train=True, seed=self.seed, y=table.y, loss=self.loss, inv_count=1.0 / (global_rows * self.q),
                   save=True, prepared=True, step_ptr=self.step_count, key_offset=key_offset)
        ex.backward(zero=False)
        self._finish_special_grads()

    def _step_exchange(self):
        if self.world > 1:
            if self._peer is not None:
                fuse = self._norm_fused()
                self._peer.allreduce(self.flat.g, self.step_count, self.flat.group_end if fuse else None, self.sqnorms)
            else:
                dist.all_reduce(self.flat.g[:self.flat.n_exchange])

    def _norm_fused(self) -> bool:
        return self._peer is not None and self.world > 1 and self.clip > 0 and not self._param_terms_possible

    def _step_update(self):
        ex, fl = self.ex, self.flat
        pen = self._add_penalty_grads()
        self._damp_center_grads()
        fused_tail = not self._norm_fused()
        scratch_tail = fl.n_scratch > 0
        ops.adamw_ema_step(fl.p, fl.g[:fl.n], fl.m, fl.v, fl.shadow, fl.group_end, self.hyper,
                           self.sqnorms if self.clip > 0 else None, self.step_count, ema_decay=self.ema_decay,
                           zero_grad=True, loss_acc=ex.loss_acc, loss_sum=self.loss_sum, loss_last=self.loss_last,
                           norm_ws=self._tail_ws if fused_tail else None)
        if scratch_tail:
            fl.g[fl.n:fl.n + fl.n_scratch].zero_()
        self._g_clean = True
        if pen is not None:
            self.loss_sum += pen

    def _step_body(self, table, perm, row_begin: int, n_rows: int, global_rows: int, key_offset: int = 0):
        self._step_compute(table, perm, row_begin, n_rows, global_rows, key_offset)
        self._step_exchange()
        self._step_update()

    def train_step(self, table, perm: torch.Tensor, row_begin: int, n_rows: int, global_rows: Optional[int] = None,
                   key_offset: Optional[int] = None):
        if global_rows is None:
            global_rows = n_rows
        if key_offset is None:
            key_offset = shard_rows(global_rows, self.rank, self.world)[0] if self.world > 1 else 0
        self._push_hyper()
        if self.use_cuda_graph:
            if self._stage_idx is None or self._stage_idx.shape[0] < n_rows:
                self._stage_idx = torch.zeros(max(n_rows, 1), dtype=torch.int64, device=self.device)
                self._graphs.clear()
            self._stage_idx[:n_rows].copy_(perm[row_begin:row_begin + n_rows])
            gkey = (n_rows, global_rows, table.coords.data_ptr(), table.t.data_ptr(), table.y.data_ptr(),
                    table.X.data_ptr() if table.X is not None else 0, key_offset)
            g = self._graphs.get(gkey)
            if g is None:
                with _CAPTURE_LOCK:
                    self._step_body(table, self._stage_idx, 0, n_rows, global_rows, key_offset)
                    torch.cuda.current_stream().synchronize()
                    mode = dict(capture_error_mode="thread_local")
                    one_graph = self.world == 1 or self._peer is not None
                    if one_graph:
                        g1 = torch.cuda.CUDAGraph()
                        with torch.cuda.graph(g1, **mode):
                            self._step_body(table, self._stage_idx, 0, n_rows, global_rows, key_offset)
                        g = (g1, None)
                    else:
                        g1, g2 = torch.cuda.CUDAGraph(), torch.cuda.CUDAGraph()
                        with torch.cuda.graph(g1, **mode):
                            self._step_compute(table, self._stage_idx, 0, n_rows, global_rows, key_offset)
                        with torch.cuda.graph(g2, **mode):
                            self._step_update()
                        g = (g1, g2)
                self._graphs[gkey] = g
            else:
                g[0].replay()
                if g[1] is not None:
                    self._step_exchange()
                    g[1].replay()
        else:
            self._step_body(table, perm, row_begin, n_rows, global_rows, key_offset)
        if self.global_step < self.warmup_steps:
            f = (self.global_step + 1) / self.warmup_steps
            for gq in self.opt.param_groups:
                gq["lr"] = gq["initial_lr"] * f
        self.global_step += 1

    def train_step_host(self, host_table, row_begin: int, n_rows: int, global_rows: Optional[int] = None,
                        lagged: bool = False) -> float:
        if self._host_stage is None or len(self._host_stage[0]) < n_rows:
            from stnf.dataio import ObservationTable
            z = lambda *sh: torch.zeros(*sh, dtype=torch.float32, device=self.device)
            mk = lambda: ObservationTable(z(n_rows, 2), z(n_rows), z(n_rows),
                                          z(n_rows, self.model.p) if self.model.p > 0 else None)
            self._host_stage = [mk(), mk()]
            self._graphs.clear()
            self._host_perm = torch.arange(n_rows, dtype=torch.int64, device=self.device)
            self._host_copy_stream = torch.cuda.Stream(device=self.device)
            self._host_ready = [torch.cuda.Event(), torch.cuda.Event()]
            self._host_done = [torch.cuda.Event(), torch.cuda.Event()]
            self._host_loss = [torch.full((1,), float("nan")).pin_memory(), torch.full((1,), float("nan")).pin_memory()]
            self._host_k = 0
            self._host_pending = None
            main = torch.cuda.current_stream()
            for e in self._host_done:
                e.record(main)
        k = self._host_k
        self._host_k ^= 1
        st = self._host_stage[k]
        sl = slice(row_begin, row_begin + n_rows)
        main = torch.cuda.current_stream()

        def copy_batch():
            st.coords[:n_rows].copy_(host_table.coords[sl], non_blocking=True)
            st.t[:n_rows].copy_(host_table.t[sl], non_blocking=True)
            st.y[:n_rows].copy_(host_table.y[sl], non_blocking=True)
            if st.X is not None:
                st.X[:n_rows].copy_(host_table.X[sl], non_blocking=True)

        if lagged or self._host_pending is not None:
            with torch.cuda.stream(self._host_copy_stream):
                self._host_copy_stream.wait_event(self._host_done[k])
                copy_batch()
                self._host_ready[k].record(self._host_copy_stream)
            main.wait_event(self._host_ready[k])
        else:
            copy_batch()
        self.train_step(st, self._host_perm, 0, n_rows, global_rows)
        self._host_loss[k].copy_(self.loss_last, non_blocking=True)
        self._host_done[k].record(main)
        prev, self._host_pending = self._host_pending, k
        if not lagged:
            self._host_done[k].synchronize()
            self._host_pending = None
            return float(self._host_loss[k].item())
        if prev is None:
            return float("nan")
        self._host_done[prev].synchronize()
        return float(self._host_loss[prev].item())

    def flush_host_loss(self) -> float:
        if self._host_pending is None:
            return float("nan")
        k, self._host_pending = self._host_pending, None
        self._host_done[k].synchronize()
        return float(self._host_loss[k].item())

    @property
    def launches_per_step(self) -> int:
        nh = self.ex.spec.n_hidden
        n = 1
        n += nh + nh + nh
        if self.learnable:
            n += 3
        n += 1 if not self._norm_fused() else 2
        if self._peer is not None and self.world > 1:
            n += 1
        return n

    def profile_step(self, table, perm, n_rows: int, global_rows: int, repeats: int = 10) -> dict:
        rec: List[tuple] = []
        saved = {}

        def wrap(name, fn, flops_of):
            def inner(*a, **k):
                e0, e1 = torch.cuda.Event(enable_timing=True), torch.cuda.Event(enable_timing=True)
                e0.record()
                r = fn(*a, **k)
                e1.record()
                rec.append((name(*a, **k) if callable(name) else name, e0, e1, flops_of(*a, **k)))
                return r
            return inner

        rows = float(n_rows)
        f_fwd = lambda a: 2.0 * rows * a.layer.n_in * a.layer.n_out
        f_bwd = lambda a: 2.0 * rows * a.layer.n_out * (a.layer.n_in + (a.n_next if not a.head else 0))
        f_wg = lambda a: 2.0 * rows * a.n_in * a.n_out
        patches = {
            "layer_fwd": (lambda a: f"layer_fwd[{a.layer.layer_id}]", f_fwd),
            "layer_bwd": (lambda a: f"layer_bwd[{a.layer.layer_id}]", f_bwd),
            "wgrad": (lambda a: f"wgrad[{a.n_in}x{a.n_out}]", f_wg),
            "knot_grad": ("knot_grad", lambda a: 2.0 * rows * a.n_out * self.model.k_spatial),
# ... 172 lines not shown
```

Measured before the change: 27.85 million.

## Precompute dropout masks and prenormalized activations before PDL wait in backward and AdamW

Work that does not depend on the previous kernel's output now runs before the programmatic dependent launch wait. In the layer backward, dropout keep masks are generated early, and for TM=64 non-head layers the saved pre-activations are loaded, normalized and staged in tensor memory. The fused AdamW tail likewise loads hyperparameters and optimizer state (p, m, v, shadow) into registers before the wait. Together these overlap the previous kernel's tail. In exchange the kernels use more registers and tensor memory and take on extra code paths. Debug timing macros gated by a compile flag are also added.

New measurement: 29.01 million, median of 6. 4.2% higher.

```diff
diff --git a/include/stdadk.h b/include/stdadk.h
--- a/include/stdadk.h
+++ b/include/stdadk.h
@@ -80,6 +80,9 @@
     float* out_img_lo;
 } stdadk_fwd_args;
 
+#define STDADK_SETTLED_STEP 1
+#define STDADK_SETTLED_X 2
+
 typedef struct {
     const stdadk_basis* basis;
     stdadk_points pts;
@@ -92,7 +95,8 @@
     float* d_head_b;
     const float* dz_next_img;
     const float* wt_next_img;
-    int32_t n_next, _pad;
+    int32_t n_next;
+    int32_t settled;
     float* dz_img;
     float* d_bias;
     float* d_gamma;
@@ -147,7 +151,7 @@
     float* loss_sum;
     float* loss_last;
     int32_t fuse_norm;
-    int32_t _pad;
+    int32_t state_early;
     float* norm_ws;
 } stdadk_adamw_args;
 
diff --git a/st_dadk_b200/_lib.py b/st_dadk_b200/_lib.py
--- a/st_dadk_b200/_lib.py
+++ b/st_dadk_b200/_lib.py
@@ -13,6 +13,9 @@
 CALIBRATION = {"wendland": 1.0, "gaussian": 0.223477, "triangular": 0.654714}
 
 fp = C.c_void_p
+
+
+SETTLED_STEP, SETTLED_X = 1, 2
 
 
 class Basis(C.Structure):
@@ -50,7 +53,7 @@
 class BwdArgs(C.Structure):
     _fields_ = [("basis", C.POINTER(Basis)), ("pts", Points), ("a_img", fp), ("layer", Layer), ("drop", Dropout),
                 ("stats", fp), ("head", C.POINTER(Head)), ("d_head_w", fp), ("d_head_b", fp), ("dz_next_img", fp),
-                ("wt_next_img", fp), ("n_next", C.c_int32), ("_pad", C.c_int32), ("dz_img", fp), ("d_bias", fp),
+                ("wt_next_img", fp), ("n_next", C.c_int32), ("settled", C.c_int32), ("dz_img", fp), ("d_bias", fp),
                 ("d_gamma", fp), ("d_beta", fp), ("addend", fp), ("x_img", fp), ("a_img_lo", fp), ("dz_next_img_lo", fp),
                 ("wt_next_img_lo", fp), ("dz_img_lo", fp)]
 
@@ -71,7 +74,7 @@
                 ("n_groups", C.c_int32), ("zero_grad", C.c_int32), ("group_end", C.POINTER(C.c_int64)), ("hyper", fp),
                 ("sqnorms", fp), ("step_count", fp), ("beta1", C.c_float), ("beta2", C.c_float), ("eps", C.c_float),
                 ("ema_decay", C.c_float), ("loss_acc", fp), ("loss_sum", fp), ("loss_last", fp), ("fuse_norm", C.c_int32),
-                ("_pad", C.c_int32), ("norm_ws", fp)]
+                ("state_early", C.c_int32), ("norm_ws", fp)]
 
 
 MAX_LEVELS = 8
diff --git a/st_dadk_b200/csrc/api.cu b/st_dadk_b200/csrc/api.cu
--- a/st_dadk_b200/csrc/api.cu
+++ b/st_dadk_b200/csrc/api.cu
@@ -359,6 +359,8 @@
 }
 
 extern "C" void stdadk_debug_counters(void* dev_u64x16) { g_predict_dbg = static_cast<unsigned long long*>(dev_u64x16); }
+static unsigned long long* g_step_dbg = nullptr;
+extern "C" void stdadk_debug_step_counters(void* dev_u64x64) { g_step_dbg = static_cast<unsigned long long*>(dev_u64x64); }
 
 static int fill_pred_layers(const stdadk_layer* layers, int n_layers, PredLayerP* out, const char* who) {
     for (int l = 0; l < n_layers; ++l) {
@@ -548,6 +550,11 @@
     K.passes = x3 ? 3 : 1;
     K.addend = a->addend;
     K.x_img = a->x_img;
+    K.step_settled = a->x_img && (a->settled & STDADK_SETTLED_STEP) ? 1 : 0;
+    K.x_settled = a->x_img && (a->settled & STDADK_SETTLED_X) ? 1 : 0;
+#ifdef STDADK_PF_DEBUG
+    K.dbg = g_step_dbg && a->layer.layer_id < 7 ? g_step_dbg + 8 * a->layer.layer_id : nullptr;
+#endif
     K.stats = a->stats;
     K.dz_next_img = a->dz_next_img;
     K.wt_next_img = a->wt_next_img;
@@ -896,6 +903,8 @@
     K.eps = a->eps;
     K.ema_decay = a->ema_decay;
     K.g_zero = a->zero_grad ? const_cast<float*>(a->g) : nullptr;
+    K.state_early = a->fuse_norm && a->state_early ? 1 : 0;
+    K.dbg = g_step_dbg ? g_step_dbg + 56 : nullptr;
     K.loss_acc = a->loss_acc;
     K.loss_sum = a->loss_sum;
     K.loss_last = a->loss_last;
diff --git a/st_dadk_b200/csrc/common.cuh b/st_dadk_b200/csrc/common.cuh
--- a/st_dadk_b200/csrc/common.cuh
+++ b/st_dadk_b200/csrc/common.cuh
@@ -7,6 +7,27 @@
 #include "ptx.cuh"
 
 namespace stdadk {
+
+#ifdef STDADK_PF_DEBUG
+#define STEP_T_BEGIN(dbg)                                                  \
+    unsigned long long t_prev_ = 0;                                        \
+    if ((dbg) && threadIdx.x == 0) {                                       \
+        asm volatile("mov.u64 %0, %%globaltimer;" : "=l"(t_prev_));        \
+        atomicAdd((dbg) + 7, 1ull);                                        \
+    }
+#define STEP_T(dbg, slot)                                                  \
+    do {                                                                   \
+        if ((dbg) && threadIdx.x == 0) {                                   \
+            unsigned long long now_;                                       \
+            asm volatile("mov.u64 %0, %%globaltimer;" : "=l"(now_));       \
+            atomicAdd((dbg) + (slot), now_ - t_prev_);                     \
+            t_prev_ = now_;                                                \
+        }                                                                  \
+    } while (0)
+#else
+#define STEP_T_BEGIN(dbg)
+#define STEP_T(dbg, slot)
+#endif
 
 constexpr int TILE_M = 128;
 constexpr int SLAB_K = 32;
diff --git a/st_dadk_b200/csrc/layer.cuh b/st_dadk_b200/csrc/layer.cuh
--- a/st_dadk_b200/csrc/layer.cuh
+++ b/st_dadk_b200/csrc/layer.cuh
@@ -141,6 +141,10 @@
     float* d_head_w;
     float* d_head_b;
     int has_head, k_slabs, k_slabs2, n_pad, tmem_cols, passes;
+    int step_settled, x_settled;
+#ifdef STDADK_PF_DEBUG
+    unsigned long long* dbg;
+#endif
     unsigned int thresh16;
     float drop_scale;
 };
@@ -541,6 +545,24 @@
 #pragma unroll 1
     for (int b = 0; b < 4; ++b) keep |= dropout_keep8(seed, step, layer, key_row, (uint32_t)(c0 / 8 + b), thresh16) << (8 * b);
     return keep;
+}
+template <int TM, int CG, int MAXCH>
+__device__ __forceinline__ void chunk_keep_masks(const LayerP& L, unsigned int thresh16, long long lrow, int cg, int lane,
+                                                 int n_pad, uint32_t (&keeps)[MAXCH]) {
+    using G = TileGeo<TM>;
+    const bool drop = L.drop_p > 0.0f;
+    const unsigned int step = drop ? dropout_step(L) : 0u;
+    int ch = 0;
+    for (int wc = G::WARP_COLS * cg; wc < n_pad; wc += G::WARP_COLS * CG, ++ch) {
+        const int c0 = wc + G::chunk_off(lane);
+        const uint32_t kb = (drop && (TM == 128 || c0 < n_pad))
+                                ? pf_keep_mask(L.seed, step, (uint32_t)L.layer_id, L.key_offset + (unsigned long long)lrow,
+                                               c0, thresh16)
+                                : 0xFFFFFFFFu;
+#pragma unroll
+        for (int k = 0; k < MAXCH; ++k)
+            if (k == ch) keeps[k] = kb;
+    }
 }
 __device__ __forceinline__ void pf_dropout(float (&v)[32], uint32_t keep, float scale) {
 #pragma unroll
@@ -931,6 +953,7 @@
 
     const int tid = threadIdx.x, warp = tid >> 5, lane = tid & 31;
     const int tile = blockIdx.x;
+    STEP_T_BEGIN(P.dbg);
     const int itile = tile / (TILE_M / TM), irow0 = (tile % (TILE_M / TM)) * TM;
     const int n_pad = P.n_pad, n_out = P.L.n_out;
     constexpr bool has_ln = LN;
@@ -969,6 +992,7 @@
     __syncthreads();
     tc_fence_after();
     const uint32_t tmem_base = *tmem_slot;
+    STEP_T(P.dbg, 0);
 
     if (warp == 4 * CG) {
         if (lane == 0) {
@@ -1057,33 +1081,74 @@
             else if (P.basis.fn == STDADK_TRIANGULAR) gen_all(std::integral_constant<int, STDADK_TRIANGULAR>{});
             else gen_all(std::integral_constant<int, STDADK_GAUSSIAN>{});
         }
+        const uint32_t trow = tmem_base + ((uint32_t)(q4 * 32) << 16);
+        const bool drop = P.L.drop_p > 0.0f;
+        const float inv_n = 1.0f / (float)n_out;
+        float mean = 0.0f, rstd = 1.0f;
+        uint32_t actbits[MAXCH];
+        float z[32], g[32], tmp[32];
+        auto load_stats = [&]() {
+            if (has_ln && rvalid) {
+                mean = P.stats[2 * lrow];
+                rstd = P.stats[2 * lrow + 1];
+            }
+        };
+        constexpr bool X_EARLY_OK = TM == 64 && !HEAD;
+        const bool keeps_early = P.step_settled != 0;
+        const bool x_early = X_EARLY_OK && keeps_early && P.x_settled != 0;
+        if (keeps_early) chunk_keep_masks<TM, CG, MAXCH>(P.L, P.thresh16, lrow, cg, lane, n_pad, actbits);
+        if (x_early) {
+            load_stats();
+            int ch = 0;
+            for (int wc = G::WARP_COLS * cg; wc < n_pad; wc += WSTEP, ++ch) {
+                const int c0 = wc + coff;
+                const bool cvalid = c0 < n_pad;
+                if (cvalid) image_load_chunk(P.x_img, itile, n_pad / SLAB_K, c0, (uint32_t)irow, z);
+                else
+#pragma unroll
+                    for (int i = 0; i < 32; ++i) z[i] = 0.0f;
+                uint32_t keep = 0, act = 0;
+#pragma unroll
+                for (int k = 0; k < MAXCH; ++k)
+                    if (k == ch) keep = actbits[k];
+#pragma unroll
+                for (int i = 0; i < 32; ++i) {
+                    const int col = c0 + i;
+                    const float xh = has_ln ? (z[i] - mean) * rstd : z[i];
+                    const float yv = has_ln ? fmaf(xh, sgam[col], sbet[col]) : z[i];
+                    const bool on = (yv > 0.0f) && ((keep >> i) & 1u) && (col < n_out) && rvalid;
+                    act |= (on ? 1u : 0u) << i;
+                    z[i] = xh;
+                }
+#pragma unroll
+                for (int k = 0; k < MAXCH; ++k)
+                    if (k == ch) actbits[k] = act;
+                tmem_st32(trow + (uint32_t)(wc / 2), z);
+            }
+            tmem_st_wait();
+        }
+        STEP_T(P.dbg, 1);
         pdl_wait();
+        STEP_T(P.dbg, 2);
+        if (!x_early) load_stats();
         mbar_wait(accf, 0);
         tc_fence_after();
-        const uint32_t trow = tmem_base + ((uint32_t)(q4 * 32) << 16);
+        STEP_T(P.dbg, 3);
         float* myred = red + ((size_t)grp * TM + row) * RED_STRIDE;
         const float* arow = (P.addend && rvalid) ? P.addend + (size_t)lrow * n_out : nullptr;
-        float mean = 0.0f, rstd = 1.0f;
-        if (has_ln && rvalid) {
-            mean = P.stats[2 * lrow];
-            rstd = P.stats[2 * lrow + 1];
-        }
         float dyh[STDADK_MAX_Q];
 #pragma unroll
         for (int k = 0; k < STDADK_MAX_Q; ++k)
             dyh[k] = (HEAD && rvalid && k < q) ? P.head.dyhat[lrow * q + k] : 0.0f;
-        const bool drop = P.L.drop_p > 0.0f;
-        const unsigned int drop_step = drop ? dropout_step(P.L) : 0u;
-        const float inv_n = 1.0f / (float)n_out;
-        uint32_t actbits[MAXCH];
         float Sa = 0.0f, Sb = 0.0f;
-        float z[32], g[32], tmp[32];
 
         int ch = 0;
         for (int wc = G::WARP_COLS * cg; wc < n_pad; wc += WSTEP, ++ch) {
             const int c0 = wc + coff;
             const bool cvalid = TM == 128 || c0 < n_pad;
-            if (P.x_img) {
+            if (x_early) {
+                tmem_ld32(trow + (uint32_t)(wc / 2), z);
+            } else if (P.x_img) {
                 if (cvalid) image_load_chunk(P.x_img, itile, n_pad / SLAB_K, c0, (uint32_t)irow, z);
             } else {
                 acc_ld<TM>(trow + wc, z);
@@ -1091,38 +1156,46 @@
 #pragma unroll
                 for (int i = 0; i < 32; ++i) z[i] += sbias[c0 + i];
             }
-            if (!cvalid)
+            if (!cvalid && !x_early)
 #pragma unroll
                 for (int i = 0; i < 32; ++i) z[i] = 0.0f;
             if (!HEAD) acc_ld<TM>(trow + acc1_off + wc, g);
             else head_dh_chunk(g, dyh, shw, n_pad, c0, cvalid ? q : 0);
-            uint32_t keep = 0xFFFFFFFFu;
-            if (drop && cvalid) {
-                keep = 0;
-#pragma unroll 1
-                for (int b = 0; b < 4; ++b)
-                    keep |= dropout_keep8(P.L.seed, drop_step, (uint32_t)P.L.layer_id, P.L.key_offset + (unsigned long long)lrow,
-                                          (uint32_t)(c0 / 8 + b), P.thresh16)
-                            << (8 * b);
-            }
-            uint32_t act = 0;
-#pragma unroll
-            for (int i = 0; i < 32; ++i) {
-                const int col = c0 + i;
-                float x = z[i];
-                float xh = has_ln ? (x - mean) * rstd : x;
-                float yv = has_ln ? fmaf(xh, sgam[col], sbet[col]) : x;
-                bool on = (yv > 0.0f) && ((keep >> i) & 1u) && (col < n_out) && rvalid;
-                act |= (on ? 1u : 0u) << i;
-                const float dh = g[i];
-                float h = on ? yv * P.drop_scale : 0.0f;
-                g[i] = on ? dh * P.drop_scale : 0.0f;
-                z[i] = xh;
-                tmp[i] = h;
-            }
-#pragma unroll
-            for (int k = 0; k < MAXCH; ++k)
-                if (k == ch) actbits[k] = act;
+            if (x_early) {
+                uint32_t act = 0;
+#pragma unroll
+                for (int k = 0; k < MAXCH; ++k)
+                    if (k == ch) act = actbits[k];
+#pragma unroll
+                for (int i = 0; i < 32; ++i) g[i] = ((act >> i) & 1u) ? g[i] * P.drop_scale : 0.0f;
+            } else {
+                uint32_t keep = 0xFFFFFFFFu, act = 0;
+                if (keeps_early) {
+#pragma unroll
+                    for (int k = 0; k < MAXCH; ++k)
+                        if (k == ch) keep = actbits[k];
+                } else if (drop && cvalid) {
+                    keep = pf_keep_mask(P.L.seed, dropout_step(P.L), (uint32_t)P.L.layer_id,
+                                        P.L.key_offset + (unsigned long long)lrow, c0, P.thresh16);
+                }
+#pragma unroll
+                for (int i = 0; i < 32; ++i) {
+                    const int col = c0 + i;
+                    float x = z[i];
+                    float xh = has_ln ? (x - mean) * rstd : x;
+                    float yv = has_ln ? fmaf(xh, sgam[col], sbet[col]) : x;
+                    bool on = (yv > 0.0f) && ((keep >> i) & 1u) && (col < n_out) && rvalid;
+                    act |= (on ? 1u : 0u) << i;
+                    const float dh = g[i];
+                    float h = on ? yv * P.drop_scale : 0.0f;
+                    g[i] = on ? dh * P.drop_scale : 0.0f;
+                    z[i] = xh;
+                    tmp[i] = h;
+                }
+#pragma unroll
+                for (int k = 0; k < MAXCH; ++k)
+                    if (k == ch) actbits[k] = act;
+            }
             if (HEAD) {
                 for (int k = 0; k < q; ++k) {
                     float hv[32];
@@ -1149,6 +1222,7 @@
                 colsum_chunk<TM>(cs_bias, c0, cvalid, g, lane);
             }
         }
+        STEP_T(P.dbg, 4);
         if (HEAD && cg == 0) {
             for (int k = 0; k < q; ++k) {
                 float s = warp_sum(TM == 128 || lane < 16 ? dyh[k] : 0.0f);
@@ -1172,7 +1246,9 @@
             for (int wc = G::WARP_COLS * cg; wc < n_pad; wc += WSTEP, ++ch) {
                 const int c0 = wc + coff;
                 const bool cvalid = TM == 128 || c0 < n_pad;
-                if (P.x_img) {
+                if (x_early) {
+                    tmem_ld32(trow + (uint32_t)(wc / 2), z);
+                } else if (P.x_img) {
                     if (cvalid) image_load_chunk(P.x_img, itile, n_pad / SLAB_K, c0, (uint32_t)irow, z);
                 } else {
                     acc_ld<TM>(trow + wc, z);
@@ -1180,7 +1256,7 @@
 #pragma unroll
                     for (int i = 0; i < 32; ++i) z[i] += sbias[c0 + i];
                 }
-                if (!cvalid)
+                if (!cvalid && !x_early)
 #pragma unroll
                     for (int i = 0; i < 32; ++i) z[i] = 0.0f;
                 if (!HEAD) acc_ld<TM>(trow + acc1_off + wc, g);
@@ -1192,7 +1268,7 @@
 #pragma unroll
                 for (int i = 0; i < 32; ++i) {
                     const int col = c0 + i;
-                    float xh = (z[i] - mean) * rstd;
+                    float xh = x_early ? z[i] : (z[i] - mean) * rstd;
                     const float dh = g[i];
                     float gy = ((act >> i) & 1u) ? dh * P.drop_scale * sgam[col] : 0.0f;
                     float dz = rstd * (gy - ma - xh * mb);
@@ -1213,6 +1289,7 @@
             for (int k = 0; k < q; ++k) atomicAdd(&P.d_head_w[(size_t)k * n_out + c], cs_hw[k * n_pad + c]);
         }
         if (tid < q) atomicAdd(&P.d_head_b[tid], cs_hb[tid]);
+        STEP_T(P.dbg, 5);
     }
     __syncthreads();
     if (warp == 4 * CG) tmem_dealloc(tmem_base, (uint32_t)P.tmem_cols);
diff --git a/st_dadk_b200/csrc/misc.cuh b/st_dadk_b200/csrc/misc.cuh
--- a/st_dadk_b200/csrc/misc.cuh
+++ b/st_dadk_b200/csrc/misc.cuh
@@ -374,22 +374,64 @@
     float* sq_out;
     float* norm_ws;
     int* step_rw;
+    int state_early;
+    unsigned long long* dbg;
 };
+constexpr int TAIL_RES = 2;
 template <bool FUSED>
 __global__ void __launch_bounds__(256) adamw_ema_kernel(AdamK A) {
     __shared__ float s_sq[8];
+    const long long n4 = A.n >> 2;
+    const long long i0 = blockIdx.x * (long long)blockDim.x + threadIdx.x, stride = (long long)gridDim.x * blockDim.x;
+    const float4* g4 = reinterpret_cast<const float4*>(A.g);
+    float4* p4 = reinterpret_cast<float4*>(A.p);
+    float4* m4 = reinterpret_cast<float4*>(A.m);
+    float4* v4 = reinterpret_cast<float4*>(A.v);
+    float4* s4 = reinterpret_cast<float4*>(A.shadow);
+    const bool early = FUSED && A.state_early;
+    const bool resident = early && n4 <= TAIL_RES * stride;
+    float4 rg[TAIL_RES], rp[TAIL_RES], rm[TAIL_RES], rv[TAIL_RES], rs[TAIL_RES];
+    float hy[8][3];
     int step;
+    auto load_state = [&]() {
+        step = FUSED ? *A.step_count + 1 : *A.step_count;
+#pragma unroll
+        for (int k = 0; k < 8; ++k)
+            if (k < A.G.n) {
+                hy[k][0] = A.hyper[4 * k];
+                hy[k][1] = A.hyper[4 * k + 1];
+                hy[k][2] = A.hyper[4 * k + 2];
+            }
+        if (resident) {
+#pragma unroll
+            for (int r = 0; r < TAIL_RES; ++r) {
+                const long long i = i0 + r * stride;
+                if (i < n4) {
+                    rp[r] = p4[i];
+                    rm[r] = m4[i];
+                    rv[r] = v4[i];
+                    rs[r] = s4 ? s4[i] : make_float4(0.f, 0.f, 0.f, 0.f);
+                }
+            }
+        }
+    };
+    STEP_T_BEGIN(A.dbg);
+    if (early) load_state();
+    STEP_T(A.dbg, 0);
     if (FUSED) {
         pdl_wait();
-        step = *A.step_count + 1;
+        STEP_T(A.dbg, 1);
+        if (!early) load_state();
+        if (resident) {
+#pragma unroll
+            for (int r = 0; r < TAIL_RES; ++r)
+                if (i0 + r * stride < n4) rg[r] = __ldg(g4 + i0 + r * stride);
+        }
         float acc[8];
 #pragma unroll
         for (int k = 0; k < 8; ++k) acc[k] = 0.0f;
         if (A.sqnorms) {
-            const long long n4q = A.n >> 2;
-            const float4* gq = reinterpret_cast<const float4*>(A.g);
-            for (long long i = blockIdx.x * (long long)blockDim.x + threadIdx.x; i < n4q; i += (long long)gridDim.x * blockDim.x) {
-                const float4 v = __ldg(gq + i);
+            auto add_sq = [&](const float4 v, long long i) {
                 const long long e = i << 2;
                 const float vv[4] = {v.x, v.y, v.z, v.w};
 #pragma unroll
@@ -399,9 +441,16 @@
                     for (int k = 0; k < 8; ++k)
                         if (k == gi) acc[k] = fmaf(vv[j], vv[j], acc[k]);
                 }
+            };
+            if (resident) {
+#pragma unroll
+                for (int r = 0; r < TAIL_RES; ++r)
+                    if (i0 + r * stride < n4) add_sq(rg[r], i0 + r * stride);
+            } else {
+                for (long long i = i0; i < n4; i += stride) add_sq(__ldg(g4 + i), i);
             }
             if (blockIdx.x == 0 && threadIdx.x < (A.n & 3)) {
-                const long long i = (n4q << 2) + threadIdx.x;
+                const long long i = (n4 << 2) + threadIdx.x;
                 const float v = A.g[i];
                 const int gi = group_of(A.G, i);
 #pragma unroll
@@ -422,6 +471,7 @@
             for (int w = 0; w < 8; ++w) sk += wsum[w][threadIdx.x];
             A.norm_ws[blockIdx.x * 8 + threadIdx.x] = sk;
         }
+        STEP_T(A.dbg, 2);
         __threadfence();
         __syncthreads();
         if (threadIdx.x == 0) {
@@ -449,8 +499,9 @@
         }
         if (blockIdx.x == 0 && threadIdx.x == 0) *A.step_rw = step;
         __syncthreads();
+        STEP_T(A.dbg, 3);
     } else {
-        step = *A.step_count;
+        load_state();
     }
     const float bc1 = 1.0f - powf(A.beta1, (float)step);
     const float bc2 = 1.0f - powf(A.beta2, (float)step);
@@ -461,9 +512,9 @@
         lr[k] = wd[k] = 0.0f;
         clip[k] = 1.0f;
         if (k < A.G.n) {
-            lr[k] = A.hyper[4 * k];
-            wd[k] = A.hyper[4 * k + 1];
-            float mx = A.hyper[4 * k + 2];
+            lr[k] = hy[k][0];
+            wd[k] = hy[k][1];
+            float mx = hy[k][2];
             if (A.sqnorms && mx > 0.0f) clip[k] = fminf(1.0f, mx / (sqrtf(FUSED ? s_sq[k] : A.sqnorms[k]) + 1e-6f));
         }
     }
@@ -481,16 +532,7 @@
         p -= (l / bc1) * (m / denom);
         sh = A.ema_decay * sh + (1.0f - A.ema_decay) * p;
     };
-    const long long n4 = A.n >> 2;
-    const float4* g4 = reinterpret_cast<const float4*>(A.g);
-    float4* p4 = reinterpret_cast<float4*>(A.p);
-    float4* m4 = reinterpret_cast<float4*>(A.m);
-    float4* v4 = reinterpret_cast<float4*>(A.v);
-    float4* s4 = reinterpret_cast<float4*>(A.shadow);
-    for (long long i = blockIdx.x * (long long)blockDim.x + threadIdx.x; i < n4;
-         i += (long long)gridDim.x * blockDim.x) {
-        float4 g = __ldg(g4 + i), p = p4[i], m = m4[i], v = v4[i];
-        float4 sh = s4 ? s4[i] : make_float4(0.f, 0.f, 0.f, 0.f);
+    auto update4 = [&](long long i, float4 g, float4 p, float4 m, float4 v, float4 sh) {
         const long long e = i << 2;
         update(e, g.x, p.x, m.x, v.x, sh.x);
         update(e + 1, g.y, p.y, m.y, v.y, sh.y);
@@ -501,7 +543,16 @@
         v4[i] = v;
         if (s4) s4[i] = sh;
         if (A.g_zero) reinterpret_cast<float4*>(A.g_zero)[i] = make_float4(0.f, 0.f, 0.f, 0.f);
-    }
+    };
+    if (resident) {
+#pragma unroll
+        for (int r = 0; r < TAIL_RES; ++r)
+            if (i0 + r * stride < n4) update4(i0 + r * stride, rg[r], rp[r], rm[r], rv[r], rs[r]);
+    } else {
+        for (long long i = i0; i < n4; i += stride)
+            update4(i, __ldg(g4 + i), p4[i], m4[i], v4[i], s4 ? s4[i] : make_float4(0.f, 0.f, 0.f, 0.f));
+    }
+    STEP_T(A.dbg, 4);
     if (blockIdx.x == 0 && threadIdx.x == 0 && A.loss_acc && A.loss_sum) {
         const float step_loss = *A.loss_acc;
         *A.loss_sum += step_loss;
diff --git a/st_dadk_b200/executor.py b/st_dadk_b200/executor.py
--- a/st_dadk_b200/executor.py
+++ b/st_dadk_b200/executor.py
@@ -1,5 +1,6 @@
 from __future__ import annotations
 
+import os
 import ctypes as C
 from dataclasses import dataclass
 from typing import Dict, List, Optional, Sequence, Tuple
@@ -101,6 +102,7 @@
         self._knots_ready = False
         self._side = None
         self.fused_predict = True
+        self.prewait = os.environ.get("STDADK_PREWAIT", "1") != "0"
         self._fused_ok = None
         self._field_ok = None
         self._cell_ws = None
@@ -543,6 +545,8 @@
             a.drop = drop
             if ws.x is not None:
                 a.x_img = ws.x[l].data_ptr()
+                if self.prewait:
+                    a.settled = L.SETTLED_STEP | (L.SETTLED_X if l < nh - 1 else 0)
             if ws.stats[l] is not None:
                 a.stats = ws.stats[l].data_ptr()
                 a.d_gamma = g["gammas"][l].data_ptr()
diff --git a/st_dadk_b200/ops.py b/st_dadk_b200/ops.py
--- a/st_dadk_b200/ops.py
+++ b/st_dadk_b200/ops.py
@@ -212,11 +212,11 @@
 
 def adamw_ema_step(p, g, m, v, shadow, group_end: Sequence[int], hyper: torch.Tensor, sqnorms, step_count,
                    beta1=0.9, beta2=0.999, eps=1e-8, ema_decay=0.0, zero_grad=False, loss_acc=None, loss_sum=None,
-                   loss_last=None, norm_ws=None):
+                   loss_last=None, norm_ws=None, state_early=False):
     arr = (C.c_int64 * len(group_end))(*group_end)
     a = L.AdamWArgs(_ptr(p), _ptr(g), _ptr(m), _ptr(v), _ptr(shadow), p.numel(), len(group_end), int(bool(zero_grad)),
                     arr, _ptr(hyper), _ptr(sqnorms), _ptr(step_count), beta1, beta2, eps, ema_decay, _ptr(loss_acc),
-                    _ptr(loss_sum), _ptr(loss_last), int(norm_ws is not None), 0, _ptr(norm_ws))
+                    _ptr(loss_sum), _ptr(loss_last), int(norm_ws is not None), int(bool(state_early)), _ptr(norm_ws))
     L.check(L.lib().stdadk_adamw_ema_step(C.byref(a), _stream()), "adamw_ema_step")
 
 
diff --git a/st_dadk_b200/trainer.py b/st_dadk_b200/trainer.py
--- a/st_dadk_b200/trainer.py
+++ b/st_dadk_b200/trainer.py
@@ -373,7 +373,7 @@
         ops.adamw_ema_step(fl.p, fl.g[:fl.n], fl.m, fl.v, fl.shadow, fl.group_end, self.hyper,
                            self.sqnorms if self.clip > 0 else None, self.step_count, ema_decay=self.ema_decay,
                            zero_grad=True, loss_acc=ex.loss_acc, loss_sum=self.loss_sum, loss_last=self.loss_last,
-                           norm_ws=self._tail_ws if fused_tail else None)
+                           norm_ws=self._tail_ws if fused_tail else None, state_early=fused_tail and ex.prewait)
         if scratch_tail:
             fl.g[fl.n:fl.n + fl.n_scratch].zero_()
         self._g_clean = True
```
